# tokamak-network/Tokamak-zk-EVM

Measured on AMD Instinct MI355X. Metric: constraints/sec (prove step), higher is better.
Workload: dtype u32 limbs (255-bit Fr / 381-bit Fq modular integer arithmetic)

## Files before the change

include/tkmk.h:

```cpp
#ifndef TKMK_H
#define TKMK_H
#include <stdbool.h>
#include <stddef.h>
#include <stdint.h>

#ifdef __cplusplus
extern "C" {
#endif

typedef enum {
    TKMK_SUCCESS = 0,
    TKMK_ERR_INVALID_DEVICE = 1,
    TKMK_ERR_OUT_OF_MEMORY = 2,
    TKMK_ERR_INVALID_POINTER = 3,
    TKMK_ERR_ALLOCATION_FAILED = 4,
    TKMK_ERR_DEALLOCATION_FAILED = 5,
    TKMK_ERR_COPY_FAILED = 6,
    TKMK_ERR_SYNCHRONIZATION_FAILED = 7,
    TKMK_ERR_STREAM_CREATION_FAILED = 8,
    TKMK_ERR_STREAM_DESTRUCTION_FAILED = 9,
    TKMK_ERR_API_NOT_IMPLEMENTED = 10,
    TKMK_ERR_INVALID_ARGUMENT = 11,
    TKMK_ERR_NO_DEVICE = 12,
    TKMK_ERR_UNKNOWN = 999
} tkmk_error;

typedef struct { uint32_t limbs[8]; } tkmk_fr;
typedef struct { uint32_t limbs[12]; } tkmk_fq;
typedef struct { tkmk_fq x, y; } tkmk_g1_affine;
typedef struct { tkmk_fq x, y, z; } tkmk_g1_projective;
typedef void *tkmk_stream;

#define TKMK_BLS12_381_FR_ROOT_GENERATOR 5

tkmk_error tkmk_device_count(int *count);
tkmk_error tkmk_set_device(int device_id);
tkmk_error tkmk_diag_device_switch(int bound_device, int requested_device, int device_count);
tkmk_error tkmk_get_available_memory(size_t *total, size_t *free_bytes);
tkmk_error tkmk_malloc(void **ptr, size_t bytes);
tkmk_error tkmk_malloc_async(void **ptr, size_t bytes, tkmk_stream s);
tkmk_error tkmk_free(void *ptr);
tkmk_error tkmk_free_async(void *ptr, tkmk_stream s);
tkmk_error tkmk_memcpy_h2d(void *dst, const void *src, size_t bytes);
tkmk_error tkmk_memcpy_d2h(void *dst, const void *src, size_t bytes);
tkmk_error tkmk_memcpy_d2d(void *dst, const void *src, size_t bytes);
tkmk_error tkmk_memcpy_h2d_async(void *dst, const void *src, size_t bytes, tkmk_stream s);
tkmk_error tkmk_memcpy_d2h_async(void *dst, const void *src, size_t bytes, tkmk_stream s);
tkmk_error tkmk_memcpy_2d_d2d(void *dst, size_t dst_pitch, const void *src, size_t src_pitch, size_t width_bytes, size_t rows);
tkmk_error tkmk_memset(void *ptr, int value, size_t bytes);
tkmk_error tkmk_stream_create(tkmk_stream *s);
tkmk_error tkmk_stream_synchronize(tkmk_stream s);
tkmk_error tkmk_stream_destroy(tkmk_stream s);
tkmk_error tkmk_stream_set_background(tkmk_stream stream, int on);
tkmk_error tkmk_device_synchronize(void);
tkmk_error tkmk_release_scratch(void);
const char *tkmk_error_string(tkmk_error e);
tkmk_error bls12_381_generate_scalars(tkmk_fr *out_host, size_t n);
tkmk_error bls12_381_generate_random_affine_points(tkmk_g1_affine *out_host, size_t n);
int tkmk_is_hip_build(void);
tkmk_error tkmk_keccak256(const uint8_t *data, size_t len, uint8_t out[32]);
tkmk_error tkmk_r1cs_index(const uint8_t *section, size_t section_bytes, uint32_t n_constraints, uint32_t field_size,
                           uint64_t *starts, uint32_t *counts, size_t *consumed);

typedef struct {
    tkmk_stream stream_handle;
    int precompute_factor;
    int c;
    int bitsize;
    int batch_size;
    bool are_points_shared_in_batch;
    bool are_scalars_on_device;
    bool are_scalars_montgomery_form;
    bool are_points_on_device;
    bool are_points_montgomery_form;
    bool are_results_on_device;
    bool is_async;
    void *ext;
} tkmk_msm_config;

tkmk_msm_config tkmk_msm_default_config(void);

tkmk_error bls12_381_msm(const tkmk_fr *scalars, const tkmk_g1_affine *bases, int msm_size,
                         const tkmk_msm_config *cfg, tkmk_g1_projective *results);

tkmk_error bls12_381_msm_precompute_bases(const tkmk_g1_affine *bases, int msm_size, const tkmk_msm_config *cfg,
                                          tkmk_g1_affine *output_bases);

typedef struct {
    const tkmk_fr *scalars;
    const tkmk_g1_affine *bases;
    int msm_size;
} tkmk_msm_job;
tkmk_error tkmk_msm_multi(const tkmk_msm_job *jobs, int n_jobs, const tkmk_msm_config *cfg, tkmk_g1_projective *results);

#define TKMK_BASES_PLAIN 0
#define TKMK_BASES_MONTGOMERY 1
#define TKMK_BASES_CONVERTED 2
typedef struct {
    const tkmk_fr *scalars;
    const tkmk_g1_affine *bases;
    int msm_size;
    uint32_t scalar_cols, scalar_stride;
    uint32_t base_cols, base_stride;
    const uint32_t *base_index;
    uint64_t base_table_len;
    uint32_t table_c, table_factor;
} tkmk_msm_job_ex;
tkmk_error tkmk_msm_multi_ex(const tkmk_msm_job_ex *jobs, int n_jobs, const tkmk_msm_config *cfg, int bases_form,
                             tkmk_g1_projective *results);
tkmk_error bls12_381_msm_convert_bases(const tkmk_g1_affine *bases, uint64_t n, const tkmk_msm_config *cfg, tkmk_g1_affine *out);

typedef enum { TKMK_NTT_FORWARD = 0, TKMK_NTT_INVERSE = 1 } tkmk_ntt_dir;
typedef enum { TKMK_ORDER_NN = 0 } tkmk_ntt_ordering;

typedef struct {
    tkmk_stream stream_handle;
    tkmk_fr coset_gen;
    int batch_size;
    bool columns_batch;
    tkmk_ntt_ordering ordering;
    bool are_inputs_on_device;
    bool are_outputs_on_device;
    bool is_async;
    void *ext;
} tkmk_ntt_config;

typedef struct {
    tkmk_stream stream_handle;
    bool is_async;
    void *ext;
} tkmk_ntt_init_domain_config;

tkmk_ntt_config tkmk_ntt_default_config(void);
tkmk_error bls12_381_get_root_of_unity(uint64_t max_size, tkmk_fr *rou_out);
tkmk_error bls12_381_ntt_init_domain(const tkmk_fr *primitive_root, const tkmk_ntt_init_domain_config *cfg);
tkmk_error bls12_381_ntt_release_domain(void);
tkmk_error bls12_381_ntt_domain_size(uint64_t *size);
tkmk_error bls12_381_ntt(const tkmk_fr *input, int size, tkmk_ntt_dir dir, const tkmk_ntt_config *cfg,
                         tkmk_fr *output);

tkmk_error tkmk_bintt(const tkmk_fr *input, size_t x_size, size_t y_size, tkmk_ntt_dir dir,
                      const tkmk_fr *coset_x, const tkmk_fr *coset_y, bool on_device,
                      tkmk_stream stream, tkmk_fr *output);
tkmk_error tkmk_bintt_padded(const tkmk_fr *input, size_t in_x, size_t in_y, size_t x_size, size_t y_size, const tkmk_fr *coset_x,
                             const tkmk_fr *coset_y, tkmk_stream stream, tkmk_fr *output);

typedef struct {
    tkmk_stream stream_handle;
    bool is_a_on_device;
    bool is_b_on_device;
    bool is_result_on_device;
    bool is_async;
    int batch_size;
    bool columns_batch;
    void *ext;
} tkmk_vecops_config;

tkmk_vecops_config tkmk_vecops_default_config(void);
tkmk_error bls12_381_vector_add(const tkmk_fr *a, const tkmk_fr *b, uint64_t n, const tkmk_vecops_config *cfg, tkmk_fr *out);
tkmk_error bls12_381_vector_accumulate(tkmk_fr *a, const tkmk_fr *b, uint64_t n, const tkmk_vecops_config *cfg);
tkmk_error bls12_381_vector_sub(const tkmk_fr *a, const tkmk_fr *b, uint64_t n, const tkmk_vecops_config *cfg, tkmk_fr *out);
tkmk_error bls12_381_vector_mul(const tkmk_fr *a, const tkmk_fr *b, uint64_t n, const tkmk_vecops_config *cfg, tkmk_fr *out);
tkmk_error bls12_381_vector_div(const tkmk_fr *a, const tkmk_fr *b, uint64_t n, const tkmk_vecops_config *cfg, tkmk_fr *out);
tkmk_error bls12_381_vector_inv(const tkmk_fr *a, uint64_t n, const tkmk_vecops_config *cfg, tkmk_fr *out);
tkmk_error bls12_381_scalar_add_vec(const tkmk_fr *a, const tkmk_fr *b, uint64_t n, const tkmk_vecops_config *cfg, tkmk_fr *out);
tkmk_error bls12_381_scalar_sub_vec(const tkmk_fr *a, const tkmk_fr *b, uint64_t n, const tkmk_vecops_config *cfg, tkmk_fr *out);
tkmk_error bls12_381_scalar_mul_vec(const tkmk_fr *a, const tkmk_fr *b, uint64_t n, const tkmk_vecops_config *cfg, tkmk_fr *out);
tkmk_error bls12_381_vector_sum(const tkmk_fr *a, uint64_t n, const tkmk_vecops_config *cfg, tkmk_fr *out);
tkmk_error bls12_381_vector_product(const tkmk_fr *a, uint64_t n, const tkmk_vecops_config *cfg, tkmk_fr *out);
tkmk_error tkmk_vec_suffix_product(const tkmk_fr *a_dev, uint64_t n, tkmk_fr *out_dev, tkmk_stream stream);
tkmk_error bls12_381_matrix_transpose(const tkmk_fr *in, uint32_t rows, uint32_t cols, const tkmk_vecops_config *cfg, tkmk_fr *out);

tkmk_error tkmk_g1_ntt(const tkmk_g1_affine *in_dev, int bases_form, uint32_t in_stride, uint32_t x_size, uint32_t y_size, tkmk_ntt_dir dir,
                       tkmk_g1_affine *out_dev, tkmk_stream stream);
#define TKMK_G1_NTT_AXIS_X 1
#define TKMK_G1_NTT_AXIS_Y 2
tkmk_error tkmk_g1_ntt_axes(const tkmk_g1_affine *in_dev, int bases_form, uint32_t in_stride, uint32_t x_size, uint32_t y_size, tkmk_ntt_dir dir,
                            int axes, tkmk_g1_affine *out_dev, tkmk_stream stream);
tkmk_error tkmk_g1_scale(const tkmk_g1_affine *in_dev, uint64_t n, const tkmk_fr *scalar, tkmk_g1_affine *out_dev, tkmk_stream stream);
tkmk_error tkmk_g1_prefix_sums(const tkmk_g1_affine *in_dev, int bases_form, uint32_t rows, uint32_t cols, int transposed,
                               tkmk_g1_affine *out_dev, tkmk_stream stream);

typedef struct { tkmk_fq c0, c1; } tkmk_fq2;
typedef struct { tkmk_fq2 x, y; } tkmk_g2_affine;
typedef struct { tkmk_fq2 x, y, z; } tkmk_g2_projective;
tkmk_error bls12_381_g2_msm(const tkmk_fr *scalars, const tkmk_g2_affine *bases, int msm_size, const tkmk_msm_config *cfg,
                            tkmk_g2_projective *results);

typedef struct { uint32_t limbs[8]; } tkmk_bn254_fr;
typedef struct { uint32_t limbs[8]; } tkmk_bn254_fq;
typedef struct { tkmk_bn254_fq x, y; } tkmk_bn254_g1_affine;
typedef struct { tkmk_bn254_fq x, y, z; } tkmk_bn254_g1_projective;
tkmk_error bn254_msm(const tkmk_bn254_fr *scalars, const tkmk_bn254_g1_affine *bases, int msm_size,
                     const tkmk_msm_config *cfg, tkmk_bn254_g1_projective *results);
typedef struct {
    const tkmk_bn254_fr *scalars;
    const tkmk_bn254_g1_affine *bases;
    int msm_size;
} tkmk_bn254_msm_job;
tkmk_error bn254_msm_precompute_bases(const tkmk_bn254_g1_affine *bases, int msm_size, const tkmk_msm_config *cfg,
                                      tkmk_bn254_g1_affine *output_bases);
tkmk_error tkmk_bn254_msm_multi(const tkmk_bn254_msm_job *jobs, int n_jobs, const tkmk_msm_config *cfg,
                                tkmk_bn254_g1_projective *results);
tkmk_error bn254_get_root_of_unity(uint64_t max_size, tkmk_bn254_fr *rou_out);
tkmk_error bn254_ntt_init_domain(const tkmk_bn254_fr *primitive_root, const tkmk_ntt_init_domain_config *cfg);
tkmk_error bn254_ntt_release_domain(void);
tkmk_error bn254_ntt_domain_size(uint64_t *size);
tkmk_error bn254_ntt(const tkmk_bn254_fr *input, int size, tkmk_ntt_dir dir, const tkmk_ntt_config *cfg,
                     tkmk_bn254_fr *output);
tkmk_error tkmk_bn254_bintt(const tkmk_bn254_fr *input, size_t x_size, size_t y_size, tkmk_ntt_dir dir,
                            const tkmk_bn254_fr *coset_x, const tkmk_bn254_fr *coset_y, bool on_device, tkmk_stream stream,
                            tkmk_bn254_fr *output);
tkmk_error tkmk_bn254_fr_random_device(uint64_t seed, uint64_t first, uint64_t n, tkmk_bn254_fr *out_dev, tkmk_stream s);
tkmk_error tkmk_bn254_g1_batch_scalar_mul_device(const tkmk_bn254_fr *scalars_dev, const tkmk_bn254_g1_affine *base_host,
                                                 uint64_t n, tkmk_bn254_g1_affine *out_dev, tkmk_stream s);

tkmk_error tkmk_fr_random_device(uint64_t seed, uint64_t first, uint64_t n, tkmk_fr *out_dev, tkmk_stream s);
tkmk_error tkmk_gather_rows_device(const void *src_dev, uint32_t row_bytes, const uint32_t *idx_dev, uint64_t n, void *dst_dev,
                                   tkmk_stream s);
tkmk_error tkmk_g1_batch_scalar_mul_device(const tkmk_fr *scalars_dev, const tkmk_g1_affine *base_host,
                                           uint64_t n, tkmk_g1_affine *out_dev, tkmk_stream s);

tkmk_error tkmk_poly_find_degree(const tkmk_fr *coeffs_dev, uint32_t x_size, uint32_t y_size, int64_t *x_degree,
                                 int64_t *y_degree, tkmk_stream stream);
tkmk_error tkmk_poly_place(const tkmk_fr *src_dev, uint32_t sx, uint32_t sy, tkmk_fr *dst_dev, uint32_t dx, uint32_t dy,
                           uint32_t off_x, uint32_t off_y, tkmk_stream stream);
tkmk_error tkmk_poly_scale_coeffs(const tkmk_fr *src_dev, uint32_t x_size, uint32_t y_size, const tkmk_fr *factor_x,
                                  const tkmk_fr *factor_y, tkmk_fr *dst_dev, tkmk_stream stream);
tkmk_error tkmk_poly_mul_ones_x(const tkmk_fr *p_dev, uint32_t x_size, uint32_t y_size, uint32_t m, const tkmk_fr *scale,
                                uint32_t out_x_size, tkmk_fr *out_dev, tkmk_stream stream);
tkmk_error tkmk_poly_mul_x_minus_one_evals(const tkmk_fr *evals_dev, uint32_t x_size, uint32_t y_size, tkmk_fr *dst_dev,
                                           tkmk_stream stream);

typedef enum {
    TKMK_EXPR_LEAF = 0, TKMK_EXPR_CONST = 1, TKMK_EXPR_ADD = 2, TKMK_EXPR_SUB = 3, TKMK_EXPR_MUL = 4, TKMK_EXPR_SCALE = 5,
    TKMK_EXPR_MUL_X_MINUS_ONE = 6
} tkmk_expr_opcode;
typedef struct { uint8_t op; uint8_t arg; } tkmk_expr_instr;
tkmk_error tkmk_poly_expr_eval(const tkmk_expr_instr *prog, uint32_t n_instr, const tkmk_fr *const *leaves_dev, uint32_t n_leaves,
                               const tkmk_fr *consts, uint32_t n_consts, uint32_t x_size, uint32_t y_size, tkmk_fr *out_dev,
                               tkmk_stream stream);
typedef struct {
    const tkmk_fr *data;
    uint32_t x_len, y_len, rot_x, rot_y;
} tkmk_expr_leaf;
tkmk_error tkmk_poly_expr_eval_views(const tkmk_expr_instr *prog, uint32_t n_instr, const tkmk_expr_leaf *leaves, uint32_t n_leaves,
                                     const tkmk_fr *consts, uint32_t n_consts, uint32_t x_size, uint32_t y_size, tkmk_fr *out_dev,
                                     tkmk_stream stream);
tkmk_error tkmk_poly_expr_eval_views_slab(const tkmk_expr_instr *prog, uint32_t n_instr, const tkmk_expr_leaf *leaves, uint32_t n_leaves,
                                          const tkmk_fr *consts, uint32_t n_consts, uint32_t x_global, uint32_t x_first, uint32_t x_rows,
                                          uint32_t y_size, tkmk_fr *out_dev, tkmk_stream stream);
tkmk_error tkmk_poly_eval_x(const tkmk_fr *coeffs_dev, uint32_t x_size, uint32_t y_size, const tkmk_fr *x, tkmk_fr *out_dev,
                            tkmk_stream stream);
tkmk_error tkmk_poly_eval_y(const tkmk_fr *coeffs_dev, uint32_t x_size, uint32_t y_size, const tkmk_fr *y, tkmk_fr *out_dev,
                            tkmk_stream stream);
tkmk_error tkmk_poly_eval(const tkmk_fr *coeffs_dev, uint32_t x_size, uint32_t y_size, const tkmk_fr *x, const tkmk_fr *y,
                          tkmk_fr *out_host, tkmk_stream stream);
tkmk_error tkmk_poly_div_by_vanishing_opt(const tkmk_fr *p_dev, uint32_t x_size, uint32_t y_size, uint32_t c, uint32_t d,
                                          tkmk_fr *quo_x_dev, tkmk_fr *quo_y_dev, tkmk_stream stream);
tkmk_error tkmk_poly_lincomb(uint32_t n_terms, const tkmk_fr *coeffs_host, const tkmk_fr *const *polys_dev, const uint32_t *x_sizes,
                             const uint32_t *y_sizes, const uint32_t *off_x, const uint32_t *off_y, tkmk_fr *out_dev, uint32_t out_xs,
                             uint32_t out_ys, tkmk_stream stream);
tkmk_error tkmk_poly_div_by_ruffini(const tkmk_fr *p_dev, uint32_t x_size, uint32_t y_size, const tkmk_fr *x, const tkmk_fr *y,
// ... 56 lines not shown
```

tokamak-zk-evm_amd/csrc/ec_u.h:

```cpp
#pragma once
#include "ec.h"
#include "ffu.h"

template <class P>
struct ecu {
    using FU = ffu<P>;
    using FS = ff<P>;
    using GS = ec<FS>;
    using E = typename FU::E;
    struct A {
        E x, y;
    };
    struct X {
        E x, y, zz, zzz;
        bool inf;
    };

    static FF_HD X inf() {
        X r;
        r.x = FU::zero();
        r.y = FU::zero();
        r.zz = FU::zero();
        r.zzz = FU::zero();
        r.inf = true;
        return r;
    }
    static FF_HD bool load_affine(A &q, const affine_t<FS> &rec) {
        if (FS::is_zero(rec.x) && FS::is_zero(rec.y)) return false;
        q.x = FU::from_packed(rec.x);
        q.y = FU::from_packed(rec.y);
        return true;
    }
    static FF_HD A neg(const A &q) {
        A r;
        r.x = q.x;
        E m;
#pragma unroll
        for (int i = 0; i < FU::L; i++) m.l[i] = P::MODU[i];
        E t;
        uint32_t br = 0;
#pragma unroll
        for (int i = 0; i < FU::L; i++) {
            uint32_t d = m.l[i] - q.y.l[i] - br;
            br = d >> 31;
            t.l[i] = i < FU::L - 1 ? (d & FU::MASK) : d;
        }
        r.y = t;
        return r;
    }
    static FF_HD X from_affine(const A &q) {
        X r;
        r.x = q.x;
        r.y = q.y;
        r.zz = FU::one();
        r.zzz = FU::one();
        r.inf = false;
        return r;
    }

    static FF_HD xyzz_t<FS> to_sat(const X &p) {
        xyzz_t<FS> r;
        if (p.inf) return GS::inf();
        r.x = FU::to_sat_mont(p.x);
        r.y = FU::to_sat_mont(p.y);
        r.zz = FU::to_sat_mont(p.zz);
        r.zzz = FU::to_sat_mont(p.zzz);
        return r;
    }
    static FF_HD xyzz_t<FS> to_raw(const X &p) {
        xyzz_t<FS> r;
        if (p.inf) return GS::inf();
        r.x = FU::pack(FU::norm(p.x));
        r.y = FU::pack(FU::norm(p.y));
        r.zz = FU::pack(FU::norm(p.zz));
        r.zzz = FU::pack(FU::norm(p.zzz));
        return r;
    }
    static FF_HD xyzz_t<FS> raw_to_sat(const xyzz_t<FS> &raw) {
        if (FS::is_zero(raw.zz)) return GS::inf();
        xyzz_t<FS> r;
        r.x = FU::to_sat_mont(FU::unpack(raw.x));
        r.y = FU::to_sat_mont(FU::unpack(raw.y));
        r.zz = FU::to_sat_mont(FU::unpack(raw.zz));
        r.zzz = FU::to_sat_mont(FU::unpack(raw.zzz));
        return r;
    }
    static FF_HD X from_raw(const xyzz_t<FS> &raw) {
        X r;
        r.inf = FS::is_zero(raw.zz);
        if (r.inf) return inf();
        r.x = FU::unpack(raw.x);
        r.y = FU::unpack(raw.y);
        r.zz = FU::unpack(raw.zz);
        r.zzz = FU::unpack(raw.zzz);
        return r;
    }
    static FF_HD E from_sat_mont(const typename FS::E &s) {
        typename FS::E k;
#pragma unroll
        for (int i = 0; i < FS::N; i++) k.l[i] = P::KSATM[i];
        return FU::unpack(FS::mul(s, k));
    }
    static FF_HD X from_sat(const xyzz_t<FS> &p) {
        X r;
        r.inf = GS::is_inf(p);
        if (r.inf) return inf();
        r.x = from_sat_mont(p.x);
        r.y = from_sat_mont(p.y);
        r.zz = from_sat_mont(p.zz);
        r.zzz = from_sat_mont(p.zzz);
        return r;
    }
    static FF_HD X add_mixed_slow(const X &p, const A &q) {
        affine_t<FS> qs;
        qs.x = FU::to_sat_mont(q.x);
        qs.y = FU::to_sat_mont(q.y);
        return from_sat(GS::add_mixed(to_sat(p), qs));
    }

    static FF_HD X add_slow(const X &p, const X &q) { return from_sat(GS::add(to_sat(p), to_sat(q))); }
    static FF_HD X add(const X &p, const X &q) {
        if (p.inf) return q;
        if (q.inf) return p;
        E u1 = FU::mul(p.x, q.zz), u2 = FU::mul(q.x, p.zz);
        E s1 = FU::mul(p.y, q.zzz), s2 = FU::mul(q.y, p.zzz);
        E pd = FU::template sub<2>(u2, u1);
        if (FU::maybe_multiple_of_p(pd, 3)) return add_slow(p, q);
        E rd = FU::template sub<2>(s2, s1);
        E pp = FU::sqr(pd);
        E ppp = FU::mul(pd, pp);
        E qq = FU::mul(u1, pp);
        X r;
        r.inf = false;
        r.x = FU::template sub<4>(FU::sqr(rd), FU::add_dbl(ppp, qq));
        r.y = FU::mul_add(rd, FU::template sub<8>(qq, r.x), FU::template sub<2>(FU::zero(), s1), ppp);
        r.zz = FU::mul(FU::mul(p.zz, q.zz), pp);
        r.zzz = FU::mul(FU::mul(p.zzz, q.zzz), ppp);
        return r;
    }
    static FF_HD X dbl(const X &p) {
        if (p.inf) return p;
        E u = FU::dbl(p.y);
        E v = FU::sqr(u);
        E w = FU::mul(u, v);
        E sx = FU::mul(p.x, v);
        E x2 = FU::sqr(p.x);
        E m = FU::add(FU::dbl(x2), x2);
        X r;
        r.inf = false;
        r.x = FU::template sub<4>(FU::sqr(m), FU::dbl(sx));
        r.y = FU::mul_add(m, FU::template sub<8>(sx, r.x), FU::template sub<2>(FU::zero(), w), p.y);
        r.zz = FU::mul(v, p.zz);
        r.zzz = FU::mul(w, p.zzz);
        return r;
    }

    static FF_HD X add_mixed(const X &p, const A &q) {
        if (p.inf) return from_affine(q);
        E u2 = FU::mul(q.x, p.zz);
        E s2 = FU::mul(q.y, p.zzz);
        E pd = FU::template sub<8>(u2, p.x);
        if (FU::maybe_multiple_of_p(pd, 9)) return add_mixed_slow(p, q);
        E rd = FU::template sub<2>(s2, p.y);
        E pp = FU::sqr(pd);
        E ppp = FU::mul(pd, pp);
        E qq = FU::mul(p.x, pp);
        X r;
        r.inf = false;
        E t = FU::add_dbl(ppp, qq);
        r.x = FU::template sub<4>(FU::sqr(rd), t);
        E d = FU::template sub<8>(qq, r.x);
        r.y = FU::mul_add(rd, d, FU::template sub<2>(FU::zero(), p.y), ppp);
        r.zz = FU::mul(p.zz, pp);
        r.zzz = FU::mul(p.zzz, ppp);
        return r;
    }
};

using G1U = ecu<bls12_381_fq_params>;
```

tokamak-zk-evm_amd/csrc/ffu.h:

```cpp
#pragma once
#include <stdint.h>

#include "ff.h"

#if !defined(__HIP_DEVICE_COMPILE__)
#include <assert.h>
#define FFU_ASSERT(c) assert(c)
#else
#define FFU_ASSERT(c) ((void)0)
#endif

template <class P>
struct ffu {
    static constexpr int L = P::LU;
    static constexpr int N = P::N;
    static constexpr uint32_t W = P::WU, MASK = (1u << P::WU) - 1;
    struct alignas(8) E {
        uint32_t l[L];
    };
    using S = Fp<P>;

    static FF_HD E zero() {
        E r;
#pragma unroll
        for (int i = 0; i < L; i++) r.l[i] = 0;
        return r;
    }
    static FF_HD E one() {
        E r;
#pragma unroll
        for (int i = 0; i < L; i++) r.l[i] = P::ONEU[i];
        return r;
    }
    static FF_HD bool strict(const E &a) {
        for (int i = 0; i < L - 1; i++)
            if (a.l[i] > MASK) return false;
        return true;
    }
    static FF_HD bool below(const E &a, uint32_t k) { return (uint64_t)a.l[L - 1] * 1024 <= (uint64_t)k * P::TOP_PER_P_X1024 + 1024; }

    static FF_HD E norm(const E &a) {
        E r;
        uint32_t c = 0;
#pragma unroll
        for (int i = 0; i < L - 1; i++) {
            uint32_t t = a.l[i] + c;
            r.l[i] = t & MASK;
            c = t >> W;
        }
        r.l[L - 1] = a.l[L - 1] + c;
        return r;
    }
    static FF_HD E add(const E &a, const E &b) {
        FFU_ASSERT(strict(a) && strict(b));
        E t;
#pragma unroll
        for (int i = 0; i < L; i++) t.l[i] = a.l[i] + b.l[i];
        return norm(t);
    }
    static FF_HD E dbl(const E &a) { return add(a, a); }
    static FF_HD E add_dbl(const E &a, const E &b) {
        FFU_ASSERT(strict(a) && strict(b));
        E t;
#pragma unroll
        for (int i = 0; i < L; i++) t.l[i] = a.l[i] + (b.l[i] << 1);
        return norm(t);
    }
    template <int K>
    static FF_HD E sub(const E &a, const E &b) {
        FFU_ASSERT(strict(a) && strict(b) && below(b, K));
        E t;
#pragma unroll
        for (int i = 0; i < L; i++) {
            uint32_t c = K == 2 ? P::SUB2[i] : K == 4 ? P::SUB4[i] : K == 8 ? P::SUB8[i] : P::SUB16[i];
            FFU_ASSERT(c >= b.l[i]);
            t.l[i] = a.l[i] + (c - b.l[i]);
        }
        return norm(t);
    }

    static FF_HD E mul(const E &a, const E &b) {
        FFU_ASSERT(strict(a) && strict(b) && a.l[L - 1] <= MASK && b.l[L - 1] <= MASK);
        uint32_t m[L];
        uint64_t acc = 0;
        E r;
#pragma unroll
        for (int k = 0; k < L; k++) {
#pragma unroll
            for (int j = 0; j <= k; j++) acc += (uint64_t)a.l[j] * b.l[k - j];
#pragma unroll
            for (int j = 0; j < k; j++) acc += (uint64_t)m[j] * P::MODU[k - j];
            m[k] = ((uint32_t)acc * P::INVU) & MASK;
            acc += (uint64_t)m[k] * P::MODU[0];
            acc >>= W;
        }
#pragma unroll
        for (int k = L; k < 2 * L - 1; k++) {
#pragma unroll
            for (int j = k - L + 1; j < L; j++) {
                acc += (uint64_t)a.l[j] * b.l[k - j];
                acc += (uint64_t)m[j] * P::MODU[k - j];
            }
            r.l[k - L] = (uint32_t)acc & MASK;
            acc >>= W;
        }
        r.l[L - 1] = (uint32_t)acc;
        return r;
    }
    static FF_HD E mul_add(const E &a, const E &b, const E &c, const E &d) {
        static_assert(3 * L < (1 << (64 - 2 * (int)W)), "column accumulator would overflow");
        FFU_ASSERT(strict(a) && strict(b) && strict(c) && strict(d));
        FFU_ASSERT(a.l[L - 1] <= MASK && b.l[L - 1] <= MASK && c.l[L - 1] <= MASK && d.l[L - 1] <= MASK);
        uint32_t m[L];
        uint64_t acc = 0;
        E r;
#pragma unroll
        for (int k = 0; k < L; k++) {
#pragma unroll
            for (int j = 0; j <= k; j++) {
                acc += (uint64_t)a.l[j] * b.l[k - j];
                acc += (uint64_t)c.l[j] * d.l[k - j];
            }
#pragma unroll
            for (int j = 0; j < k; j++) acc += (uint64_t)m[j] * P::MODU[k - j];
            m[k] = ((uint32_t)acc * P::INVU) & MASK;
            acc += (uint64_t)m[k] * P::MODU[0];
            acc >>= W;
        }
#pragma unroll
        for (int k = L; k < 2 * L - 1; k++) {
#pragma unroll
            for (int j = k - L + 1; j < L; j++) {
                acc += (uint64_t)a.l[j] * b.l[k - j];
                acc += (uint64_t)c.l[j] * d.l[k - j];
                acc += (uint64_t)m[j] * P::MODU[k - j];
            }
            r.l[k - L] = (uint32_t)acc & MASK;
            acc >>= W;
        }
        r.l[L - 1] = (uint32_t)acc;
        return r;
    }
    static FF_HD E sqr(const E &a) {
        FFU_ASSERT(strict(a) && a.l[L - 1] <= MASK);
        uint32_t m[L], a2[L];
#pragma unroll
        for (int i = 0; i < L; i++) a2[i] = a.l[i] << 1;
        uint64_t acc = 0;
        E r;
#pragma unroll
        for (int k = 0; k < L; k++) {
#pragma unroll
            for (int j = 0; 2 * j < k; j++) acc += (uint64_t)a2[j] * a.l[k - j];
            if ((k & 1) == 0) acc += (uint64_t)a.l[k / 2] * a.l[k / 2];
#pragma unroll
            for (int j = 0; j < k; j++) acc += (uint64_t)m[j] * P::MODU[k - j];
            m[k] = ((uint32_t)acc * P::INVU) & MASK;
            acc += (uint64_t)m[k] * P::MODU[0];
            acc >>= W;
        }
#pragma unroll
        for (int k = L; k < 2 * L - 1; k++) {
#pragma unroll
            for (int j = k - L + 1; 2 * j < k; j++) acc += (uint64_t)a2[j] * a.l[k - j];
            if ((k & 1) == 0) acc += (uint64_t)a.l[k / 2] * a.l[k / 2];
#pragma unroll
            for (int j = k - L + 1; j < L; j++) acc += (uint64_t)m[j] * P::MODU[k - j];
            r.l[k - L] = (uint32_t)acc & MASK;
            acc >>= W;
        }
        r.l[L - 1] = (uint32_t)acc;
        return r;
    }

    static FF_HD bool maybe_multiple_of_p(const E &a, uint32_t jmax) { return ((a.l[0] * P::PINVU) & MASK) <= jmax; }

    static FF_HD E unpack(const S &s) {
        E r;
#pragma unroll
        for (int i = 0; i < L; i++) {
            int bit = (int)W * i, w = bit >> 5, sh = bit & 31;
            uint32_t lo = w < N ? s.l[w] : 0u, hi = w + 1 < N ? s.l[w + 1] : 0u;
            uint32_t v = sh ? (lo >> sh) | (hi << (32 - sh)) : lo;
            r.l[i] = i < L - 1 ? (v & MASK) : v;
        }
        return r;
    }
    static FF_HD S pack(const E &a) {
        S s;
#pragma unroll
        for (int w = 0; w < N; w++) {
            uint32_t v = 0;
#pragma unroll
            for (int i = 0; i < L; i++) {
                int lo = (int)W * i - 32 * w;
                if (lo >= 32 || lo + 32 <= 0) continue;
                v |= lo >= 0 ? a.l[i] << lo : a.l[i] >> (-lo);
            }
            s.l[w] = v;
        }
        return s;
    }
    static FF_HD E cond_sub_p(const E &a) {
        E t;
        uint32_t br = 0;
#pragma unroll
        for (int i = 0; i < L; i++) {
            uint32_t d = a.l[i] - P::MODU[i] - br;
            br = d >> 31;
            t.l[i] = i < L - 1 ? (d & MASK) : d;
        }
        uint32_t keep = 0u - br;
        E r;
#pragma unroll
        for (int i = 0; i < L; i++) r.l[i] = (a.l[i] & keep) | (t.l[i] & ~keep);
        return r;
    }
    static FF_HD S to_sat_mont(const E &a) {
        E c;
#pragma unroll
        for (int i = 0; i < L; i++) c.l[i] = P::RSATU[i];
        return pack(cond_sub_p(mul(a, c)));
    }
    static FF_HD E from_packed(const S &s) { return unpack(s); }
};

using Fqu = ffu<bls12_381_fq_params>;
using fqu_t = Fqu::E;
```

tokamak-zk-evm_amd/csrc/msm.hip:

```cpp
#include <stdio.h>
#include <stdlib.h>

#include <algorithm>
#include <map>
#include <memory>
#include <mutex>
#include <vector>

#include "common.h"
#include "ec_u.h"

#define TK_MSM_PRIMARY 1
#define TK_MSM_NS tk_msm_bls12_381
#define TK_MSM_FR_PARAMS bls12_381_fr_params
#define TK_MSM_FQ_PARAMS bls12_381_fq_params
#define TK_MSM_SCALAR_BITS 255
#define TK_MSM_ABI_FR tkmk_fr
#define TK_MSM_ABI_AFFINE tkmk_g1_affine
#define TK_MSM_ABI_PROJ tkmk_g1_projective
#define TK_MSM_ABI_JOB tkmk_msm_job
#define TK_MSM_SYM_MSM bls12_381_msm
#define TK_MSM_SYM_MULTI tkmk_msm_multi
#define TK_MSM_SYM_PRECOMPUTE bls12_381_msm_precompute_bases
#define TK_MSM_ABI_JOB_EX tkmk_msm_job_ex
#define TK_MSM_SYM_MULTI_EX tkmk_msm_multi_ex
#define TK_MSM_SYM_CONVERT bls12_381_msm_convert_bases
#include "msm_impl.inc"
```

tokamak-zk-evm_amd/csrc/msm_impl.inc:

```
namespace TK_MSM_NS {

using FrP = TK_MSM_FR_PARAMS;
using FqP = TK_MSM_FQ_PARAMS;
using Fr = ff<FrP>;
using Fq = ff<FqP>;
using fr_t = Fr::E;
using fq_t = Fq::E;
using G1 = ec<Fq>;
using g1_affine_t = affine_t<Fq>;
using g1_xyzz_t = xyzz_t<Fq>;
using G1U = ecu<FqP>;
using G1K = G1;
using FqK = Fq;
using g1k_xyzz = g1_xyzz_t;
using g1k_aff = g1_affine_t;
using abi_fr = TK_MSM_ABI_FR;
using abi_affine = TK_MSM_ABI_AFFINE;
using abi_proj = TK_MSM_ABI_PROJ;
using abi_job = TK_MSM_ABI_JOB;
#ifdef TK_MSM_SYM_MULTI_EX
using abi_job_ex = TK_MSM_ABI_JOB_EX;
#endif
constexpr size_t AFF_BYTES = sizeof(g1_affine_t), FR_BYTES = sizeof(fr_t);

static_assert(sizeof(g1_affine_t) == 2 * 4 * Fq::N && sizeof(g1_xyzz_t) == 4 * 4 * Fq::N, "layout");
static_assert(sizeof(abi_fr) == FR_BYTES && sizeof(abi_affine) == AFF_BYTES && sizeof(abi_proj) == 3 * 4 * Fq::N, "ABI layout");
static_assert(Fr::N == 8, "k_digits reads 8 scalar limbs");

struct msm_plan_t {
    uint32_t n;
    uint32_t c;
    uint32_t W;
    uint32_t B;
    uint32_t chunks;
    uint32_t chunk_len;
    uint32_t bits;
    uint32_t n_src;
    uint32_t W_src;
    uint32_t chunk;
    uint32_t win_parts;
    uint32_t hi_bits, lo_bits;
    uint32_t big;
};

struct msm_view_t {
    const uint32_t *index;
    uint32_t cols, stride;
    uint32_t limit;
    uint32_t *flag;
};
__device__ __forceinline__ uint32_t view_at(const msm_view_t &v, uint32_t k) {
    uint32_t r = k;
    if (v.index) r = v.index[k];
    else if (v.cols) {
        uint32_t row = k / v.cols;
        r = row * v.stride + (k - row * v.cols);
    }
    if (v.limit && r >= v.limit) {
        if (v.flag) atomicOr(v.flag, 1u);
        r = 0;
    }
    return r;
}
__device__ __forceinline__ uint32_t view_at_expanded(const msm_view_t &v, uint32_t k, uint32_t n_src, uint32_t level_rows) {
    if (!level_rows) return view_at(v, k);
    uint32_t j = k / n_src;
    return j * level_rows + view_at(v, k - j * n_src);
}
static inline msm_view_t view_identity() { return msm_view_t{nullptr, 0, 0, 0, nullptr}; }
static inline bool view_is_identity(const msm_view_t &v) { return !v.index && !v.cols; }

__global__ __launch_bounds__(256) void k_convert_bases(const g1_affine_t *__restrict__ in, g1_affine_t *__restrict__ out,
                                                      uint64_t n, int in_montgomery, msm_view_t bv) {
    uint64_t i = (uint64_t)blockIdx.x * blockDim.x + threadIdx.x;
    if (i >= n) return;
    g1_affine_t p = tk_load(in + view_at(bv, (uint32_t)i));
    if (!G1::is_inf(p)) {
        fq_t k;
#pragma unroll
        for (int j = 0; j < Fq::N; j++) k.l[j] = in_montgomery ? FqP::KSATM[j] : FqP::KSAT[j];
        p.x = Fq::mul(Fq::canon(p.x), k);
        p.y = Fq::mul(Fq::canon(p.y), k);
    }
    tk_store(out + i, p);
}

__global__ __launch_bounds__(256) void k_digits(const fr_t *__restrict__ scalars, uint32_t *__restrict__ dig, msm_plan_t pl,
                                               int scalars_mont, msm_view_t sv) {
    uint32_t i = blockIdx.x * blockDim.x + threadIdx.x;
    if (i >= pl.n_src) return;
    fr_t s = Fr::canon(tk_load(scalars + view_at(sv, i)));
    if (scalars_mont) s = Fr::from_mont(s);
    uint32_t carry = 0;
    const uint32_t mask = (1u << pl.c) - 1u;
    const uint32_t groups = pl.n / pl.n_src;
    uint32_t j = 0, t = 0;
    for (uint32_t w = 0; w < groups * pl.W; w++) {
        if (w >= pl.W_src) {
            dig[(uint64_t)t * pl.n + (uint64_t)j * pl.n_src + i] = 0;
            if (++t == pl.W) { t = 0; j++; }
            continue;
        }
        uint32_t lo = w * pl.c, li = lo >> 5, sh = lo & 31;
        uint32_t raw = 0;
        if (li < 8) {
            raw = s.l[li] >> sh;
            if (sh + pl.c > 32 && li + 1 < 8) raw |= s.l[li + 1] << (32 - sh);
        }
        raw &= mask;
        if (lo + pl.c > pl.bits) {
            uint32_t keep = pl.bits > lo ? pl.bits - lo : 0;
            raw &= keep >= 32 ? 0xffffffffu : ((1u << keep) - 1u);
        }
        uint32_t v = raw + carry;
        uint32_t rec;
        if (v > pl.B) {
            rec = ((1u << pl.c) - v) | 0x80000000u;
            carry = 1;
        } else {
            rec = v;
            carry = 0;
        }
        dig[(uint64_t)t * pl.n + (uint64_t)j * pl.n_src + i] = rec;
        if (++t == pl.W) { t = 0; j++; }
    }
}

__global__ __launch_bounds__(128) void k_precompute_bases(const g1_affine_t *__restrict__ in, g1_affine_t *__restrict__ out, uint64_t n,
                                                         int in_montgomery, uint32_t factor, uint32_t step) {
    uint64_t i = (uint64_t)blockIdx.x * blockDim.x + threadIdx.x;
    if (i >= n) return;
    g1_affine_t p = tk_load(in + i);
    const bool inf = G1::is_inf(p);
    if (!inf) {
        p.x = Fq::canon(p.x);
        p.y = Fq::canon(p.y);
        if (!in_montgomery) {
            p.x = Fq::to_mont(p.x);
            p.y = Fq::to_mont(p.y);
        }
    }
    fq_t k;
#pragma unroll
    for (int l = 0; l < Fq::N; l++) k.l[l] = FqP::KSATM[l];
    g1_xyzz_t acc = G1::from_affine(p);
    for (uint32_t j = 0; j < factor; j++) {
        g1_affine_t a = p;
        if (j) {
            for (uint32_t d = 0; d < step; d++) acc = G1::dbl(acc);
            a = G1::to_affine(acc);
        }
        if (!inf) {
            a.x = Fq::mul(a.x, k);
            a.y = Fq::mul(a.y, k);
        }
        tk_store(out + (uint64_t)j * n + i, a);
    }
}

__global__ __launch_bounds__(1024) void k_hist(const uint32_t *__restrict__ dig, uint32_t *__restrict__ counts, msm_plan_t pl,
                                              uint32_t shift) {
    extern __shared__ uint32_t hist[];
    const uint32_t w = blockIdx.y, ch = blockIdx.x;
    for (uint32_t b = threadIdx.x; b < pl.B; b += blockDim.x) hist[b] = 0;
    __syncthreads();
    uint32_t lo = ch * pl.chunk_len, hi = lo + pl.chunk_len;
    if (hi > pl.n) hi = pl.n;
    const uint32_t *d = dig + (uint64_t)w * pl.n;
    uint32_t i = lo + threadIdx.x;
    for (; i + 3 * 1024 < hi; i += 4 * 1024) {
        uint32_t r[4];
#pragma unroll
        for (int j = 0; j < 4; j++) r[j] = d[i + 1024 * j] & 0x7fffffffu;
#pragma unroll
        for (int j = 0; j < 4; j++)
            if (r[j]) atomicAdd(&hist[(r[j] - 1) >> shift], 1u);
    }
    for (; i < hi; i += 1024) {
        uint32_t r = d[i] & 0x7fffffffu;
        if (r) atomicAdd(&hist[(r - 1) >> shift], 1u);
    }
    __syncthreads();
    uint32_t *c = counts + (uint64_t)w * pl.B * pl.chunks;
    for (uint32_t b = threadIdx.x; b < pl.B; b += blockDim.x) c[(uint64_t)b * pl.chunks + ch] = hist[b];
}

__global__ __launch_bounds__(1024) void k_scan_local(const uint32_t *__restrict__ counts, uint32_t *__restrict__ local,
                                                    uint32_t *__restrict__ gtot, msm_plan_t pl) {
    __shared__ uint32_t part[1024];
    const uint32_t w = blockIdx.y, t = threadIdx.x, b = blockIdx.x * 1024 + t;
    uint32_t sum = 0;
    if (b < pl.B) {
        const uint32_t *c = counts + ((uint64_t)w * pl.B + b) * pl.chunks;
        uint32_t k = 0;
        for (; k + 8 <= pl.chunks; k += 8) {
            uint32_t v[8];
#pragma unroll
            for (int j = 0; j < 8; j++) v[j] = c[k + j];
#pragma unroll
            for (int j = 0; j < 8; j++) sum += v[j];
        }
        for (; k < pl.chunks; k++) sum += c[k];
    }
    part[t] = sum;
    __syncthreads();
    for (uint32_t off = 1; off < 1024; off <<= 1) {
        uint32_t v = t >= off ? part[t - off] : 0;
        __syncthreads();
        part[t] += v;
        __syncthreads();
    }
    if (b < pl.B) local[(uint64_t)w * pl.B + b] = part[t] - sum;
    if (t == 1023) gtot[w * gridDim.x + blockIdx.x] = part[t];
}
__global__ __launch_bounds__(1024) void k_scan_apply(uint32_t *__restrict__ counts, const uint32_t *__restrict__ local,
                                                    const uint32_t *__restrict__ gtot, uint32_t *__restrict__ bstart, msm_plan_t pl) {
    const uint32_t w = blockIdx.y, t = threadIdx.x, b = blockIdx.x * 1024 + t;
    uint32_t base = 0, total = 0;
    for (uint32_t g = 0; g < gridDim.x; g++) {
        uint32_t v = gtot[w * gridDim.x + g];
        if (g < blockIdx.x) base += v;
        total += v;
    }
    uint32_t *bs = bstart + (uint64_t)w * (pl.B + 1);
    if (b < pl.B) {
        uint32_t run = base + local[(uint64_t)w * pl.B + b];
        bs[b] = run;
        uint32_t *c = counts + ((uint64_t)w * pl.B + b) * pl.chunks;
        uint32_t k = 0;
        for (; k + 8 <= pl.chunks; k += 8) {
            uint32_t v[8];
#pragma unroll
            for (int j = 0; j < 8; j++) v[j] = c[k + j];
#pragma unroll
            for (int j = 0; j < 8; j++) {
                c[k + j] = run;
                run += v[j];
            }
        }
        for (; k < pl.chunks; k++) {
            uint32_t v = c[k];
            c[k] = run;
            run += v;
        }
    }
    if (blockIdx.x == 0 && t == 0) bs[pl.B] = total;
}

#define SCW_TPB 16
#define SCW_BINS (1024 / SCW_TPB)
__global__ __launch_bounds__(1024) void k_scan_local_wide(const uint32_t *__restrict__ counts, uint32_t *__restrict__ local,
                                                         uint32_t *__restrict__ gtot, msm_plan_t pl) {
    __shared__ uint32_t binsum[SCW_BINS];
    const uint32_t w = blockIdx.y, t = threadIdx.x, slot = t / SCW_TPB, sub = t % SCW_TPB, b = blockIdx.x * SCW_BINS + slot;
    const uint32_t per = (pl.chunks + SCW_TPB - 1) / SCW_TPB, lo = sub * per, hi = lo + per < pl.chunks ? lo + per : pl.chunks;
    uint32_t sum = 0;
    if (b < pl.B) {
        const uint32_t *c = counts + ((uint64_t)w * pl.B + b) * pl.chunks;
        for (uint32_t k = lo; k < hi; k++) sum += c[k];
    }
#pragma unroll
    for (uint32_t off = SCW_TPB / 2; off > 0; off >>= 1) sum += __shfl_down(sum, off, SCW_TPB);
    if (sub == 0) binsum[slot] = sum;
    __syncthreads();
    if (t < SCW_BINS) {
        uint32_t mine = binsum[t], incl = mine;
#pragma unroll
        for (uint32_t off = 1; off < SCW_BINS; off <<= 1) {
            uint32_t v = __shfl_up(incl, off, SCW_BINS);
            if (t >= off) incl += v;
        }
        const uint32_t bb = blockIdx.x * SCW_BINS + t;
        if (bb < pl.B) local[(uint64_t)w * pl.B + bb] = incl - mine;
        if (t == SCW_BINS - 1) gtot[w * gridDim.x + blockIdx.x] = incl;
    }
}
__global__ __launch_bounds__(1024) void k_scan_apply_wide(uint32_t *__restrict__ counts, const uint32_t *__restrict__ local,
                                                         const uint32_t *__restrict__ gtot, uint32_t *__restrict__ bstart, msm_plan_t pl) {
    const uint32_t w = blockIdx.y, t = threadIdx.x, slot = t / SCW_TPB, sub = t % SCW_TPB, b = blockIdx.x * SCW_BINS + slot;
    const uint32_t per = (pl.chunks + SCW_TPB - 1) / SCW_TPB, lo = sub * per, hi = lo + per < pl.chunks ? lo + per : pl.chunks;
    uint32_t base = 0, total = 0;
    for (uint32_t g = 0; g < gridDim.x; g++) {
        uint32_t v = gtot[w * gridDim.x + g];
        if (g < blockIdx.x) base += v;
        total += v;
    }
    uint32_t *bs = bstart + (uint64_t)w * (pl.B + 1);
    uint32_t *c = counts + ((uint64_t)w * pl.B + (b < pl.B ? b : 0)) * pl.chunks;
    uint32_t sum = 0;
    if (b < pl.B)
        for (uint32_t k = lo; k < hi; k++) sum += c[k];
    uint32_t incl = sum;
#pragma unroll
    for (uint32_t off = 1; off < SCW_TPB; off <<= 1) {
        uint32_t v = __shfl_up(incl, off, SCW_TPB);
        if (sub >= off) incl += v;
    }
    if (b < pl.B) {
        const uint32_t bin_start = base + local[(uint64_t)w * pl.B + b];
        if (sub == 0) bs[b] = bin_start;
        uint32_t run = bin_start + incl - sum;
        for (uint32_t k = lo; k < hi; k++) {
            uint32_t v = c[k];
            c[k] = run;
            run += v;
        }
    }
    if (blockIdx.x == 0 && t == 0) bs[pl.B] = total;
}

__global__ __launch_bounds__(1024) void k_scatter(const uint32_t *__restrict__ dig, const uint32_t *__restrict__ counts,
// ... 48 lines not shown
        const uint32_t *cs = seg_start + (uint64_t)w * (coarse_bins + 1);
        uint32_t s0 = cs[cb], s1 = cs[cb + 1];
        uint32_t per = sc_part_len(s1 - s0, parts);
        lo = s0 + part * per;
        if (lo > s1) lo = s1;
        hi = lo + per < s1 ? lo + per : s1;
        base = s0;
    } else {
        lo = part * chunk_len;
        hi = lo + chunk_len < n ? lo + chunk_len : n;
        if (lo > n) lo = n;
    }
    in0 += (uint64_t)w * n;
    if (PASS_B) in1 += (uint64_t)w * n;
    out0 += (uint64_t)w * n;
    if (!PASS_B) out1 += (uint64_t)w * n;
    if (tid < bins) cur[tid] = cursors[((uint64_t)sgm * bins + tid) * parts + part] + base;
    hist[tid] = 0;
    __syncthreads();
    for (uint32_t tlo = lo; tlo < hi; tlo += SC_TILE) {
        uint32_t v0[SC_PER], v1[SC_PER], rk[SC_PER];
        bool ok[SC_PER];
#pragma unroll
        for (int j = 0; j < SC_PER; j++) {
            uint32_t k = tlo + tid + 1024u * j;
            ok[j] = k < hi;
            v0[j] = v1[j] = rk[j] = 0;
            if (ok[j]) {
                if (PASS_B) {
                    v0[j] = in0[k];
                    v1[j] = in1[k];
                } else {
                    uint32_t rec = in0[k], r = rec & 0x7fffffffu;
                    ok[j] = r != 0;
                    v0[j] = (ok[j] ? view_at_expanded(bv, k, n_src, level_rows) : 0u) | (rec & 0x80000000u);
                    v1[j] = r - 1;
                }
            }
            if (ok[j]) rk[j] = atomicAdd(&hist[PASS_B ? (v1[j] & fmask) : (v1[j] >> fbits)], 1u);
        }
        __syncthreads();
        static_assert(SC_MAXBINS == 1024, "one bin per thread of the 1024-thread workgroup");
        const uint32_t mine = hist[tid];
        uint32_t incl = mine;
        const uint32_t lane = tid & 63u, wave = tid >> 6;
#pragma unroll
        for (uint32_t off = 1; off < 64; off <<= 1) {
            uint32_t t = __shfl_up(incl, off, 64);
            if (lane >= off) incl += t;
        }
        if (lane == 63) wsum[wave] = incl;
        __syncthreads();
        uint32_t before = 0, total = 0;
#pragma unroll
        for (uint32_t w2 = 0; w2 < 16; w2++) {
            uint32_t v = wsum[w2];
            total += v;
            if (w2 < wave) before += v;
        }
        start[tid] = before + incl - mine;
        __syncthreads();
#pragma unroll
        for (int j = 0; j < SC_PER; j++)
            if (ok[j]) {
                uint32_t b = PASS_B ? (v1[j] & fmask) : (v1[j] >> fbits);
                uint32_t pos = start[b] + rk[j];
                sv0[pos] = v0[j];
                sv1[pos] = v1[j];
            }
        __syncthreads();
#pragma unroll
        for (int j = 0; j < SC_PER; j++) {
            uint32_t k2 = tid + 1024u * j;
            if (k2 < total) {
                uint32_t a0 = sv0[k2], a1 = sv1[k2];
                uint32_t b = PASS_B ? (a1 & fmask) : (a1 >> fbits);
                uint32_t g = cur[b] + (k2 - start[b]);
                out0[g] = a0;
                if (!PASS_B) out1[g] = (uint16_t)(a1 & fmask);
            }
        }
        __syncthreads();
        cur[tid] += hist[tid];
        hist[tid] = 0;
        __syncthreads();
    }
}

__global__ __launch_bounds__(1024) void k_hist_fine(const uint16_t *__restrict__ key, const uint32_t *__restrict__ seg_start,
                                                   uint32_t *__restrict__ counts, uint32_t n, uint32_t coarse_bins, uint32_t fbits) {
    __shared__ uint32_t hist[SC_MAXFINE];
    const uint32_t fb_n = 1u << fbits;
    const uint32_t tid = threadIdx.x, part = blockIdx.x, parts = gridDim.x, sgm = blockIdx.y;
    const uint32_t w = sgm / coarse_bins, cb = sgm - w * coarse_bins;
    const uint32_t *cs = seg_start + (uint64_t)w * (coarse_bins + 1);
    uint32_t s0 = cs[cb], s1 = cs[cb + 1];
    uint32_t per = sc_part_len(s1 - s0, parts);
    uint32_t lo = s0 + part * per;
    if (lo > s1) lo = s1;
    uint32_t hi = lo + per < s1 ? lo + per : s1;
    if (tid < fb_n) hist[tid] = 0;
    __syncthreads();
    const uint16_t *k = key + (uint64_t)w * n;
    uint32_t i = lo + tid;
    for (; i + 3 * 1024 < hi; i += 4 * 1024) {
        uint32_t r[4];
#pragma unroll
        for (int j = 0; j < 4; j++) r[j] = k[i + 1024 * j];
#pragma unroll
        for (int j = 0; j < 4; j++) atomicAdd(&hist[r[j] & (fb_n - 1)], 1u);
    }
    for (; i < hi; i += 1024) atomicAdd(&hist[k[i] & (fb_n - 1)], 1u);
    __syncthreads();
    if (tid < fb_n) counts[((uint64_t)sgm * fb_n + tid) * parts + part] = hist[tid];
}

__global__ __launch_bounds__(256) void k_bstart_assemble(const uint32_t *__restrict__ coarse_start, const uint32_t *__restrict__ fine_start,
                                                        uint32_t *__restrict__ bstart, uint32_t W, uint32_t B, uint32_t coarse_bins,
                                                        uint32_t fbits) {
    uint64_t e = (uint64_t)blockIdx.x * blockDim.x + threadIdx.x;
    if (e >= (uint64_t)W * (B + 1)) return;
    uint32_t w = (uint32_t)(e / (B + 1)), b = (uint32_t)(e - (uint64_t)w * (B + 1));
    const uint32_t *cs = coarse_start + (uint64_t)w * (coarse_bins + 1);
    if (b == B) {
        bstart[e] = cs[coarse_bins];
        return;
    }
    uint32_t cb = b >> fbits, fb = b & ((1u << fbits) - 1);
    bstart[e] = cs[cb] + fine_start[((uint64_t)w * coarse_bins + cb) * ((1u << fbits) + 1) + fb];
}

__global__ void k_count_entries(const uint32_t *__restrict__ bstart, uint32_t W, uint32_t B, unsigned long long *__restrict__ cell) {
    unsigned long long t = 0;
    for (uint32_t w = 0; w < W; w++) t += bstart[(uint64_t)w * (B + 1) + B];
    atomicAdd(cell, t);
}

#define MSM_CHUNK 64
#define MSM_BIG 12
#define MSM_GIANT 2048
#define MSM_GIANT_PARTS 32
#define MSM_GIANT_CAP 2048

__device__ __forceinline__ uint32_t bucket_of(const uint32_t *__restrict__ bs, uint32_t B, uint32_t pos) {
    uint32_t lo = 0, hi = B;
    while (hi - lo > 1) {
        uint32_t mid = (lo + hi) >> 1;
        if (bs[mid] <= pos) lo = mid;
        else hi = mid;
    }
    return lo;
}

__global__ __launch_bounds__(256, 2) void k_accumulate_chunks(const g1_affine_t *__restrict__ bases, const uint32_t *__restrict__ sorted,
                                                          const uint32_t *__restrict__ bstart, g1_xyzz_t *__restrict__ buckets,
                                                          g1_xyzz_t *__restrict__ frag_head, g1_xyzz_t *__restrict__ frag_tail,
                                                          msm_plan_t pl, uint32_t chunks_per_window) {
    uint32_t gid = blockIdx.x * blockDim.x + threadIdx.x;
    if (gid >= pl.W * chunks_per_window) return;
    uint32_t w = gid / chunks_per_window, t = gid - w * chunks_per_window;
    const uint32_t *bs = bstart + (uint64_t)w * (pl.B + 1);
    const uint32_t total = bs[pl.B];
    uint32_t lo = t * pl.chunk;
    if (lo >= total) return;
    uint32_t hi = lo + pl.chunk < total ? lo + pl.chunk : total;
    const uint32_t *s = sorted + (uint64_t)w * pl.n;
    uint32_t b = bucket_of(bs, pl.B, lo);
    uint32_t bend = bs[b + 1];
    while (bend <= lo) bend = bs[++b + 1];
    const bool first_starts_here = bs[b] == lo;
    uint32_t nb = b + 2 <= pl.B ? bs[b + 2] : 0xffffffffu;
    uint32_t seg_lo = lo;
    G1U::X acc = G1U::inf();
    uint32_t rec_next = s[lo], rec_next2 = lo + 1 < hi ? s[lo + 1] : 0u;
    g1_affine_t raw = tk_load(bases + (rec_next & 0x7fffffffu));
    for (uint32_t k = lo; k < hi; k++) {
        const uint32_t rec = rec_next;
        G1U::A q;
        const bool have = G1U::load_affine(q, raw);
        rec_next = rec_next2;
        if (k + 1 < hi) {
            raw = tk_load(bases + (rec_next & 0x7fffffffu));
        }
        if (k + 2 < hi) rec_next2 = s[k + 2];
        if (have) {
            if (rec & 0x80000000u) q = G1U::neg(q);
            acc = G1U::add_mixed(acc, q);
        }
        if (k + 1 == bend || k + 1 == hi) {
            bool whole = (seg_lo != lo || first_starts_here) && k + 1 == bend;
            g1_xyzz_t *dst;
            if (whole) dst = buckets + (uint64_t)w * pl.B + b;
            else if (seg_lo == lo) dst = frag_head + (uint64_t)w * chunks_per_window + t;
            else dst = frag_tail + (uint64_t)w * chunks_per_window + t;
            tk_store(dst, G1U::to_raw(acc));
            acc = G1U::inf();
            seg_lo = k + 1;
            if (k + 1 < hi) {
                do {
                    b++;
                    bend = nb;
                    nb = b + 2 <= pl.B ? bs[b + 2] : 0xffffffffu;
                } while (bend <= k + 1);
            }
        }
    }
}

__global__ __launch_bounds__(256) void k_combine(const uint32_t *__restrict__ bstart, g1_xyzz_t *__restrict__ buckets,
                                                const g1_xyzz_t *__restrict__ frag_head, const g1_xyzz_t *__restrict__ frag_tail,
                                                msm_plan_t pl, uint32_t chunks_per_window, uint32_t *__restrict__ big,
                                                uint32_t big_cap, uint32_t *__restrict__ giant) {
    uint32_t gid = blockIdx.x * blockDim.x + threadIdx.x;
    if (gid >= pl.W * pl.B) return;
    uint32_t w = gid / pl.B, b = gid - w * pl.B;
    const uint32_t *bs = bstart + (uint64_t)w * (pl.B + 1);
    uint32_t sb = bs[b], eb = bs[b + 1];
    if (eb == sb) return;
    uint32_t t0 = sb / pl.chunk, t1 = (eb - 1) / pl.chunk;
    if (t0 == t1) return;
    if (t1 - t0 > MSM_GIANT) {
        uint32_t slot = atomicAdd(&giant[0], 1u);
        if (slot < MSM_GIANT_CAP) {
            giant[1 + slot] = gid;
            return;
        }
    }
    if (t1 - t0 > pl.big) {
        uint32_t slot = atomicAdd(&big[0], 1u);
        if (slot < big_cap) {
            big[1 + slot] = gid;
            return;
        }
    }
    const g1_xyzz_t *fh = frag_head + (uint64_t)w * chunks_per_window, *ft = frag_tail + (uint64_t)w * chunks_per_window;
    G1U::X acc = G1U::from_raw(tk_load(sb == t0 * pl.chunk ? fh + t0 : ft + t0));
    for (uint32_t t = t0 + 1; t <= t1; t++) acc = G1U::add(acc, G1U::from_raw(tk_load(fh + t)));
    tk_store(buckets + gid, G1U::to_raw(acc));
}

__global__ __launch_bounds__(256) void k_combine_big(const uint32_t *__restrict__ bstart, g1_xyzz_t *__restrict__ buckets,
                                                    const g1_xyzz_t *__restrict__ frag_head, const g1_xyzz_t *__restrict__ frag_tail,
                                                    msm_plan_t pl, uint32_t chunks_per_window, const uint32_t *__restrict__ big,
                                                    uint32_t big_cap) {
    __shared__ g1_xyzz_t sh[256];
    const uint32_t lane = threadIdx.x & 63u, wave = threadIdx.x >> 6;
    uint32_t count = big[0] < big_cap ? big[0] : big_cap;
    for (uint32_t base = blockIdx.x * 4u; base < count; base += gridDim.x * 4u) {
        const uint32_t i = base + wave;
        const bool live = i < count;
        uint32_t gid = 0;
        G1U::X acc = G1U::inf();
        if (live) {
            gid = big[1 + i];
            uint32_t w = gid / pl.B, b = gid - w * pl.B;
            const uint32_t *bs = bstart + (uint64_t)w * (pl.B + 1);
            uint32_t sb = bs[b], eb = bs[b + 1];
            uint32_t t0 = sb / pl.chunk, t1 = (eb - 1) / pl.chunk;
            const g1_xyzz_t *fh = frag_head + (uint64_t)w * chunks_per_window, *ft = frag_tail + (uint64_t)w * chunks_per_window;
            for (uint32_t t = t0 + lane; t <= t1; t += 64) {
                const g1_xyzz_t *src = (t == t0 && sb != t0 * pl.chunk) ? ft + t : fh + t;
                acc = G1U::add(acc, G1U::from_raw(tk_load(src)));
            }
        }
        sh[threadIdx.x] = G1U::to_raw(acc);
        __syncthreads();
        for (uint32_t st = 32; st > 0; st >>= 1) {
            if (lane < st) {
                acc = G1U::add(acc, G1U::from_raw(sh[threadIdx.x + st]));
                sh[threadIdx.x] = G1U::to_raw(acc);
            }
            __syncthreads();
        }
        if (live && lane == 0) tk_store(buckets + gid, G1U::to_raw(acc));
        __syncthreads();
    }
}

__global__ __launch_bounds__(256) void k_combine_giant_parts(const uint32_t *__restrict__ bstart, const g1_xyzz_t *__restrict__ frag_head,
                                                            const g1_xyzz_t *__restrict__ frag_tail, msm_plan_t pl,
                                                            uint32_t chunks_per_window, const uint32_t *__restrict__ giant,
                                                            g1_xyzz_t *__restrict__ part_out) {
    __shared__ g1_xyzz_t sh[256];
    uint32_t count = giant[0] < MSM_GIANT_CAP ? giant[0] : MSM_GIANT_CAP;
    for (uint32_t item = blockIdx.x; item < count * MSM_GIANT_PARTS; item += gridDim.x) {
        uint32_t i = item / MSM_GIANT_PARTS, part = item - i * MSM_GIANT_PARTS;
        uint32_t gid = giant[1 + i];
        uint32_t w = gid / pl.B, b = gid - w * pl.B;
        const uint32_t *bs = bstart + (uint64_t)w * (pl.B + 1);
        uint32_t sb = bs[b], eb = bs[b + 1];
        uint32_t t0 = sb / pl.chunk, t1 = (eb - 1) / pl.chunk;
        uint32_t per = (t1 - t0 + MSM_GIANT_PARTS) / MSM_GIANT_PARTS;
        uint32_t lo = t0 + part * per, hi = lo + per - 1 < t1 ? lo + per - 1 : t1;
        const g1_xyzz_t *fh = frag_head + (uint64_t)w * chunks_per_window, *ft = frag_tail + (uint64_t)w * chunks_per_window;
        G1U::X acc = G1U::inf();
        for (uint32_t t = lo + threadIdx.x; t <= hi && lo <= t1; t += 256) {
            const g1_xyzz_t *src = (t == t0 && sb != t0 * pl.chunk) ? ft + t : fh + t;
            acc = G1U::add(acc, G1U::from_raw(tk_load(src)));
        }
        sh[threadIdx.x] = G1U::to_raw(acc);
        __syncthreads();
        for (uint32_t st = 128; st > 0; st >>= 1) {
            if (threadIdx.x < st) {
                acc = G1U::add(acc, G1U::from_raw(sh[threadIdx.x + st]));
                sh[threadIdx.x] = G1U::to_raw(acc);
            }
            __syncthreads();
        }
        if (threadIdx.x == 0) tk_store(part_out + item, G1U::to_raw(acc));
        __syncthreads();
    }
}
__global__ __launch_bounds__(64) void k_combine_giant_final(g1_xyzz_t *__restrict__ buckets, const uint32_t *__restrict__ giant,
                                                           const g1_xyzz_t *__restrict__ part_in) {
    __shared__ g1_xyzz_t sh[MSM_GIANT_PARTS];
    uint32_t count = giant[0] < MSM_GIANT_CAP ? giant[0] : MSM_GIANT_CAP;
    for (uint32_t i = blockIdx.x; i < count; i += gridDim.x) {
        G1U::X acc = G1U::inf();
        if (threadIdx.x < MSM_GIANT_PARTS) {
            sh[threadIdx.x] = tk_load(part_in + (uint64_t)i * MSM_GIANT_PARTS + threadIdx.x);
            acc = G1U::from_raw(sh[threadIdx.x]);
        }
        __syncthreads();
        for (uint32_t st = MSM_GIANT_PARTS / 2; st > 0; st >>= 1) {
            if (threadIdx.x < st) {
                acc = G1U::add(acc, G1U::from_raw(sh[threadIdx.x + st]));
                sh[threadIdx.x] = G1U::to_raw(acc);
            }
            __syncthreads();
        }
        if (threadIdx.x == 0) tk_store(buckets + giant[1 + i], G1U::to_raw(acc));
        __syncthreads();
    }
}

#define MSM_SEG 8
__global__ __launch_bounds__(128) void k_reduce_segments(const g1_xyzz_t *__restrict__ buckets, g1_xyzz_t *__restrict__ seg_out,
                                                        msm_plan_t pl, uint32_t segs) {
    uint32_t gid = blockIdx.x * blockDim.x + threadIdx.x;
    if (gid >= pl.W * segs) return;
    uint32_t w = gid / segs, sg = gid - w * segs;
    uint32_t v0 = sg * MSM_SEG;
    uint32_t len = pl.B - v0 < MSM_SEG ? pl.B - v0 : MSM_SEG;
    const g1_xyzz_t *bk = buckets + (uint64_t)w * pl.B + v0;
    G1U::X run = G1U::inf(), tot = G1U::inf();
    for (int k = (int)len - 1; k >= 0; k--) {
        run = G1U::add(run, G1U::from_raw(tk_load(bk + k)));
        tot = G1U::add(tot, run);
    }
    if (v0) {
        G1U::X m = G1U::inf();
        for (int bit = 31 - __builtin_clz(v0); bit >= 0; bit--) {
            m = G1U::dbl(m);
            if ((v0 >> bit) & 1) m = G1U::add(m, run);
        }
        tot = G1U::add(tot, m);
    }
    tk_store(seg_out + gid, G1U::to_raw(tot));
}

// ... 167 lines not shown
    }
    for (int i = 0; i < Fq::N; i++) {
        o->x.limbs[i] = x.l[i];
        o->y.limbs[i] = y.l[i];
        o->z.limbs[i] = z.l[i];
    }
}

#ifdef TK_MSM_PRIMARY
TK_API tkmk_msm_config tkmk_msm_default_config(void) {
    tkmk_msm_config c;
    c.stream_handle = nullptr;
    c.precompute_factor = 1;
    c.c = 0;
    c.bitsize = 0;
    c.batch_size = 1;
    c.are_points_shared_in_batch = true;
    c.are_scalars_on_device = false;
    c.are_scalars_montgomery_form = false;
    c.are_points_on_device = false;
    c.are_points_montgomery_form = false;
    c.are_results_on_device = false;
    c.is_async = false;
    c.ext = nullptr;
    return c;
}
#endif


static bool xyzz_same_point(const g1_xyzz_t &a, const g1_xyzz_t &b) {
    g1_affine_t pa = G1::to_affine(a), pb = G1::to_affine(b);
    return Fq::eq(pa.x, pb.x) && Fq::eq(pa.y, pb.y);
}
static tkmk_error msm_debug_check(const msm_plan_t &pl, const fr_t *scalars, const g1_affine_t *bases, const uint32_t *d_dig,
                                  const uint32_t *d_sorted, const uint32_t *d_bstart, const g1_xyzz_t *d_buckets, hipStream_t s) {
    TK_HIP(hipStreamSynchronize(s));
    TK_HIP(hipGetLastError());
    std::vector<fr_t> sc(pl.n);
    std::vector<g1_affine_t> bs(pl.n);
    std::vector<uint32_t> dig((size_t)pl.W * pl.n), sorted((size_t)pl.W * pl.n), bstart((size_t)pl.W * (pl.B + 1));
    std::vector<g1_xyzz_t> buckets((size_t)pl.W * pl.B);
    TK_HIP(hipMemcpy(sc.data(), scalars, sc.size() * sizeof(fr_t), hipMemcpyDeviceToHost));
    TK_HIP(hipMemcpy(bs.data(), bases, bs.size() * sizeof(g1_affine_t), hipMemcpyDeviceToHost));
    {
        fq_t rp;
        for (int j = 0; j < Fq::N; j++) rp.l[j] = FqP::KSATM[j];
        fq_t rinv = Fq::inv(Fq::to_mont(rp));
        for (auto &b : bs)
            if (!G1::is_inf(b)) {
                b.x = Fq::mul(Fq::to_mont(b.x), rinv);
                b.y = Fq::mul(Fq::to_mont(b.y), rinv);
            }
    }
    TK_HIP(hipMemcpy(dig.data(), d_dig, dig.size() * 4, hipMemcpyDeviceToHost));
    TK_HIP(hipMemcpy(sorted.data(), d_sorted, sorted.size() * 4, hipMemcpyDeviceToHost));
    TK_HIP(hipMemcpy(bstart.data(), d_bstart, bstart.size() * 4, hipMemcpyDeviceToHost));
    TK_HIP(hipMemcpy(buckets.data(), d_buckets, buckets.size() * sizeof(g1_xyzz_t), hipMemcpyDeviceToHost));
    fprintf(stderr, "[msm debug] n=%u c=%u W=%u B=%u chunks=%u chunk_len=%u\n", pl.n, pl.c, pl.W, pl.B, pl.chunks, pl.chunk_len);
    int bad = 0;
    for (uint32_t i = 0; i < pl.n && bad < 5; i++) {
        unsigned __int128 acc = 0;
        for (int w = (int)pl.W - 1; w >= 0; w--) {
            uint32_t rec = dig[(size_t)w * pl.n + i];
            long long d = (long long)(rec & 0x7fffffffu);
            if (rec & 0x80000000u) d = -d;
            if ((rec & 0x7fffffffu) > pl.B) { fprintf(stderr, "[msm debug] digit too large i=%u w=%d rec=%08x\n", i, w, rec); bad++; }
            if ((uint32_t)w * pl.c < 100) acc = (acc << pl.c) + (unsigned __int128)(__int128)d;
        }
        uint64_t lo = (uint64_t)sc[i].l[0] | ((uint64_t)sc[i].l[1] << 32);
        (void)lo;
    }
    for (uint32_t w = 0; w < pl.W; w++) {
        const uint32_t *bsw = &bstart[(size_t)w * (pl.B + 1)];
        uint32_t nz = 0;
        for (uint32_t i = 0; i < pl.n; i++) nz += (dig[(size_t)w * pl.n + i] & 0x7fffffffu) != 0;
        if (bsw[pl.B] != nz && bad < 20) { fprintf(stderr, "[msm debug] w=%u total %u != nonzero digits %u\n", w, bsw[pl.B], nz); bad++; }
        for (uint32_t b = 0; b < pl.B; b++) {
            if (bsw[b] > bsw[b + 1]) { if (bad < 20) fprintf(stderr, "[msm debug] w=%u b=%u bstart not monotone\n", w, b); bad++; continue; }
            g1_xyzz_t acc = G1::inf();
            for (uint32_t k = bsw[b]; k < bsw[b + 1]; k++) {
                uint32_t rec = sorted[(size_t)w * pl.n + k], i = rec & 0x7fffffffu;
                if (i >= pl.n) { if (bad < 20) fprintf(stderr, "[msm debug] w=%u b=%u bad index %u\n", w, b, i); bad++; continue; }
                uint32_t drec = dig[(size_t)w * pl.n + i];
                if ((drec & 0x7fffffffu) != b + 1 || ((drec ^ rec) & 0x80000000u)) {
                    if (bad < 20) fprintf(stderr, "[msm debug] w=%u b=%u entry %u: digit rec %08x does not belong here\n", w, b, k, drec);
                    bad++;
                }
                g1_affine_t pnt = bs[i];
                if (rec & 0x80000000u) pnt.y = Fq::neg(pnt.y);
                acc = G1::add_mixed(acc, pnt);
            }
            buckets[(size_t)w * pl.B + b] = G1U::raw_to_sat(buckets[(size_t)w * pl.B + b]);
            bool okb = xyzz_same_point(acc, buckets[(size_t)w * pl.B + b]);
            if (atoi(getenv("TKMK_MSM_DEBUG")) >= 2 && w == 7 && bsw[b + 1] > bsw[b])
                fprintf(stderr, "[msm debug] w7 b=%u pos=%u cnt=%u %s\n", b, bsw[b], bsw[b + 1] - bsw[b], okb ? "ok" : "BAD");
            if (!okb) {
                if (bad < 20) {
                    const g1_xyzz_t &dv = buckets[(size_t)w * pl.B + b];
                    uint32_t rec0 = bsw[b + 1] > bsw[b] ? sorted[(size_t)w * pl.n + bsw[b]] : 0;
                    const char *cls = "other";
                    if (G1::is_inf(dv)) cls = "inf";
                    else if (xyzz_same_point(G1::neg(acc), dv)) cls = "negated";
                    fprintf(stderr, "[msm debug] w=%u b=%u bucket sum mismatch (%u entries) rec0=%08x device=%s zz0=%08x x0=%08x\n", w, b,
                            bsw[b + 1] - bsw[b], rec0, cls, dv.zz.l[0], dv.x.l[0]);
                }
                bad++;
            }
        }
    }
    fprintf(stderr, "[msm debug] %d inconsistencies\n", bad);
    return TKMK_SUCCESS;
}

#define MSM_MAX_WINDOWS 128
static uint32_t msm_choose_chunk(uint64_t entries, uint32_t W, uint32_t n) {
    static const uint32_t slots = [] {
        int dev = 0, cus = 256;
        if (hipGetDevice(&dev) == hipSuccess) (void)hipDeviceGetAttribute(&cus, hipDeviceAttributeMultiprocessorCount, dev);
        if (cus <= 0) cus = 256;
        return (uint32_t)cus * 4u * 2u * 64u;
    }();
    if (getenv("TKMK_MSM_FIXED_CHUNK")) return MSM_CHUNK;
    if (const char *e = getenv("TKMK_MSM_CHUNK_LEN")) {
        int v = atoi(e);
        if (v >= 8 && v <= 8192) return (uint32_t)v;
    }
    uint64_t target = entries / (8ull * slots);
    if (target < 48) target = 48;
    if (target > 224) target = 224;
    uint64_t r = (entries + target * slots / 2) / (target * slots);
    if (r < 1) r = 1;
    uint64_t lanes_per_window = r * slots / W;
    if (lanes_per_window < 1) lanes_per_window = 1;
    uint64_t chunk = (n + lanes_per_window - 1) / lanes_per_window;
    if (chunk < 32) chunk = 32;
    if (chunk > 256) chunk = 256;
    if (entries > (1ull << 30)) {
        uint64_t big = entries / (32ull * slots);
        if (big > 4096) big = 4096;
        if (big > chunk) chunk = big;
    }
    return (uint32_t)chunk;
}
#define MSM_MAX_C 20
static uint32_t msm_resolve_c(uint32_t c_req, uint32_t n_src) {
    uint32_t c = c_req ? c_req : choose_c(n_src);
    if (c < 2) c = 2;
    if (c > MSM_MAX_C) c = MSM_MAX_C;
    static const bool force_one_pass = getenv("TKMK_MSM_ONE_PASS") != nullptr;
    if (c > 16 && (force_one_pass || n_src < (1u << 18))) c = 16;
    return c;
}

static thread_local bool tl_background_batch = false;
static tkmk_error msm_enqueue(const fr_t *scalars, const g1_affine_t *bases_mont, uint32_t n_src, uint32_t factor, uint32_t c_req,
                              uint32_t bits, bool scalars_mont, hipStream_t s, g1_xyzz_t *wins_host, msm_plan_t *plan_out,
                              msm_view_t sv = view_identity(), msm_view_t bv = view_identity(), uint32_t level_rows = 0) {
    msm_plan_t pl;
    static const bool force_one_pass = getenv("TKMK_MSM_ONE_PASS") != nullptr;
    pl.bits = bits;
    pl.c = level_rows ? c_req : msm_resolve_c(c_req, n_src);
    if (pl.c < 2 || pl.c > MSM_MAX_C) return TKMK_ERR_INVALID_ARGUMENT;
    pl.n_src = n_src;
    pl.W_src = bits / pl.c + 1;
    if (factor < 1) factor = 1;
    if (factor > pl.W_src) factor = pl.W_src;
    if ((uint64_t)n_src * factor >= (1ull << 31)) return TKMK_ERR_INVALID_ARGUMENT;
    if (factor > 1 && !view_is_identity(bv) && !level_rows) return TKMK_ERR_INVALID_ARGUMENT;
    if (level_rows && (uint64_t)level_rows * factor >= (1ull << 31)) return TKMK_ERR_INVALID_ARGUMENT;
    const uint32_t n = n_src * factor;
    pl.n = n;
    pl.W = (pl.W_src + factor - 1) / factor;
    pl.B = 1u << (pl.c - 1);
    pl.chunk = msm_choose_chunk((uint64_t)pl.W * n, pl.W, n);
    {
        static const uint32_t big_env = getenv("TKMK_MSM_BIG") ? (uint32_t)atoi(getenv("TKMK_MSM_BIG")) : 0u;
        const uint64_t avg_spans = (uint64_t)n / ((uint64_t)pl.chunk * pl.B);
        pl.big = big_env ? big_env : (avg_spans >= 4 ? 4u * MSM_BIG : MSM_BIG);
    }
    pl.win_parts = pl.W >= 8 ? MSM_WIN_PARTS : 32;
    pl.hi_bits = pl.lo_bits = 0;
    if (pl.W == 1 && pl.c >= 15) {
        pl.lo_bits = (pl.c - 1) / 2;
        pl.hi_bits = pl.c - 1 - pl.lo_bits;
    }
    static const bool no_rowcol = getenv("TKMK_MSM_SEGMENT_TAIL") != nullptr;
    if (no_rowcol) pl.hi_bits = pl.lo_bits = 0;
    uint32_t want = (512 + pl.W - 1) / pl.W;
    if (getenv("TKMK_MSM_CHUNKS")) want = (uint32_t)atoi(getenv("TKMK_MSM_CHUNKS"));
    uint32_t maxc = (n + 8191) / 8192;
    pl.chunks = want < maxc ? want : maxc;
    if (pl.chunks < 1) pl.chunks = 1;
    pl.chunk_len = (n + pl.chunks - 1) / pl.chunks;

    tk_scratch d_dig, d_sorted, d_counts, d_bstart, d_buckets, d_segs, d_wins;
    TK_TRY(d_dig.alloc((size_t)pl.W * n * 4, s));
    TK_TRY(d_sorted.alloc((size_t)pl.W * n * 4, s));
    const bool two_pass = !force_one_pass && pl.c >= 13 && n >= (1u << 18);
    if (pl.c > 16 && !two_pass) return TKMK_ERR_INVALID_ARGUMENT;
    {
        const uint32_t fb = pl.c >= 19 ? 9u : pl.c >= 17 ? 8u : 7u;
        TK_TRY(d_counts.alloc((size_t)pl.W * (two_pass ? (pl.B >> fb) : pl.B) * pl.chunks * 4, s));
    }
    TK_TRY(d_bstart.alloc((size_t)pl.W * (pl.B + 1) * 4, s));
    TK_TRY(d_buckets.alloc((size_t)pl.W * pl.B * sizeof(g1_xyzz_t), s));
    uint32_t segs = (pl.B + MSM_SEG - 1) / MSM_SEG;
    TK_TRY(d_segs.alloc((size_t)pl.W * segs * sizeof(g1_xyzz_t), s));
    TK_TRY(d_wins.alloc((size_t)pl.W * pl.win_parts * sizeof(g1_xyzz_t), s));

    tk_stat_add(TK_STAT_MSM_POINTS, n_src);
    tk_stat_add(TK_STAT_MSM_CALLS, 1);
    tk_prof prof(s);
    hipLaunchKernelGGL(k_digits, tk_div_up(n_src, 256), 256, 0, s, scalars, d_dig.as<uint32_t>(), pl, scalars_mont ? 1 : 0, sv);
    prof.mark("msm.digits");
    size_t lds = (size_t)pl.B * 4;
    static std::once_flag attr_once;
    static hipError_t attr_err = hipSuccess;
    std::call_once(attr_once, [] {
        attr_err = hipFuncSetAttribute((const void *)k_hist, hipFuncAttributeMaxDynamicSharedMemorySize, 128 * 1024);
        if (attr_err == hipSuccess)
            attr_err = hipFuncSetAttribute((const void *)k_scatter, hipFuncAttributeMaxDynamicSharedMemorySize, 128 * 1024);
    });
    TK_HIP(attr_err);
    if (!two_pass) {
        hipLaunchKernelGGL(k_hist, dim3(pl.chunks, pl.W), 1024, lds, s, (const uint32_t *)d_dig.p, d_counts.as<uint32_t>(), pl, 0u);
        prof.mark("msm.hist");
        const uint32_t groups = (pl.B + 1023) / 1024;
        tk_scratch d_local, d_gtot;
        TK_TRY(d_local.alloc((size_t)pl.W * pl.B * 4, s));
        TK_TRY(d_gtot.alloc((size_t)pl.W * groups * 4, s));
        hipLaunchKernelGGL(k_scan_local, dim3(groups, pl.W), 1024, 0, s, (const uint32_t *)d_counts.p, d_local.as<uint32_t>(),
                           d_gtot.as<uint32_t>(), pl);
        hipLaunchKernelGGL(k_scan_apply, dim3(groups, pl.W), 1024, 0, s, d_counts.as<uint32_t>(), (const uint32_t *)d_local.p,
                           (const uint32_t *)d_gtot.p, d_bstart.as<uint32_t>(), pl);
        prof.mark("msm.scan");
        hipLaunchKernelGGL(k_scatter, dim3(pl.chunks, pl.W), 1024, lds, s, (const uint32_t *)d_dig.p, (const uint32_t *)d_counts.p,
                           d_sorted.as<uint32_t>(), pl, bv, level_rows);
        prof.mark("msm.scatter");
    } else {
        const uint32_t fbits = pl.c >= 19 ? 9u : pl.c >= 17 ? 8u : 7u, FB = 1u << fbits, CB = pl.B >> fbits;
        tk_scratch d_aidx, d_akey, d_cs, d_localA, d_gtotA, d_cntB, d_fs, d_localB, d_gtotB;
        TK_TRY(d_aidx.alloc((size_t)pl.W * n * 4, s));
        TK_TRY(d_akey.alloc((size_t)pl.W * n * 2, s));
        TK_TRY(d_cs.alloc((size_t)pl.W * (CB + 1) * 4, s));
        msm_plan_t pa = pl;
        pa.B = CB;
        hipLaunchKernelGGL(k_hist, dim3(pl.chunks, pl.W), 1024, (size_t)CB * 4, s, (const uint32_t *)d_dig.p, d_counts.as<uint32_t>(), pa,
                           fbits);
        prof.mark("msm.hist");
        TK_TRY(d_localA.alloc((size_t)pl.W * CB * 4, s));
        const bool wide_scan = pl.W <= 4 && pl.chunks >= 64;
        const uint32_t groupsA = wide_scan ? (CB + SCW_BINS - 1) / SCW_BINS : 1u;
        TK_TRY(d_gtotA.alloc((size_t)pl.W * groupsA * 4, s));
        if (wide_scan) {
            hipLaunchKernelGGL(k_scan_local_wide, dim3(groupsA, pl.W), 1024, 0, s, (const uint32_t *)d_counts.p, d_localA.as<uint32_t>(),
                               d_gtotA.as<uint32_t>(), pa);
            hipLaunchKernelGGL(k_scan_apply_wide, dim3(groupsA, pl.W), 1024, 0, s, d_counts.as<uint32_t>(), (const uint32_t *)d_localA.p,
                               (const uint32_t *)d_gtotA.p, d_cs.as<uint32_t>(), pa);
        } else {
            hipLaunchKernelGGL(k_scan_local, dim3(1, pl.W), 1024, 0, s, (const uint32_t *)d_counts.p, d_localA.as<uint32_t>(),
                               d_gtotA.as<uint32_t>(), pa);
            hipLaunchKernelGGL(k_scan_apply, dim3(1, pl.W), 1024, 0, s, d_counts.as<uint32_t>(), (const uint32_t *)d_localA.p,
                               (const uint32_t *)d_gtotA.p, d_cs.as<uint32_t>(), pa);
        }
        prof.mark("msm.scan");
        hipLaunchKernelGGL(k_scatter_staged<false>, dim3(pl.chunks, pl.W), 1024, 0, s, (const uint32_t *)d_dig.p, (const uint16_t *)nullptr,
                           (const uint32_t *)nullptr, (const uint32_t *)d_counts.p, d_aidx.as<uint32_t>(), d_akey.as<uint16_t>(), n, CB, CB,
                           pl.chunk_len, fbits, bv, pl.n_src, level_rows);
        const uint32_t segs_b = pl.W * CB;
        TK_TRY(d_cntB.alloc((size_t)segs_b * FB * SC_PARTS * 4, s));
        TK_TRY(d_fs.alloc((size_t)segs_b * (FB + 1) * 4, s));
        TK_TRY(d_localB.alloc((size_t)segs_b * FB * 4, s));
        TK_TRY(d_gtotB.alloc((size_t)segs_b * 4, s));
        hipLaunchKernelGGL(k_hist_fine, dim3(SC_PARTS, segs_b), 1024, 0, s, (const uint16_t *)d_akey.p, (const uint32_t *)d_cs.p,
                           d_cntB.as<uint32_t>(), n, CB, fbits);
        msm_plan_t pb = pl;
        pb.B = FB;
        pb.chunks = SC_PARTS;
        hipLaunchKernelGGL(k_scan_local, dim3(1, segs_b), 1024, 0, s, (const uint32_t *)d_cntB.p, d_localB.as<uint32_t>(),
                           d_gtotB.as<uint32_t>(), pb);
        hipLaunchKernelGGL(k_scan_apply, dim3(1, segs_b), 1024, 0, s, d_cntB.as<uint32_t>(), (const uint32_t *)d_localB.p,
                           (const uint32_t *)d_gtotB.p, d_fs.as<uint32_t>(), pb);
        hipLaunchKernelGGL(k_bstart_assemble, tk_div_up((size_t)pl.W * (pl.B + 1), 256), 256, 0, s, (const uint32_t *)d_cs.p,
                           (const uint32_t *)d_fs.p, d_bstart.as<uint32_t>(), pl.W, pl.B, CB, fbits);
        hipLaunchKernelGGL(k_scatter_staged<true>, dim3(SC_PARTS, segs_b), 1024, 0, s, (const uint32_t *)d_aidx.p, (const uint16_t *)d_akey.p,
                           (const uint32_t *)d_cs.p, (const uint32_t *)d_cntB.p, d_sorted.as<uint32_t>(), (uint16_t *)nullptr, n, FB, CB,
                           0u, fbits, view_identity(), 0u, 0u);
        prof.mark("msm.scatter");
    }
    if (unsigned long long *cell = tk_stat_device_entries())
        hipLaunchKernelGGL(k_count_entries, 1, 1, 0, s, (const uint32_t *)d_bstart.p, pl.W, pl.B, cell);
    const uint32_t cpw = (n + pl.chunk - 1) / pl.chunk;
    const uint32_t big_cap = pl.W * pl.B;
    tk_scratch d_fh, d_ft, d_big, d_giant, d_gpart;
    TK_TRY(d_fh.alloc((size_t)pl.W * cpw * sizeof(g1_xyzz_t), s));
    TK_TRY(d_ft.alloc((size_t)pl.W * cpw * sizeof(g1_xyzz_t), s));
    TK_TRY(d_big.alloc((size_t)(big_cap + 1) * 4, s));
    TK_TRY(d_giant.alloc((size_t)(MSM_GIANT_CAP + 1) * 4, s));
    TK_TRY(d_gpart.alloc((size_t)MSM_GIANT_CAP * MSM_GIANT_PARTS * sizeof(g1_xyzz_t), s));
    TK_HIP(hipMemsetAsync(d_buckets.p, 0, (size_t)pl.W * pl.B * sizeof(g1_xyzz_t), s));
    TK_HIP(hipMemsetAsync(d_big.p, 0, 4, s));
    TK_HIP(hipMemsetAsync(d_giant.p, 0, 4, s));
    static const uint32_t acc_lds = [] {
        const char *e = getenv("TKMK_MSM_ACC_LDS");
        uint32_t v = e ? (uint32_t)atoi(e) : 0u;
        if (v && hipFuncSetAttribute((const void *)k_accumulate_chunks, hipFuncAttributeMaxDynamicSharedMemorySize, (int)v) != hipSuccess) v = 0;
        return v;
    }();
    static const uint32_t bg_lds = [] {
        const char *e = getenv("TKMK_MSM_BACKGROUND_LDS");
        uint32_t v = e ? (uint32_t)atoi(e) : 98304u;
        if (v && hipFuncSetAttribute((const void *)k_accumulate_chunks, hipFuncAttributeMaxDynamicSharedMemorySize, (int)v) != hipSuccess) v = 0;
        return v;
    }();
    const uint32_t lds_claim = (tl_background_batch && bg_lds) ? bg_lds : acc_lds;
    prof.mark("msm.prepare");
    hipLaunchKernelGGL(k_accumulate_chunks, tk_div_up((size_t)pl.W * cpw, 256), 256, lds_claim, s, bases_mont, (const uint32_t *)d_sorted.p,
                       (const uint32_t *)d_bstart.p, d_buckets.as<g1_xyzz_t>(), d_fh.as<g1_xyzz_t>(), d_ft.as<g1_xyzz_t>(), pl, cpw);
    prof.mark("msm.accumulate");
    hipLaunchKernelGGL(k_combine, tk_div_up((size_t)pl.W * pl.B, 256), 256, 0, s, (const uint32_t *)d_bstart.p, d_buckets.as<g1_xyzz_t>(),
                       (const g1_xyzz_t *)d_fh.p, (const g1_xyzz_t *)d_ft.p, pl, cpw, d_big.as<uint32_t>(), big_cap, d_giant.as<uint32_t>());
    if ((uint64_t)n > (uint64_t)MSM_GIANT * pl.chunk) {
        hipLaunchKernelGGL(k_combine_giant_parts, 1024, 256, 0, s, (const uint32_t *)d_bstart.p, (const g1_xyzz_t *)d_fh.p,
                           (const g1_xyzz_t *)d_ft.p, pl, cpw, (const uint32_t *)d_giant.p, d_gpart.as<g1_xyzz_t>());
        hipLaunchKernelGGL(k_combine_giant_final, 256, 64, 0, s, d_buckets.as<g1_xyzz_t>(), (const uint32_t *)d_giant.p,
                           (const g1_xyzz_t *)d_gpart.p);
    }
    hipLaunchKernelGGL(k_combine_big, 1024, 256, 0, s, (const uint32_t *)d_bstart.p, d_buckets.as<g1_xyzz_t>(),
                       (const g1_xyzz_t *)d_fh.p, (const g1_xyzz_t *)d_ft.p, pl, cpw, (const uint32_t *)d_big.p, big_cap);
    prof.mark("msm.combine");
    size_t wins_count = (size_t)pl.W * pl.win_parts;
    if (pl.lo_bits) {
        const uint32_t HI = 1u << pl.hi_bits, LO = 1u << pl.lo_bits;
        g1_xyzz_t *rows = d_segs.as<g1_xyzz_t>(), *cols = rows + HI;
        hipLaunchKernelGGL(k_reduce_rows_cols, HI / 4 + LO / 2, 256, 0, s, (const g1_xyzz_t *)d_buckets.p, rows, cols, HI, LO);
        prof.mark("msm.reduce_segments");
        wins_count = 1 + pl.hi_bits + pl.lo_bits;
        hipLaunchKernelGGL(k_reduce_bits, (unsigned)wins_count, 256, 0, s, (const g1_xyzz_t *)rows, (const g1_xyzz_t *)cols, HI, LO, pl.hi_bits,
                           d_wins.as<g1_xyzz_t>());
        prof.mark("msm.reduce_windows");
    } else {
        hipLaunchKernelGGL(k_reduce_segments, tk_div_up((size_t)pl.W * segs, 128), 128, 0, s, (const g1_xyzz_t *)d_buckets.p,
                           d_segs.as<g1_xyzz_t>(), pl, segs);
        prof.mark("msm.reduce_segments");
        hipLaunchKernelGGL(k_reduce_windows, dim3(pl.W, pl.win_parts), 256, 0, s, (const g1_xyzz_t *)d_segs.p, d_wins.as<g1_xyzz_t>(), segs, pl.win_parts);
        prof.mark("msm.reduce_windows");
    }
    TK_HIP(hipGetLastError());
    if (getenv("TKMK_MSM_DEBUG"))
        fprintf(stderr, "[msm debug] ptrs dig=%p sorted=%p counts=%p bstart=%p buckets=%p (+%zu) segs=%p (+%zu) wins=%p\n", d_dig.p,
                d_sorted.p, d_counts.p, d_bstart.p, d_buckets.p, (size_t)pl.W * pl.B * sizeof(g1_xyzz_t), d_segs.p,
                (size_t)pl.W * segs * sizeof(g1_xyzz_t), d_wins.p);
    if (getenv("TKMK_MSM_DEBUG") && factor == 1 && view_is_identity(sv) && view_is_identity(bv) && !level_rows) TK_TRY(msm_debug_check(pl, scalars, bases_mont, d_dig.as<uint32_t>(), d_sorted.as<uint32_t>(),
                                                          d_bstart.as<uint32_t>(), d_buckets.as<g1_xyzz_t>(), s));
    TK_HIP(hipMemcpyAsync(wins_host, d_wins.p, wins_count * sizeof(g1_xyzz_t), hipMemcpyDeviceToHost, s));
    prof.finish();
    *plan_out = pl;
    return TKMK_SUCCESS;
}

static g1_xyzz_t msm_horner(const msm_plan_t &pl, const g1_xyzz_t *wins) {
    if (pl.lo_bits) {
        g1_xyzz_t hi = G1::inf(), lo = G1::inf();
        for (int k = (int)pl.hi_bits - 1; k >= 0; k--) hi = G1::add(G1::dbl(hi), G1U::raw_to_sat(wins[1 + k]));
        for (int k = (int)pl.lo_bits - 1; k >= 0; k--) lo = G1::add(G1::dbl(lo), G1U::raw_to_sat(wins[1 + pl.hi_bits + k]));
        for (uint32_t k = 0; k < pl.lo_bits; k++) hi = G1::dbl(hi);
        return G1::add(G1::add(G1U::raw_to_sat(wins[0]), hi), lo);
    }
    g1_xyzz_t acc = G1::inf();
    for (int w = (int)pl.W - 1; w >= 0; w--) {
        for (uint32_t k = 0; k < pl.c; k++) acc = G1::dbl(acc);
        for (uint32_t part = 0; part < pl.win_parts; part++) acc = G1::add(acc, G1U::raw_to_sat(wins[w * pl.win_parts + part]));
    }
    return acc;
}

static tkmk_error msm_one(const fr_t *scalars, const g1_affine_t *bases_mont, uint32_t n, uint32_t factor, uint32_t c_req, uint32_t bits,
                          bool scalars_mont, hipStream_t s, g1_xyzz_t *result_host) {
    tk_frame frame(s);
    std::vector<g1_xyzz_t> wins_v((size_t)MSM_MAX_WINDOWS * MSM_WIN_PARTS);
    g1_xyzz_t *wins = wins_v.data();
    msm_plan_t pl;
    TK_TRY(msm_enqueue(scalars, bases_mont, n, factor, c_req, bits, scalars_mont, s, wins, &pl));
    TK_HIP(hipStreamSynchronize(s));
    *result_host = msm_horner(pl, wins);
    return TKMK_SUCCESS;
}

struct msm_slot {
    hipStream_t s = nullptr;
    hipEvent_t done = nullptr;
    g1_xyzz_t *wins = nullptr;
    tk_frame *frame = nullptr;
    msm_plan_t pl;
    int job = -1;
};
struct msm_pipe_job {
    const fr_t *scalars;
    const g1_affine_t *bases;
    uint32_t n;
    bool convert, bases_mont;
    uint32_t factor = 1;
    msm_view_t sv = view_identity(), bv = view_identity();
    uint32_t c = 0;
    uint32_t level_rows = 0;
};
struct msm_pipe_set {
    std::mutex mu;
    std::vector<msm_slot> slots;
};
static std::mutex g_pipe_sets_mu;
static std::map<hipStream_t, std::unique_ptr<msm_pipe_set>> g_pipe_sets;
static msm_pipe_set &msm_pipe_set_of(hipStream_t caller) {
    std::lock_guard<std::mutex> lk(g_pipe_sets_mu);
    std::unique_ptr<msm_pipe_set> &p = g_pipe_sets[caller];
    if (!p) p.reset(new msm_pipe_set());
    return *p;
}

void drop_pipe_set(hipStream_t caller) {
    std::unique_ptr<msm_pipe_set> set;
    {
        std::lock_guard<std::mutex> lk(g_pipe_sets_mu);
        auto it = g_pipe_sets.find(caller);
        if (it == g_pipe_sets.end()) return;
        set = std::move(it->second);
        g_pipe_sets.erase(it);
    }
    std::lock_guard<std::mutex> lk(set->mu);
    for (msm_slot &sl : set->slots) {
        (void)hipStreamSynchronize(sl.s);
        (void)hipStreamDestroy(sl.s);
        (void)hipEventDestroy(sl.done);
        (void)hipHostFree(sl.wins);
    }
    set->slots.clear();
}

static tkmk_error msm_pipe_slots(std::vector<msm_slot> &g_slots, uint32_t want) {
    while (g_slots.size() < want) {
        msm_slot sl;
        TK_HIP(hipStreamCreateWithFlags(&sl.s, hipStreamNonBlocking));
        TK_HIP(hipEventCreateWithFlags(&sl.done, hipEventDisableTiming));
        TK_HIP(hipHostMalloc((void **)&sl.wins, (size_t)MSM_MAX_WINDOWS * MSM_WIN_PARTS * sizeof(g1_xyzz_t), hipHostMallocDefault));
        g_slots.push_back(sl);
    }
    return TKMK_SUCCESS;
}

static tkmk_error msm_pipe_finish(msm_slot &sl, g1_xyzz_t *results) {
    if (sl.job < 0) return TKMK_SUCCESS;
    hipError_t e = hipEventSynchronize(sl.done);
    delete sl.frame;
    sl.frame = nullptr;
    int j = sl.job;
    sl.job = -1;
    TK_HIP(e);
    results[j] = msm_horner(sl.pl, sl.wins);
    return TKMK_SUCCESS;
}

static tkmk_error msm_pipeline(const std::vector<msm_pipe_job> &jobs, uint32_t c_req, uint32_t bits, bool scalars_mont,
                               hipStream_t caller, g1_xyzz_t *results) {
    msm_pipe_set &set = msm_pipe_set_of(caller);
    std::lock_guard<std::mutex> lk(set.mu);
    tl_background_batch = tk_stream_is_background(caller);
    std::vector<msm_slot> &g_slots = set.slots;
    const uint32_t n_streams = tk_msm_pipeline_streams();
    const uint32_t K = jobs.size() < n_streams ? (uint32_t)jobs.size() : n_streams;
    TK_TRY(msm_pipe_slots(g_slots, K));
    hipEvent_t ready;
    TK_HIP(hipEventCreateWithFlags(&ready, hipEventDisableTiming));
    TK_HIP(hipEventRecord(ready, caller));
    tkmk_error err = TKMK_SUCCESS;
    for (size_t j = 0; j < jobs.size() && err == TKMK_SUCCESS; j++) {
        msm_slot &sl = g_slots[j % K];
        err = msm_pipe_finish(sl, results);
        if (err != TKMK_SUCCESS) break;
        const msm_pipe_job &jb = jobs[j];
        if (j < K) {
            hipError_t e = hipStreamWaitEvent(sl.s, ready, 0);
            if (e != hipSuccess) { err = TKMK_ERR_UNKNOWN; break; }
        }
        sl.frame = new tk_frame(sl.s);
        sl.job = (int)j;
        const g1_affine_t *bm = jb.bases;
        if (jb.convert) {
            tk_scratch d_bm;
            err = d_bm.alloc((size_t)jb.n * AFF_BYTES, sl.s);
            if (err != TKMK_SUCCESS) break;
            hipLaunchKernelGGL(k_convert_bases, tk_div_up(jb.n, 256), 256, 0, sl.s, jb.bases, d_bm.as<g1_affine_t>(), (uint64_t)jb.n,
                               jb.bases_mont ? 1 : 0, jb.bv);
            bm = d_bm.as<g1_affine_t>();
        }
        err = msm_enqueue(jb.scalars, bm, jb.n, jb.factor, jb.c ? jb.c : c_req, bits, scalars_mont, sl.s, sl.wins, &sl.pl, jb.sv,
                          jb.convert ? view_identity() : jb.bv, jb.convert ? 0u : jb.level_rows);
        if (err != TKMK_SUCCESS) break;
        if (hipEventRecord(sl.done, sl.s) != hipSuccess) err = TKMK_ERR_UNKNOWN;
    }
    {
        std::vector<msm_slot *> live;
        for (auto &sl : g_slots)
            if (sl.job >= 0) live.push_back(&sl);
        std::sort(live.begin(), live.end(), [](msm_slot *a, msm_slot *b) { return a->job < b->job; });
        for (msm_slot *sl : live) {
            if (err != TKMK_SUCCESS) (void)hipStreamSynchronize(sl->s);
            tkmk_error e2 = msm_pipe_finish(*sl, results);
            if (err == TKMK_SUCCESS) err = e2;
        }
    }
    (void)hipEventDestroy(ready);
    return err;
}

TK_API tkmk_error TK_MSM_SYM_MSM(const abi_fr *scalars, const abi_affine *bases, int msm_size, const tkmk_msm_config *cfg,
                                abi_proj *results) {
    if (!cfg || cfg->ext) return TKMK_ERR_INVALID_ARGUMENT;
    if (msm_size < 0 || cfg->batch_size < 1 || cfg->bitsize < 0 || cfg->bitsize > 255 || cfg->c < 0 || cfg->c > MSM_MAX_C ||
        cfg->precompute_factor < 0)
        return TKMK_ERR_INVALID_ARGUMENT;
    if (!results) return TKMK_ERR_INVALID_POINTER;
    TK_TRY(tk_require_device());
    const uint32_t n = (uint32_t)msm_size, batch = (uint32_t)cfg->batch_size;
    const uint32_t bits = cfg->bitsize ? (uint32_t)cfg->bitsize : (uint32_t)TK_MSM_SCALAR_BITS;
    uint32_t factor = cfg->precompute_factor > 1 ? (uint32_t)cfg->precompute_factor : 1u;
    if (factor > 1) {
        if (n < 2) return TKMK_ERR_INVALID_ARGUMENT;
        if (cfg->c && msm_resolve_c((uint32_t)cfg->c, n) != (uint32_t)cfg->c) return TKMK_ERR_INVALID_ARGUMENT;
        const uint32_t w_src = bits / msm_resolve_c((uint32_t)cfg->c, n) + 1;
        if (factor > w_src) factor = w_src;
    }
    hipStream_t s = tk_stream(cfg->stream_handle);
    tk_frame frame(s);
    std::vector<abi_proj> host_res(batch);
    if (n == 0) {
        for (uint32_t b = 0; b < batch; b++) store_canonical(&host_res[b], G1::inf());
    } else {
        if (!scalars || !bases) return TKMK_ERR_INVALID_POINTER;
        const size_t n_bases = (cfg->are_points_shared_in_batch ? (size_t)n : (size_t)n * batch) * factor;
        tk_staged S, P;
        TK_TRY(S.in(scalars, (size_t)n * batch * FR_BYTES, cfg->are_scalars_on_device, s));
        TK_TRY(P.in(bases, n_bases * AFF_BYTES, cfg->are_points_on_device, s));
        if (n == 1) {
            tk_scratch d_out;
            TK_TRY(d_out.alloc((size_t)batch * sizeof(g1_xyzz_t), s));
            hipLaunchKernelGGL(k_msm_size1, tk_div_up(batch, 128), 128, 0, s, (const fr_t *)S.dev, (const g1_affine_t *)P.dev,
                               cfg->are_points_shared_in_batch ? 1 : 0, batch, cfg->are_points_montgomery_form ? 1 : 0,
                               cfg->are_scalars_montgomery_form ? 1 : 0, d_out.as<g1_xyzz_t>());
            TK_HIP(hipGetLastError());
            std::vector<g1_xyzz_t> r(batch);
            TK_HIP(hipMemcpyAsync(r.data(), d_out.p, (size_t)batch * sizeof(g1_xyzz_t), hipMemcpyDeviceToHost, s));
            TK_HIP(hipStreamSynchronize(s));
            for (uint32_t b = 0; b < batch; b++) store_canonical(&host_res[b], r[b]);
        } else if (n <= 64 && factor == 1 && batch <= 4096) {
            tk_scratch d_out;
            TK_TRY(d_out.alloc((size_t)batch * SM_NW * sizeof(g1_xyzz_t), s));
            hipLaunchKernelGGL(k_msm_small, dim3(SM_NW / 4, batch), 256, 0, s, (const fr_t *)S.dev, (const g1_affine_t *)P.dev,
                               cfg->are_points_shared_in_batch ? 1 : 0, n, cfg->are_points_montgomery_form ? 1 : 0,
                               cfg->are_scalars_montgomery_form ? 1 : 0, bits, d_out.as<g1_xyzz_t>());
            TK_HIP(hipGetLastError());
            std::vector<g1_xyzz_t> r((size_t)batch * SM_NW);
            TK_HIP(hipMemcpyAsync(r.data(), d_out.p, r.size() * sizeof(g1_xyzz_t), hipMemcpyDeviceToHost, s));
            TK_HIP(hipStreamSynchronize(s));
            tk_stat_add(TK_STAT_MSM_POINTS, (uint64_t)n * batch);
            tk_stat_add(TK_STAT_MSM_CALLS, batch);
            for (uint32_t b = 0; b < batch; b++) {
                g1_xyzz_t acc = G1::inf();
                for (int w = SM_NW - 1; w >= 0; w--) {
                    for (int k = 0; k < 4; k++) acc = G1::dbl(acc);
                    acc = G1::add(acc, r[(size_t)b * SM_NW + w]);
                }
                store_canonical(&host_res[b], acc);
            }
        } else {
            tk_scratch d_bm;
            const g1_affine_t *bm = (const g1_affine_t *)P.dev;
            if (factor == 1) {
                TK_TRY(d_bm.alloc(n_bases * AFF_BYTES, s));
                tk_prof prof(s);
                hipLaunchKernelGGL(k_convert_bases, tk_div_up(n_bases, 256), 256, 0, s, (const g1_affine_t *)P.dev,
                                   d_bm.as<g1_affine_t>(), (uint64_t)n_bases, cfg->are_points_montgomery_form ? 1 : 0, view_identity());
                prof.mark("msm.convert_bases");
                prof.finish();
                TK_HIP(hipGetLastError());
                bm = d_bm.as<g1_affine_t>();
            }
            if (batch == 1) {
                g1_xyzz_t r;
                TK_TRY(msm_one((const fr_t *)S.dev, bm, n, factor, (uint32_t)cfg->c, bits, cfg->are_scalars_montgomery_form, s, &r));
                store_canonical(&host_res[0], r);
            } else {
                std::vector<msm_pipe_job> jobs(batch);
                for (uint32_t b = 0; b < batch; b++)
                    jobs[b] = {(const fr_t *)S.dev + (size_t)b * n,
                               bm + (cfg->are_points_shared_in_batch ? 0 : (size_t)b * n * factor), n, false, false, factor,
                               view_identity(), view_identity()};
                std::vector<g1_xyzz_t> r(batch);
                TK_TRY(msm_pipeline(jobs, (uint32_t)cfg->c, bits, cfg->are_scalars_montgomery_form, s, r.data()));
                for (uint32_t b = 0; b < batch; b++) store_canonical(&host_res[b], r[b]);
            }
        }
    }
    if (cfg->are_results_on_device) {
        TK_HIP(hipMemcpyAsync(results, host_res.data(), (size_t)batch * sizeof(abi_proj), hipMemcpyHostToDevice, s));
        TK_HIP(hipStreamSynchronize(s));
    } else {
        for (uint32_t b = 0; b < batch; b++) results[b] = host_res[b];
    }
    return TKMK_SUCCESS;
}

TK_API tkmk_error TK_MSM_SYM_MULTI(const abi_job *jobs, int n_jobs, const tkmk_msm_config *cfg, abi_proj *results) {
    if (!cfg || cfg->ext || cfg->batch_size != 1 || n_jobs < 0) return TKMK_ERR_INVALID_ARGUMENT;
    const uint32_t factor = cfg->precompute_factor > 1 ? (uint32_t)cfg->precompute_factor : 1u;
    if (cfg->bitsize < 0 || cfg->bitsize > 255 || cfg->c < 0 || cfg->c > MSM_MAX_C) return TKMK_ERR_INVALID_ARGUMENT;
    if (n_jobs == 0) return TKMK_SUCCESS;
    if (!jobs || !results) return TKMK_ERR_INVALID_POINTER;
    TK_TRY(tk_require_device());
    const uint32_t bits = cfg->bitsize ? (uint32_t)cfg->bitsize : (uint32_t)TK_MSM_SCALAR_BITS;
    hipStream_t s = tk_stream(cfg->stream_handle);
    tk_frame frame(s);
    std::vector<abi_proj> host_res(n_jobs);
    std::vector<msm_pipe_job> pj;
    std::vector<int> pj_index;
    std::vector<tk_staged> staged((size_t)n_jobs * 2);
    for (int j = 0; j < n_jobs; j++) {
        if (jobs[j].msm_size < 0) return TKMK_ERR_INVALID_ARGUMENT;
        if (jobs[j].msm_size > 0 && (!jobs[j].scalars || !jobs[j].bases)) return TKMK_ERR_INVALID_POINTER;
    }
    for (int j = 0; j < n_jobs; j++) {
        const uint32_t n = (uint32_t)jobs[j].msm_size;
        if (n < 2) {
            if (factor > 1 && n == 1) return TKMK_ERR_INVALID_ARGUMENT;
            tkmk_msm_config c1 = *cfg;
            c1.are_results_on_device = false;
            c1.precompute_factor = 1;
            TK_TRY(TK_MSM_SYM_MSM(jobs[j].scalars, jobs[j].bases, (int)n, &c1, &host_res[j]));
            continue;
        }
        tk_staged &S = staged[2 * j], &P = staged[2 * j + 1];
        TK_TRY(S.in(jobs[j].scalars, (size_t)n * FR_BYTES, cfg->are_scalars_on_device, s));
        uint32_t f = factor;
        if (f > 1) {
            const uint32_t w_src = bits / msm_resolve_c((uint32_t)cfg->c, n) + 1;
            if (f > w_src) f = w_src;
        }
        TK_TRY(P.in(jobs[j].bases, (size_t)n * f * AFF_BYTES, cfg->are_points_on_device, s));
        pj.push_back({(const fr_t *)S.dev, (const g1_affine_t *)P.dev, n, f == 1, cfg->are_points_montgomery_form, f, view_identity(),
                      view_identity()});
        pj_index.push_back(j);
    }
    if (!pj.empty()) {
        std::vector<g1_xyzz_t> r(pj.size());
        TK_TRY(msm_pipeline(pj, (uint32_t)cfg->c, bits, cfg->are_scalars_montgomery_form, s, r.data()));
        for (size_t k = 0; k < pj.size(); k++) store_canonical(&host_res[pj_index[k]], r[k]);
    }
    if (cfg->are_results_on_device) {
        TK_HIP(hipMemcpyAsync(results, host_res.data(), (size_t)n_jobs * sizeof(abi_proj), hipMemcpyHostToDevice, s));
        TK_HIP(hipStreamSynchronize(s));
    } else {
        for (int j = 0; j < n_jobs; j++) results[j] = host_res[j];
    }
    return TKMK_SUCCESS;
}

#ifdef TK_MSM_SYM_MULTI_EX
static tkmk_error msm_ex_tiny(const abi_job_ex &jb, const tkmk_msm_config *cfg, int bases_form, abi_proj *out) {
    if (jb.msm_size == 0) {
        store_canonical(out, G1::inf());
        return TKMK_SUCCESS;
    }
    uint32_t bi = 0;
    if (jb.base_index) TK_HIP(hipMemcpy(&bi, jb.base_index, 4, hipMemcpyDeviceToHost));
    if (jb.base_table_len && bi >= jb.base_table_len) return TKMK_ERR_INVALID_ARGUMENT;
    fr_t sc;
    g1_affine_t pt;
    TK_HIP(hipMemcpy(&sc, jb.scalars, sizeof sc, hipMemcpyDeviceToHost));
    TK_HIP(hipMemcpy(&pt, (const g1_affine_t *)jb.bases + bi, sizeof pt, hipMemcpyDeviceToHost));
    tkmk_msm_config c1 = *cfg;
    c1.are_scalars_on_device = c1.are_points_on_device = c1.are_results_on_device = false;
    c1.precompute_factor = 1;
    c1.are_points_montgomery_form = bases_form == TKMK_BASES_MONTGOMERY;
    if (bases_form == TKMK_BASES_CONVERTED && !G1::is_inf(pt)) {
        fq_t rp;
        for (int j = 0; j < Fq::N; j++) rp.l[j] = FqP::KSATM[j];
        fq_t rinv = Fq::inv(Fq::to_mont(rp));
        pt.x = Fq::mul(pt.x, rinv);
        pt.y = Fq::mul(pt.y, rinv);
    }
    return TK_MSM_SYM_MSM((const abi_fr *)&sc, (const abi_affine *)&pt, 1, &c1, out);
}

TK_API tkmk_error TK_MSM_SYM_MULTI_EX(const abi_job_ex *jobs, int n_jobs, const tkmk_msm_config *cfg, int bases_form, abi_proj *results) {
    if (!cfg || cfg->ext || cfg->batch_size != 1 || n_jobs < 0 || cfg->precompute_factor > 1) return TKMK_ERR_INVALID_ARGUMENT;
    if (bases_form != TKMK_BASES_PLAIN && bases_form != TKMK_BASES_MONTGOMERY && bases_form != TKMK_BASES_CONVERTED) return TKMK_ERR_INVALID_ARGUMENT;
    if (cfg->bitsize < 0 || cfg->bitsize > 255 || cfg->c < 0 || cfg->c > MSM_MAX_C) return TKMK_ERR_INVALID_ARGUMENT;
    if (!cfg->are_scalars_on_device || !cfg->are_points_on_device) return TKMK_ERR_INVALID_ARGUMENT;
    if (n_jobs == 0) return TKMK_SUCCESS;
    if (!jobs || !results) return TKMK_ERR_INVALID_POINTER;
    TK_TRY(tk_require_device());
    const uint32_t bits = cfg->bitsize ? (uint32_t)cfg->bitsize : (uint32_t)TK_MSM_SCALAR_BITS;
    hipStream_t s = tk_stream(cfg->stream_handle);
    tk_frame frame(s);
    for (int j = 0; j < n_jobs; j++) {
        const abi_job_ex &jb = jobs[j];
        if (jb.msm_size < 0) return TKMK_ERR_INVALID_ARGUMENT;
        if (jb.msm_size > 0 && (!jb.scalars || !jb.bases)) return TKMK_ERR_INVALID_POINTER;
        if ((jb.scalar_cols && jb.scalar_stride < jb.scalar_cols) || (jb.base_cols && jb.base_stride < jb.base_cols)) return TKMK_ERR_INVALID_ARGUMENT;
        if (jb.msm_size > 0 && jb.base_cols && !jb.base_index && jb.base_table_len) {
            uint64_t last = (uint64_t)((uint32_t)jb.msm_size - 1) / jb.base_cols * jb.base_stride + ((uint32_t)jb.msm_size - 1) % jb.base_cols;
            if (last >= jb.base_table_len) return TKMK_ERR_INVALID_ARGUMENT;
        }
        if (jb.base_table_len >= (1ull << 31)) return TKMK_ERR_INVALID_ARGUMENT;
        if (jb.msm_size > 0 && jb.base_index && !jb.base_table_len) return TKMK_ERR_INVALID_ARGUMENT;
        if ((jb.table_c != 0) != (jb.table_factor != 0)) return TKMK_ERR_INVALID_ARGUMENT;
        if (jb.table_factor > 1) {
            if (bases_form != TKMK_BASES_CONVERTED || !jb.base_table_len || jb.table_c < 2 || jb.table_c > MSM_MAX_C) return TKMK_ERR_INVALID_ARGUMENT;
            if (jb.base_table_len * jb.table_factor >= (1ull << 31)) return TKMK_ERR_INVALID_ARGUMENT;
            if (jb.table_c > 16 && (uint64_t)jb.msm_size * jb.table_factor < (1ull << 18)) return TKMK_ERR_INVALID_ARGUMENT;
        }
    }
    tk_scratch d_flag;
    TK_TRY(d_flag.alloc(4, s));
    TK_HIP(hipMemsetAsync(d_flag.p, 0, 4, s));
    std::vector<abi_proj> host_res(n_jobs);
    std::vector<msm_pipe_job> pj;
    std::vector<int> pj_index;
    for (int j = 0; j < n_jobs; j++) {
        const abi_job_ex &jb = jobs[j];
        if (jb.msm_size < 2) {
            TK_TRY(msm_ex_tiny(jb, cfg, bases_form, &host_res[j]));
            continue;
        }
        msm_view_t sv{nullptr, jb.scalar_cols, jb.scalar_stride, 0, nullptr};
        msm_view_t bv{jb.base_index, jb.base_index ? 0u : jb.base_cols, jb.base_index ? 0u : jb.base_stride,
                      jb.base_index ? (uint32_t)jb.base_table_len : 0u, d_flag.as<uint32_t>()};
        msm_pipe_job pjob{(const fr_t *)jb.scalars, (const g1_affine_t *)jb.bases, (uint32_t)jb.msm_size, bases_form != TKMK_BASES_CONVERTED,
                          bases_form == TKMK_BASES_MONTGOMERY, 1u, sv, bv};
        if (jb.table_factor > 1) {
            pjob.factor = jb.table_factor;
            pjob.c = jb.table_c;
            pjob.level_rows = (uint32_t)jb.base_table_len;
        }
        pj.push_back(pjob);
        pj_index.push_back(j);
    }
    if (!pj.empty()) {
        std::vector<g1_xyzz_t> r(pj.size());
        TK_TRY(msm_pipeline(pj, (uint32_t)cfg->c, bits, cfg->are_scalars_montgomery_form, s, r.data()));
        uint32_t flag = 0;
        TK_HIP(hipMemcpyAsync(&flag, d_flag.p, 4, hipMemcpyDeviceToHost, s));
        TK_HIP(hipStreamSynchronize(s));
        if (flag) return TKMK_ERR_INVALID_ARGUMENT;
        for (size_t k = 0; k < pj.size(); k++) store_canonical(&host_res[pj_index[k]], r[k]);
    }
    if (cfg->are_results_on_device) {
        TK_HIP(hipMemcpyAsync(results, host_res.data(), (size_t)n_jobs * sizeof(abi_proj), hipMemcpyHostToDevice, s));
        TK_HIP(hipStreamSynchronize(s));
    } else {
        for (int j = 0; j < n_jobs; j++) results[j] = host_res[j];
    }
    return TKMK_SUCCESS;
}

TK_API tkmk_error TK_MSM_SYM_CONVERT(const abi_affine *bases, uint64_t n, const tkmk_msm_config *cfg, abi_affine *out) {
    if (!cfg || cfg->ext) return TKMK_ERR_INVALID_ARGUMENT;
    if (n == 0) return TKMK_SUCCESS;
    if (!bases || !out) return TKMK_ERR_INVALID_POINTER;
    if (n >= (1ull << 32)) return TKMK_ERR_INVALID_ARGUMENT;
    TK_TRY(tk_require_device());
    hipStream_t s = tk_stream(cfg->stream_handle);
    tk_frame frame(s);
    tk_staged P, O;
    TK_TRY(P.in(bases, (size_t)n * AFF_BYTES, cfg->are_points_on_device, s));
    TK_TRY(O.out(out, (size_t)n * AFF_BYTES, cfg->are_results_on_device, s));
    hipLaunchKernelGGL(k_convert_bases, tk_div_up(n, 256), 256, 0, s, (const g1_affine_t *)P.dev, (g1_affine_t *)O.dev, n,
                       cfg->are_points_montgomery_form ? 1 : 0, view_identity());
    TK_HIP(hipGetLastError());
    TK_TRY(O.copy_back(out, (size_t)n * AFF_BYTES, cfg->are_results_on_device, s));
    TK_HIP(hipStreamSynchronize(s));
    return TKMK_SUCCESS;
}
#endif

TK_API tkmk_error TK_MSM_SYM_PRECOMPUTE(const abi_affine *bases, int n_points, const tkmk_msm_config *cfg, abi_affine *output_bases) {
    if (!cfg || cfg->ext || n_points < 2 || cfg->bitsize < 0 || cfg->bitsize > 255 || cfg->c < 0 || cfg->c > MSM_MAX_C ||
        cfg->precompute_factor < 1)
        return TKMK_ERR_INVALID_ARGUMENT;
    if (!bases || !output_bases) return TKMK_ERR_INVALID_POINTER;
    TK_TRY(tk_require_device());
    const uint32_t n = (uint32_t)n_points;
    const uint32_t bits = cfg->bitsize ? (uint32_t)cfg->bitsize : (uint32_t)TK_MSM_SCALAR_BITS;
    const uint32_t c = cfg->c ? (uint32_t)cfg->c : msm_resolve_c(0, n);
    const uint32_t w_src = bits / c + 1;
    uint32_t factor = (uint32_t)cfg->precompute_factor;
    if (factor > w_src) factor = w_src;
    if ((uint64_t)n * factor >= (1ull << 31)) return TKMK_ERR_INVALID_ARGUMENT;
    const uint32_t wg = (w_src + factor - 1) / factor;
    hipStream_t s = tk_stream(cfg->stream_handle);
    tk_frame frame(s);
    tk_staged P, O;
    TK_TRY(P.in(bases, (size_t)n * AFF_BYTES, cfg->are_points_on_device, s));
    TK_TRY(O.out(output_bases, (size_t)n * factor * AFF_BYTES, cfg->are_results_on_device, s));
    hipLaunchKernelGGL(k_precompute_bases, tk_div_up(n, 128), 128, 0, s, (const g1_affine_t *)P.dev, (g1_affine_t *)O.dev, (uint64_t)n,
                       cfg->are_points_montgomery_form ? 1 : 0, factor, c * wg);
    TK_HIP(hipGetLastError());
    TK_TRY(O.copy_back(output_bases, (size_t)n * factor * AFF_BYTES, cfg->are_results_on_device, s));
    TK_HIP(hipStreamSynchronize(s));
    return TKMK_SUCCESS;
}

}
```

tokamak-zk-evm_amd/host/tkmk_host.hpp:

```cpp
#pragma once
#include "tkmk_base.hpp"
#include "tkmk_fr.hpp"

namespace tkmk {

template <class T>
class DeviceVec {
    T *p_ = nullptr;
    size_t n_ = 0;

  public:
    DeviceVec() = default;
    explicit DeviceVec(size_t n) : n_(n) { check(tkmk_malloc((void **)&p_, n * sizeof(T)), "DeviceVec::device_malloc"); }
    DeviceVec(const DeviceVec &) = delete;
    DeviceVec &operator=(const DeviceVec &) = delete;
    DeviceVec(DeviceVec &&o) noexcept : p_(o.p_), n_(o.n_) { o.p_ = nullptr, o.n_ = 0; }
    DeviceVec &operator=(DeviceVec &&o) noexcept {
        if (this != &o) {
            if (p_) tkmk_free(p_);
            p_ = o.p_, n_ = o.n_, o.p_ = nullptr, o.n_ = 0;
        }
        return *this;
    }
    ~DeviceVec() {
// ... 717 lines not shown
  private:
    explicit PolyExpr(Kind k) : kind(k) {}
    static PolyExpr binary(Kind k, PolyExpr l, PolyExpr r) {
        PolyExpr e{k};
        e.kids.push_back(std::move(l));
        e.kids.push_back(std::move(r));
        return e;
    }
    static std::shared_ptr<DeviceVec<ScalarField>> leaf_evals(const DensePolynomialExt *leaf, size_t xs, size_t ys, LeafCache &cache) {
        auto key = std::make_tuple(leaf, xs, ys);
        auto it = cache.find(key);
        if (it == cache.end()) {
            it = cache.emplace(key, std::make_shared<DeviceVec<ScalarField>>(leaf->evals_on(xs, ys))).first;
        }
        return it->second;
    }
    struct Program {
        std::vector<tkmk_expr_instr> code;
        struct Leaf {
            const DensePolynomialExt *p;
            size_t ord_x, ord_y;
        };
        std::vector<Leaf> leaves;
        std::vector<ScalarField> consts;
        uint8_t leaf_index(const DensePolynomialExt *p, size_t ord_x, size_t ord_y) {
            for (size_t i = 0; i < leaves.size(); i++)
                if (leaves[i].p == p && leaves[i].ord_x == ord_x && leaves[i].ord_y == ord_y) return (uint8_t)i;
            leaves.push_back({p, ord_x, ord_y});
            return (uint8_t)(leaves.size() - 1);
        }
        uint8_t const_index(const ScalarField &c) {
            for (size_t i = 0; i < consts.size(); i++)
                if (fr_eq(consts[i], c)) return (uint8_t)i;
            consts.push_back(c);
            return (uint8_t)(consts.size() - 1);
        }
    };
    int compile(Program &pg, int depth) const {
        if (pg.leaves.size() > 200 || pg.consts.size() > 200 || pg.code.size() > 1000) return -1;
        switch (kind) {
            case Poly: pg.code.push_back({TKMK_EXPR_LEAF, pg.leaf_index(leaf, shift_ord_x, shift_ord_y)}); return 1;
            case Scalar: pg.code.push_back({TKMK_EXPR_CONST, pg.const_index(scalar_)}); return 1;
            case Add:
            case Sub:
            case Mul: {
                int l = kids[0].compile(pg, depth);
                if (l < 0) return -1;
                int r = kids[1].compile(pg, depth + 1);
                if (r < 0) return -1;
                pg.code.push_back({(uint8_t)(kind == Add ? TKMK_EXPR_ADD : kind == Sub ? TKMK_EXPR_SUB : TKMK_EXPR_MUL), 0});
                return std::max(l, 1 + r);
            }
            case Scale: {
                int d = kids[0].compile(pg, depth);
                if (d < 0) return -1;
                pg.code.push_back({TKMK_EXPR_SCALE, pg.const_index(scalar_)});
                return d;
            }
            case MulXMinusOne: {
                int d = kids[0].compile(pg, depth);
                if (d < 0) return -1;
                pg.code.push_back({TKMK_EXPR_MUL_X_MINUS_ONE, 0});
                return d;
            }
            default: {
                if (kids.empty()) {
                    pg.code.push_back({TKMK_EXPR_CONST, pg.const_index(ScalarField{})});
                    return 1;
                }
                int need = 0;
                for (size_t i = 0; i < kids.size(); i++) {
                    int d = kids[i].compile(pg, depth + (i ? 1 : 0));
                    if (d < 0) return -1;
                    need = std::max(need, d + (i ? 1 : 0));
                    if (i) pg.code.push_back({TKMK_EXPR_ADD, 0});
                }
                return need;
            }
        }
    }
    DeviceVec<ScalarField> on_domain(size_t xs, size_t ys, LeafCache &cache) const {
        size_t n = xs * ys;
        tkmk_vecops_config c = dev_cfg();
        switch (kind) {
            case Poly: {
                if (!shift_ord_x && !shift_ord_y) return leaf_evals(leaf, xs, ys, cache)->clone();
                auto inv_root = [](size_t ord) {
                    ScalarField w;
                    check(bls12_381_get_root_of_unity(ord, &w), "get_root_of_unity");
                    ScalarField wi;
                    tkmk_vecops_config hc = tkmk_vecops_default_config();
                    check(bls12_381_vector_inv(&w, 1, &hc, &wi), "vector_inv");
                    return wi;
                };
                ScalarField wx = shift_ord_x ? inv_root(shift_ord_x) : fr_from_u32(1), wy = shift_ord_y ? inv_root(shift_ord_y) : fr_from_u32(1);
                return leaf->scale_coeffs(shift_ord_x ? &wx : nullptr, shift_ord_y ? &wy : nullptr).evals_on(xs, ys);
            }
            case Scalar: {
                std::vector<ScalarField> v(n, scalar_);
                return DeviceVec<ScalarField>::from_host(v);
            }
            case Add:
            case Sub:
            case Mul: {
                DeviceVec<ScalarField> l = kids[0].on_domain(xs, ys, cache), r = kids[1].on_domain(xs, ys, cache);
                auto fn = kind == Add ? bls12_381_vector_add : kind == Sub ? bls12_381_vector_sub : bls12_381_vector_mul;
                check(fn(l.ptr(), r.ptr(), n, &c, l.ptr()), "fused pointwise");
                return l;
            }
            case Scale: {
                DeviceVec<ScalarField> e = kids[0].on_domain(xs, ys, cache);
                if (fr_eq(scalar_, fr_from_u32(1))) return e;
                c.is_a_on_device = false;
                check(bls12_381_scalar_mul_vec(&scalar_, e.ptr(), n, &c, e.ptr()), "fused scale");
                return e;
            }
            case MulXMinusOne: {
                DeviceVec<ScalarField> e = kids[0].on_domain(xs, ys, cache);
                check(tkmk_poly_mul_x_minus_one_evals(e.ptr(), (uint32_t)xs, (uint32_t)ys, e.ptr(), nullptr), "fused x-1");
                return e;
            }
            default: {
                std::vector<ScalarField> z(n);
                DeviceVec<ScalarField> acc = DeviceVec<ScalarField>::from_host(z);
                for (auto &k : kids) {
                    DeviceVec<ScalarField> t = k.on_domain(xs, ys, cache);
                    check(bls12_381_vector_add(acc.ptr(), t.ptr(), n, &c, acc.ptr()), "fused sum");
                }
                return acc;
            }
        }
    }
};

struct CommitBox {
    std::string name;
    size_t x, y;
    const char *basis;
};
inline std::vector<CommitBox> *&commit_box_sink() {
    static thread_local std::vector<CommitBox> *sink = nullptr;
    return sink;
}

struct CommitComm {
    void *comm = nullptr;
    tkmk_error (*multi_ex_sharded)(void *comm, const tkmk_msm_job_ex *jobs, int n_jobs, const tkmk_msm_config *cfg, int bases_form, tkmk_g1_projective *results) = nullptr;
};
inline CommitComm &commit_comm() {
    static thread_local CommitComm c;
    return c;
}

class Sigma1 {
    DeviceVec<G1Affine> xy_powers_;
    size_t rs_x_, rs_y_;
    uint32_t table_c_ = 0, table_factor_ = 0;
    Shard shard_;
    size_t local_cols_;

  public:
    Sigma1(DeviceVec<G1Affine> &&xy_powers, size_t rs_x_size, size_t rs_y_size, uint32_t table_c = 0, Shard shard = Shard{})
        : xy_powers_(std::move(xy_powers)), rs_x_(rs_x_size), rs_y_(rs_y_size), shard_(shard), local_cols_(shard.cols_of(rs_y_size)) {
        if (shard_.world < 1 || shard_.rank >= shard_.world) throw Error("Sigma1: invalid shard");
        if (xy_powers_.len() != rs_x_ * local_cols_) throw Error("xy_powers has the wrong length");
        tkmk_msm_config cfg = tkmk_msm_default_config();
        cfg.are_points_on_device = cfg.are_results_on_device = true;
        if (table_c >= 2 && xy_powers_.len() >= 2) {
            const uint32_t windows = 255 / table_c + 1;
            if ((uint64_t)xy_powers_.len() * windows >= (1ull << 31)) throw Error("xy_powers is too large for a precomputed table");
            DeviceVec<G1Affine> table(xy_powers_.len() * windows);
            cfg.c = (int)table_c;
            cfg.precompute_factor = (int)windows;
            check(bls12_381_msm_precompute_bases(xy_powers_.ptr(), (int)xy_powers_.len(), &cfg, table.ptr()), "msm::precompute_bases");
            xy_powers_ = std::move(table);
            table_c_ = table_c, table_factor_ = windows;
        } else {
            check(bls12_381_msm_convert_bases(xy_powers_.ptr(), xy_powers_.len(), &cfg, xy_powers_.ptr()), "msm::convert_bases");
        }
    }
    size_t rs_x() const { return rs_x_; }
    size_t rs_y() const { return rs_y_; }
    size_t table_len() const { return rs_x_ * local_cols_; }
    size_t local_cols() const { return local_cols_; }
    const G1Affine *level0() const { return xy_powers_.ptr(); }
    const Shard &shard() const { return shard_; }
    static DeviceVec<G1Affine> cols_of_grid(const DeviceVec<G1Affine> &grid, size_t rs_x, size_t rs_y, Shard shard) {
        if (grid.len() != rs_x * rs_y) throw Error("cols_of_grid: the grid has the wrong length");
        if (rs_y % shard.world) throw Error("cols_of_grid: the grid's width is not a multiple of the number of ranks");
        const size_t lc = rs_y / shard.world;
        DeviceVec<G1Affine> out(rs_x * lc);
        if (out.len())
            check(tkmk_memcpy_2d_d2d(out.ptr(), sizeof(G1Affine), grid.ptr() + shard.rank, (size_t)shard.world * sizeof(G1Affine), sizeof(G1Affine), rs_x * lc), "cols_of_grid");
        return out;
    }
    static DeviceVec<G1Affine> rows_of_grid(const DeviceVec<G1Affine> &grid, size_t rs_x, size_t rs_y, Shard shard) {
        if (grid.len() != rs_x * rs_y) throw Error("rows_of_grid: the grid has the wrong length");
        const size_t rows = shard.rows_of(rs_x);
        DeviceVec<G1Affine> out(rows * rs_y);
        if (rows)
            check(tkmk_memcpy_2d_d2d(out.ptr(), rs_y * sizeof(G1Affine), grid.ptr() + (size_t)shard.rank * rs_y, (size_t)shard.world * rs_y * sizeof(G1Affine),
                                     rs_y * sizeof(G1Affine), rows),
                  "rows_of_grid");
        return out;
    }
    uint32_t table_c() const { return table_c_; }
    tkmk_msm_job_ex job(DensePolynomialExt &poly, const char *name = nullptr) const {
        const auto deg = commit_box_sink() ? poly.find_degree() : poly.shape_degree();
        size_t tx = (size_t)(deg.first + 1), ty = (size_t)(deg.second + 1);
        if (deg.first < 0 || deg.second < 0) tx = ty = 0;
        if (tx > rs_x_ || ty > rs_y_) throw Error("Insufficient length of sigma.sigma_1.xy_powers");
        if (auto *sink = commit_box_sink()) sink->push_back({name ? name : "?", tx, ty, "coeff"});
        const size_t mine = shard_.cols_of(ty);
        const ScalarField *scalars = poly.poly.ptr();
        size_t scalar_stride = poly.ly();
        if (shard_.world > 1 && poly.rep) {
            DensePolynomialExt d = poly.to_distributed();
            scalar_stride = d.ly();
            poly.commit_slice_ = std::move(d.poly);
            scalars = poly.commit_slice_.ptr();
        }
        tkmk_msm_job_ex j{};
        j.scalars = scalars;
        j.bases = xy_powers_.ptr();
        j.msm_size = (int)(tx * mine);
        j.scalar_cols = (uint32_t)mine, j.scalar_stride = (uint32_t)scalar_stride;
        j.base_cols = (uint32_t)mine, j.base_stride = (uint32_t)local_cols_;
        j.base_index = nullptr;
        j.base_table_len = table_len();
        if (table_c_ && (uint64_t)tx * mine * table_factor_ >= (1ull << 20)) j.table_c = table_c_, j.table_factor = table_factor_;
        return j;
    }
    static G1Affine to_affine(const tkmk_g1_projective &res) {
        G1Affine out{};
        bool inf = true;
        for (uint32_t l : res.z.limbs) inf &= l == 0;
        if (!inf) out.x = res.x, out.y = res.y;
        return out;
    }
    static tkmk_msm_config device_cfg() {
        tkmk_msm_config cfg = tkmk_msm_default_config();
        cfg.are_scalars_on_device = cfg.are_points_on_device = true;
        return cfg;
    }
    static std::vector<G1Affine> run_jobs(const std::vector<tkmk_msm_job_ex> &jobs, tkmk_stream stream = nullptr) {
        tkmk_msm_config cfg = device_cfg();
        cfg.stream_handle = stream;
        std::vector<tkmk_g1_projective> res(jobs.size());
        if (host_trace_on()) {
            std::string d;
            for (auto &j : jobs) d += " " + std::to_string(j.msm_size) + (j.table_c ? "t" : "") + (j.base_index ? "i" : "");
            host_trace("commit batch of %zu:%s", jobs.size(), d.c_str());
        }
        const CommitComm &cc = commit_comm();
        if (cc.comm) check(cc.multi_ex_sharded(cc.comm, jobs.data(), (int)jobs.size(), &cfg, TKMK_BASES_CONVERTED, res.data()), "tkmk_msm_multi_ex_sharded");
        else check(tkmk_msm_multi_ex(jobs.data(), (int)jobs.size(), &cfg, TKMK_BASES_CONVERTED, res.data()), "tkmk_msm_multi_ex");
        std::vector<G1Affine> out;
        for (auto &r : res) out.push_back(to_affine(r));
        return out;
    }
    G1Affine encode_poly(DensePolynomialExt &poly, const char *name = nullptr) const { return run_jobs({job(poly, name)})[0]; }
    tkmk_msm_job_ex job_evals(const DeviceVec<ScalarField> &evals, const char *name = nullptr, size_t whole_x = 0, size_t whole_y = 0) const {
        if (shard_.world != 1) throw Error("job_evals: a Lagrange-basis table is built over the rank's own part of the grid");
        if (evals.len() < rs_x_ * rs_y_) throw Error("evaluation vector shorter than the Lagrange table");
        if (auto *sink = commit_box_sink()) sink->push_back({name ? name : "?", whole_x ? whole_x : rs_x_, whole_y ? whole_y : rs_y_, "evals"});
        tkmk_msm_job_ex j{};
        j.scalars = evals.ptr();
        j.bases = xy_powers_.ptr();
        j.msm_size = (int)(rs_x_ * rs_y_);
        j.base_table_len = table_len();
        if (table_c_ && (uint64_t)rs_x_ * rs_y_ * table_factor_ >= (1ull << 20)) j.table_c = table_c_, j.table_factor = table_factor_;
        return j;
    }
    static ScalarField inverse_of_grid_size(size_t xs, size_t ys) { return fr_inv(fr_mul(fr_from_u32((uint32_t)xs), fr_from_u32((uint32_t)ys))); }
    DeviceVec<G1Affine> lagrange_points(size_t xs, size_t ys) const {
        if (shard_.world != 1) throw Error("Lagrange table: needs the whole grid (build it before the rows are sharded)");
        if (xs > rs_x_ || ys > rs_y_ || !is_pow2(xs) || !is_pow2(ys)) throw Error("Lagrange table: the grid must be a power-of-two corner of xy_powers");
        DeviceVec<G1Affine> lam(xs * ys);
        host_trace("lagrange_points %zu x %zu", xs, ys);
        check(tkmk_g1_ntt(xy_powers_.ptr(), TKMK_BASES_CONVERTED, (uint32_t)rs_y_, (uint32_t)xs, (uint32_t)ys, TKMK_NTT_INVERSE, lam.ptr(), nullptr), "tkmk_g1_ntt");
        const ScalarField inv_n = inverse_of_grid_size(xs, ys);
        check(tkmk_g1_scale(lam.ptr(), xs * ys, &inv_n, lam.ptr(), nullptr), "tkmk_g1_scale");
        return lam;
    }
    Sigma1 lagrange_of(size_t xs, size_t ys) const { return Sigma1(lagrange_points(xs, ys), xs, ys, table_c_); }
    static DeviceVec<G1Affine> lagrange_prefix_points(const DeviceVec<G1Affine> &lagrange, size_t xs, size_t ys) {
        DeviceVec<G1Affine> pre(xs * ys);
        host_trace("lagrange_prefix_of %zu x %zu", xs, ys);
        check(tkmk_g1_prefix_sums(lagrange.ptr(), TKMK_BASES_PLAIN, (uint32_t)xs, (uint32_t)ys, 1, pre.ptr(), nullptr), "tkmk_g1_prefix_sums");
        return pre;
    }
    Sigma1 lagrange_prefix_of(const DeviceVec<G1Affine> &lagrange, size_t xs, size_t ys) const {
        return Sigma1(lagrange_prefix_points(lagrange, xs, ys), xs * ys, 1, table_c_);
    }
    std::vector<G1Affine> encode_polys(const std::vector<DensePolynomialExt *> &polys, const std::vector<const char *> &names = {}) const {
        std::vector<tkmk_msm_job_ex> jobs;
        for (size_t k = 0; k < polys.size(); k++) jobs.push_back(job(*polys[k], k < names.size() ? names[k] : nullptr));
        return run_jobs(jobs);
    }
};

}
```

tokamak-zk-evm_amd/tkmk/__init__.py:

```python
import ctypes
import os

import numpy as np

os.environ.setdefault("GPU_MAX_HW_QUEUES", "8")

_PKG = os.path.dirname(os.path.dirname(os.path.abspath(__file__)))
LIB_PATH = os.environ.get("TKMK_HIP_LIBRARY") or os.path.join(_PKG, "libtkmk_hip.so")
_lib = None


class TkmkError(RuntimeError):
    def __init__(self, code, where):
        self.code = code
        msg = lib().tkmk_error_string(code).decode() if _lib is not None else str(code)
        super().__init__("%s failed: %s (tkmk_error %d)" % (where, msg, code))


class Fr(ctypes.Structure):
    _fields_ = [("limbs", ctypes.c_uint32 * 8)]


class MSMConfig(ctypes.Structure):
    _fields_ = [
        ("stream_handle", ctypes.c_void_p),
        ("precompute_factor", ctypes.c_int),
        ("c", ctypes.c_int),
        ("bitsize", ctypes.c_int),
        ("batch_size", ctypes.c_int),
        ("are_points_shared_in_batch", ctypes.c_bool),
        ("are_scalars_on_device", ctypes.c_bool),
        ("are_scalars_montgomery_form", ctypes.c_bool),
        ("are_points_on_device", ctypes.c_bool),
        ("are_points_montgomery_form", ctypes.c_bool),
        ("are_results_on_device", ctypes.c_bool),
        ("is_async", ctypes.c_bool),
        ("ext", ctypes.c_void_p),
    ]


class NTTConfig(ctypes.Structure):
    _fields_ = [
        ("stream_handle", ctypes.c_void_p),
        ("coset_gen", Fr),
        ("batch_size", ctypes.c_int),
        ("columns_batch", ctypes.c_bool),
        ("ordering", ctypes.c_int),
        ("are_inputs_on_device", ctypes.c_bool),
        ("are_outputs_on_device", ctypes.c_bool),
        ("is_async", ctypes.c_bool),
        ("ext", ctypes.c_void_p),
    ]


class NTTInitDomainConfig(ctypes.Structure):
    _fields_ = [("stream_handle", ctypes.c_void_p), ("is_async", ctypes.c_bool), ("ext", ctypes.c_void_p)]


class VecOpsConfig(ctypes.Structure):
    _fields_ = [
        ("stream_handle", ctypes.c_void_p),
        ("is_a_on_device", ctypes.c_bool),
        ("is_b_on_device", ctypes.c_bool),
        ("is_result_on_device", ctypes.c_bool),
        ("is_async", ctypes.c_bool),
        ("batch_size", ctypes.c_int),
        ("columns_batch", ctypes.c_bool),
        ("ext", ctypes.c_void_p),
    ]


SYMBOLS = [
    "tkmk_device_count", "tkmk_set_device", "tkmk_get_available_memory", "tkmk_malloc", "tkmk_malloc_async", "tkmk_free",
    "tkmk_free_async", "tkmk_memcpy_h2d", "tkmk_memcpy_d2h", "tkmk_memcpy_d2d", "tkmk_memcpy_h2d_async",
    "tkmk_memcpy_d2h_async", "tkmk_memcpy_2d_d2d", "tkmk_memset", "tkmk_stream_create", "tkmk_stream_synchronize", "tkmk_stream_destroy", "tkmk_stream_set_background",
    "tkmk_device_synchronize", "tkmk_release_scratch", "tkmk_error_string", "tkmk_is_hip_build", "tkmk_keccak256", "tkmk_r1cs_index", "tkmk_msm_default_config", "bls12_381_msm", "bls12_381_g2_msm", "tkmk_g1_ntt", "tkmk_g1_ntt_axes", "tkmk_g1_prefix_sums", "tkmk_g1_scale", "bls12_381_msm_precompute_bases", "bn254_msm_precompute_bases", "tkmk_msm_multi", "bn254_msm", "tkmk_bn254_msm_multi", "bn254_get_root_of_unity", "bn254_ntt_init_domain", "bn254_ntt_release_domain",
    "bn254_ntt", "tkmk_bn254_bintt", "tkmk_bn254_fr_random_device",
    "tkmk_bn254_g1_batch_scalar_mul_device",
    "tkmk_ntt_default_config", "bls12_381_get_root_of_unity", "bls12_381_ntt_init_domain", "bls12_381_ntt_release_domain",
    "bls12_381_ntt", "tkmk_bintt", "tkmk_vecops_default_config", "bls12_381_vector_add", "bls12_381_vector_sub",
    "bls12_381_vector_mul", "bls12_381_vector_div", "bls12_381_vector_inv", "bls12_381_scalar_add_vec",
    "bls12_381_scalar_sub_vec", "bls12_381_scalar_mul_vec", "bls12_381_vector_sum", "bls12_381_vector_product",
    "bls12_381_matrix_transpose", "tkmk_vec_suffix_product", "tkmk_fr_random_device", "tkmk_gather_rows_device", "tkmk_g1_batch_scalar_mul_device", "tkmk_profile_enable",
    "tkmk_profile_reset", "tkmk_profile_get", "tkmk_diag_bench", "tkmk_diag_field_mul", "tkmk_poly_find_degree",
    "tkmk_poly_place", "tkmk_poly_scale_coeffs", "tkmk_poly_mul_x_minus_one_evals", "tkmk_poly_mul_ones_x", "tkmk_poly_expr_eval", "tkmk_poly_expr_eval_views", "tkmk_poly_expr_eval_views_slab", "tkmk_poly_eval_x", "tkmk_poly_eval_y", "tkmk_poly_eval",
    "tkmk_poly_div_by_vanishing_opt", "tkmk_poly_div_by_ruffini", "tkmk_r1cs_eval_rows",
    "tkmk_msm_multi_ex", "bls12_381_msm_convert_bases", "tkmk_r1cs_library_create", "tkmk_r1cs_library_destroy", "tkmk_r1cs_library_eval",
    "tkmk_witness_route", "tkmk_fr_scatter_table", "tkmk_msm_set_pipeline_streams", "tkmk_msm_get_pipeline_streams", "tkmk_host_malloc", "tkmk_host_free", "tkmk_stats_reset", "tkmk_stats_get",
    "bls12_381_ntt_domain_size", "bn254_ntt_domain_size", "tkmk_poly_lincomb", "tkmk_bintt_padded", "tkmk_diag_device_switch", "tkmk_diag_gather_probe",
    "bls12_381_generate_random_affine_points", "bls12_381_generate_scalars", "bls12_381_polynomial_add", "bls12_381_polynomial_clone", "bls12_381_polynomial_coeffs_device_ptr", "bls12_381_polynomial_copy_coeffs", "bls12_381_polynomial_create_from_coefficients", "bls12_381_polynomial_create_from_rou_evaluations", "bls12_381_polynomial_degree", "bls12_381_polynomial_delete", "bls12_381_polynomial_divide", "bls12_381_polynomial_evaluate", "bls12_381_polynomial_get_coeff", "bls12_381_polynomial_multiply", "bls12_381_polynomial_multiply_by_scalar", "bls12_381_polynomial_nof_coeffs", "bls12_381_polynomial_slice", "bls12_381_polynomial_subtract", "bls12_381_vector_accumulate",
]


def lib():
    global _lib
    if _lib is None:
        if not os.path.exists(LIB_PATH):
            raise ImportError("libtkmk_hip.so is not built (run __graft_entry__.build()); there is no CPU fallback")
        _lib = ctypes.CDLL(LIB_PATH)
        _lib.tkmk_error_string.restype = ctypes.c_char_p
        _lib.tkmk_msm_default_config.restype = MSMConfig
        _lib.tkmk_ntt_default_config.restype = NTTConfig
        _lib.tkmk_vecops_default_config.restype = VecOpsConfig
    return _lib


def _check(code, where):
    if code != 0:
        raise TkmkError(code, where)


def _p(a):
    if a is None:
        return None
    if isinstance(a, DeviceBuffer):
        return ctypes.c_void_p(a.ptr)
    assert a.dtype == np.uint8 and a.flags["C_CONTIGUOUS"]
    return a.ctypes.data_as(ctypes.c_void_p)


def _on_dev(a):
    return isinstance(a, DeviceBuffer)


def _fr_struct(buf32):
    f = Fr()
    ctypes.memmove(ctypes.byref(f), buf32.ctypes.data, 32)
    return f


def _out_like(a, nbytes, out):
    if out is not None:
        return out
    if _on_dev(a):
        return DeviceBuffer(nbytes)
    return np.empty(nbytes, np.uint8)


class DeviceBuffer:

    def __init__(self, nbytes):
        p = ctypes.c_void_p()
        _check(lib().tkmk_malloc(ctypes.byref(p), ctypes.c_size_t(nbytes)), "tkmk_malloc")
        self.ptr = p.value
        self.nbytes = nbytes

    @classmethod
    def from_host(cls, arr):
        d = cls(arr.size)
        _check(lib().tkmk_memcpy_h2d(ctypes.c_void_p(d.ptr), _p(arr), ctypes.c_size_t(arr.size)), "tkmk_memcpy_h2d")
        return d

    def to_host(self, nbytes=None, offset=0):
        n = self.nbytes - offset if nbytes is None else nbytes
        out = np.empty(n, np.uint8)
        _check(lib().tkmk_memcpy_d2h(_p(out), ctypes.c_void_p(self.ptr + offset), ctypes.c_size_t(n)), "tkmk_memcpy_d2h")
        return out

    def free(self):
        if self.ptr:
            lib().tkmk_free(ctypes.c_void_p(self.ptr))
            self.ptr = 0

    def __del__(self):
        try:
            self.free()
        except Exception:
            pass


def device_count():
    n = ctypes.c_int()
    _check(lib().tkmk_device_count(ctypes.byref(n)), "tkmk_device_count")
    return n.value


def set_device(i):
    _check(lib().tkmk_set_device(int(i)), "tkmk_set_device")


def synchronize():
    _check(lib().tkmk_device_synchronize(), "tkmk_device_synchronize")


def available_memory():
    t, f = ctypes.c_size_t(), ctypes.c_size_t()
    _check(lib().tkmk_get_available_memory(ctypes.byref(t), ctypes.byref(f)), "tkmk_get_available_memory")
    return t.value, f.value


_NTT_SYMS = {
    "bls12_381": ("bls12_381_get_root_of_unity", "bls12_381_ntt_init_domain", "bls12_381_ntt_release_domain", "bls12_381_ntt", "tkmk_bintt"),
    "bn254": ("bn254_get_root_of_unity", "bn254_ntt_init_domain", "bn254_ntt_release_domain", "bn254_ntt", "tkmk_bn254_bintt"),
}


def get_root_of_unity(max_size, curve="bls12_381"):
    sym = _NTT_SYMS[curve][0]
    out = np.empty(32, np.uint8)
    _check(getattr(lib(), sym)(ctypes.c_uint64(max_size), _p(out)), sym)
    return out


_domain_size = {}


def init_ntt_domain_for_size(size, curve="bls12_381"):
    if size <= 0 or size & (size - 1):
        raise ValueError("NTT domain size must be a non-zero power of two")
    have = ntt_domain_size(curve)
    if have >= size:
        return
    if have:
        release_ntt_domain(curve)
    root = get_root_of_unity(size, curve)
    cfg = NTTInitDomainConfig(None, False, None)
    sym = _NTT_SYMS[curve][1]
    _check(getattr(lib(), sym)(_p(root), ctypes.byref(cfg)), sym)
    _domain_size[curve] = size


def ntt_domain_size(curve="bls12_381"):
    v = ctypes.c_uint64()
    sym = "bls12_381_ntt_domain_size" if curve == "bls12_381" else "bn254_ntt_domain_size"
    _check(getattr(lib(), sym)(ctypes.byref(v)), sym)
    return v.value


def bintt_padded(a, in_x, in_y, x_size, y_size, coset_x=None, coset_y=None, out=None):
# ... 4 lines not shown
    return out


def release_ntt_domain(curve="bls12_381"):
    sym = _NTT_SYMS[curve][2]
    _check(getattr(lib(), sym)(), sym)
    _domain_size.pop(curve, None)


STATS = {"msm_points": 0, "ntt_elements": 0}


def stats_reset():
    STATS["msm_points"] = STATS["ntt_elements"] = 0


def ntt(a, n, batch=1, columns_batch=False, inverse=False, coset_gen=None, out=None, stream=None, curve="bls12_381"):
    STATS["ntt_elements"] += int(n) * int(batch)
    cfg = lib().tkmk_ntt_default_config()
    cfg.batch_size = batch
    cfg.columns_batch = columns_batch
    if coset_gen is not None:
        cfg.coset_gen = _fr_struct(coset_gen)
    cfg.stream_handle = stream
    out = _out_like(a, 32 * n * batch, out)
    cfg.are_inputs_on_device = _on_dev(a)
    cfg.are_outputs_on_device = _on_dev(out)
    sym = _NTT_SYMS[curve][3]
    _check(getattr(lib(), sym)(_p(a), int(n), 1 if inverse else 0, ctypes.byref(cfg), _p(out)), sym)
    return out


def bintt(a, x_size, y_size, inverse=False, coset_x=None, coset_y=None, out=None, stream=None, curve="bls12_381"):
    STATS["ntt_elements"] += int(x_size) * int(y_size)
    out = _out_like(a, 32 * x_size * y_size, out)
    if _on_dev(a) != _on_dev(out):
        raise ValueError("tkmk_bintt takes both buffers on the same side")
    sym = _NTT_SYMS[curve][4]
    _check(getattr(lib(), sym)(_p(a), ctypes.c_size_t(x_size), ctypes.c_size_t(y_size), 1 if inverse else 0, _p(coset_x),
                               _p(coset_y), _on_dev(a), ctypes.c_void_p(stream), _p(out)), sym)
    return out


def _vec(name, a, b, n, out, batch=1, columns_batch=False, out_elems=None):
    cfg = lib().tkmk_vecops_default_config()
    cfg.is_a_on_device = _on_dev(a)
    cfg.is_b_on_device = _on_dev(b) if b is not None else False
    cfg.batch_size = batch
    cfg.columns_batch = columns_batch
    nbytes = 32 * (out_elems if out_elems is not None else n * batch)
    if out is None:
        out = DeviceBuffer(nbytes) if (_on_dev(a) or _on_dev(b)) else np.empty(nbytes, np.uint8)
    cfg.is_result_on_device = _on_dev(out)
    fn = getattr(lib(), name)
    if b is None:
        _check(fn(_p(a), ctypes.c_uint64(n), ctypes.byref(cfg), _p(out)), name)
    else:
        _check(fn(_p(a), _p(b), ctypes.c_uint64(n), ctypes.byref(cfg), _p(out)), name)
    return out


def vec_add(a, b, out=None):
    return _vec("bls12_381_vector_add", a, b, _len(a), out)


def vec_sub(a, b, out=None):
    return _vec("bls12_381_vector_sub", a, b, _len(a), out)


def vec_mul(a, b, out=None):
    return _vec("bls12_381_vector_mul", a, b, _len(a), out)


def vec_div(a, b, out=None):
    return _vec("bls12_381_vector_div", a, b, _len(a), out)


def vec_inv(a, out=None):
    return _vec("bls12_381_vector_inv", a, None, _len(a), out)


def scalar_add(s, v, out=None):
    return _vec("bls12_381_scalar_add_vec", s, v, _len(v), out)


def scalar_sub(s, v, out=None):
    return _vec("bls12_381_scalar_sub_vec", s, v, _len(v), out)


def scalar_mul(s, v, out=None):
    return _vec("bls12_381_scalar_mul_vec", s, v, _len(v), out)


def vec_sum(a, n=None, batch=1, columns_batch=False):
    n = _len(a) // batch if n is None else n
    return _vec("bls12_381_vector_sum", a, None, n, None, batch, columns_batch, out_elems=batch)


def vec_product(a, n=None, batch=1, columns_batch=False):
    n = _len(a) // batch if n is None else n
    return _vec("bls12_381_vector_product", a, None, n, None, batch, columns_batch, out_elems=batch)


def transpose(a, rows, cols, out=None):
    cfg = lib().tkmk_vecops_default_config()
    cfg.is_a_on_device = _on_dev(a)
    out = _out_like(a, 32 * rows * cols, out)
    cfg.is_result_on_device = _on_dev(out)
    _check(lib().bls12_381_matrix_transpose(_p(a), ctypes.c_uint32(rows), ctypes.c_uint32(cols), ctypes.byref(cfg), _p(out)),
           "bls12_381_matrix_transpose")
    return out


def _len(a):
    return (a.nbytes if _on_dev(a) else a.size) // 32


_CURVES = {
    "bls12_381": ("bls12_381_msm", "tkmk_msm_multi", "tkmk_fr_random_device", "tkmk_g1_batch_scalar_mul_device", 96,
                  "bls12_381_msm_precompute_bases"),
    "bn254": ("bn254_msm", "tkmk_bn254_msm_multi", "tkmk_bn254_fr_random_device", "tkmk_bn254_g1_batch_scalar_mul_device", 64,
              "bn254_msm_precompute_bases"),
}


def msm_windows(n, c=0, bitsize=0, curve="bls12_381", explicit_c=False):
    bits = bitsize or (255 if curve == "bls12_381" else 254)
    if not c:
        best, cost = 2, None
        for cc in range(2, 17):
            v = (255 // cc + 1) * (n + 4.0 * (1 << (cc - 1)))
            if cost is None or v < cost:
                best, cost = cc, v
        c = best
    if explicit_c:
        return bits // min(max(c, 2), 20) + 1
    c = min(max(c, 2), 20)
    if c > 16 and n < (1 << 18):
        c = 16
    return bits // c + 1


def msm_precompute_bases(bases, n, factor, c=0, bitsize=0, curve="bls12_381", points_montgomery=False):
    sym, aff = _CURVES[curve][5], _CURVES[curve][4]
    cfg = lib().tkmk_msm_default_config()
    cfg.precompute_factor = factor
    cfg.c, cfg.bitsize = c, bitsize
    cfg.are_points_on_device = _on_dev(bases)
    cfg.are_points_montgomery_form = points_montgomery
    cfg.are_results_on_device = True
    f = min(factor, msm_windows(n, c, bitsize, curve, explicit_c=bool(c)))
    out = DeviceBuffer(aff * n * f)
    _check(getattr(lib(), sym)(_p(bases), int(n), ctypes.byref(cfg), _p(out)), sym)
    return out


def msm(scalars, bases, msm_size=None, batch=1, shared_points=True, c=0, bitsize=0, stream=None, curve="bls12_381",
        precompute_factor=1, scalars_montgomery=False, points_montgomery=False):
    sym, aff = _CURVES[curve][0], _CURVES[curve][4]
    cfg = lib().tkmk_msm_default_config()
    n = _len(scalars) // batch if msm_size is None else msm_size
    STATS["msm_points"] += int(n) * int(batch)
    cfg.batch_size = batch
    cfg.are_points_shared_in_batch = shared_points
    cfg.are_scalars_on_device = _on_dev(scalars)
    cfg.are_points_on_device = _on_dev(bases)
    cfg.c = c
    cfg.bitsize = bitsize
    cfg.stream_handle = stream
    cfg.precompute_factor = precompute_factor
    cfg.are_scalars_montgomery_form = scalars_montgomery
    cfg.are_points_montgomery_form = points_montgomery
    out = np.empty(aff // 2 * 3 * batch, np.uint8)
    _check(getattr(lib(), sym)(_p(scalars), _p(bases), int(n), ctypes.byref(cfg), _p(out)), sym)
    return out


G1_NTT_AXIS_X, G1_NTT_AXIS_Y = 1, 2


def g1_ntt(points, x_size, y_size, inverse=False, bases_form=0, in_stride=None, out=None, axes=None):
    out = DeviceBuffer(96 * x_size * y_size) if out is None else out
    stride = ctypes.c_uint32(in_stride if in_stride is not None else y_size)
    if axes is None:
        _check(lib().tkmk_g1_ntt(_p(points), int(bases_form), stride, ctypes.c_uint32(x_size), ctypes.c_uint32(y_size), int(1 if inverse else 0), _p(out), None), "tkmk_g1_ntt")
    else:
        _check(lib().tkmk_g1_ntt_axes(_p(points), int(bases_form), stride, ctypes.c_uint32(x_size), ctypes.c_uint32(y_size), int(1 if inverse else 0), int(axes), _p(out),
                                      None), "tkmk_g1_ntt_axes")
    return out


def g1_prefix_sums(points, rows, cols, transposed=False, bases_form=0, out=None):
    out = DeviceBuffer(96 * rows * cols) if out is None else out
    _check(lib().tkmk_g1_prefix_sums(_p(points), int(bases_form), ctypes.c_uint32(rows), ctypes.c_uint32(cols), int(bool(transposed)), _p(out), None),
           "tkmk_g1_prefix_sums")
    return out


def g1_scale(points, n, scalar, out=None):
    out = DeviceBuffer(96 * n) if out is None else out
    sc = np.ascontiguousarray(np.frombuffer(bytes(scalar), np.uint8))
    _check(lib().tkmk_g1_scale(_p(points), ctypes.c_uint64(n), _p(sc), _p(out), None), "tkmk_g1_scale")
    return out


def msm_g2(scalars, bases, msm_size=None, batch=1, shared_points=True, c=0, bitsize=0, stream=None, scalars_montgomery=False,
           points_montgomery=False):
    cfg = lib().tkmk_msm_default_config()
    n = _len(scalars) // batch if msm_size is None else msm_size
    cfg.batch_size = batch
    cfg.are_points_shared_in_batch = shared_points
    cfg.are_scalars_on_device = _on_dev(scalars)
    cfg.are_points_on_device = _on_dev(bases)
    cfg.c = c
    cfg.bitsize = bitsize
    cfg.stream_handle = stream
    cfg.are_scalars_montgomery_form = scalars_montgomery
    cfg.are_points_montgomery_form = points_montgomery
    out = np.empty(288 * batch, np.uint8)
    _check(lib().bls12_381_g2_msm(_p(scalars), _p(bases), int(n), ctypes.byref(cfg), _p(out)), "bls12_381_g2_msm")
    return out


class MsmJob(ctypes.Structure):
    _fields_ = [("scalars", ctypes.c_void_p), ("bases", ctypes.c_void_p), ("msm_size", ctypes.c_int)]


def msm_multi(jobs, c=0, bitsize=0, stream=None, curve="bls12_381", precompute_factor=1):
    sym, aff = _CURVES[curve][1], _CURVES[curve][4]
    cfg = lib().tkmk_msm_default_config()
    cfg.precompute_factor = precompute_factor
    if not jobs:
        return np.empty(0, np.uint8)
    on_dev_s = {_on_dev(j[0]) for j in jobs}
    on_dev_p = {_on_dev(j[1]) for j in jobs}
    if len(on_dev_s) != 1 or len(on_dev_p) != 1:
        raise ValueError("msm_multi: every job's scalars (and every job's bases) must live on the same side")
    cfg.are_scalars_on_device = on_dev_s.pop()
    cfg.are_points_on_device = on_dev_p.pop()
    cfg.c = c
    cfg.bitsize = bitsize
    cfg.stream_handle = stream
    arr = (MsmJob * len(jobs))()
    for k, j in enumerate(jobs):
        n = j[2] if len(j) > 2 else _len(j[0])
        STATS["msm_points"] += int(n)
        arr[k] = MsmJob(_p(j[0]).value, _p(j[1]).value, int(n))
    out = np.empty(aff // 2 * 3 * len(jobs), np.uint8)
    _check(getattr(lib(), sym)(arr, len(jobs), ctypes.byref(cfg), _p(out)), sym)
    return out


class MsmJobEx(ctypes.Structure):
    _fields_ = [("scalars", ctypes.c_void_p), ("bases", ctypes.c_void_p), ("msm_size", ctypes.c_int),
                ("scalar_cols", ctypes.c_uint32), ("scalar_stride", ctypes.c_uint32), ("base_cols", ctypes.c_uint32),
                ("base_stride", ctypes.c_uint32), ("base_index", ctypes.c_void_p), ("base_table_len", ctypes.c_uint64),
                ("table_c", ctypes.c_uint32), ("table_factor", ctypes.c_uint32)]


BASES_PLAIN, BASES_MONTGOMERY, BASES_CONVERTED = 0, 1, 2


def msm_convert_bases(bases, n=None, points_montgomery=False, out=None):
    n = _len(bases) * 32 // 96 if n is None else n
    cfg = lib().tkmk_msm_default_config()
    cfg.are_points_on_device = _on_dev(bases)
    cfg.are_points_montgomery_form = points_montgomery
    cfg.are_results_on_device = True
    out = DeviceBuffer(96 * n) if out is None else out
    _check(lib().bls12_381_msm_convert_bases(_p(bases), ctypes.c_uint64(n), ctypes.byref(cfg), _p(out)), "bls12_381_msm_convert_bases")
    return out


def msm_job_ex_array(jobs):
    arr = (MsmJobEx * max(len(jobs), 1))()
    for k, j in enumerate(jobs):
        sv, bv, ix = j.get("scalar_view") or (0, 0), j.get("base_view") or (0, 0), j.get("base_index")
        STATS["msm_points"] += int(j["n"])
        tc, tf = j.get("table", (0, 0))
        arr[k] = MsmJobEx(_p(j["scalars"]).value + int(j.get("scalar_offset", 0)), _p(j["bases"]).value + int(j.get("base_offset", 0)), int(j["n"]),
                          sv[0], sv[1], bv[0], bv[1], None if ix is None else _p(ix).value, int(j.get("table_len", 0)), int(tc), int(tf))
    return arr


def msm_multi_ex(jobs, bases_form=BASES_PLAIN, c=0, bitsize=0, stream=None):
    cfg = lib().tkmk_msm_default_config()
    cfg.are_scalars_on_device = cfg.are_points_on_device = True
    cfg.c, cfg.bitsize, cfg.stream_handle = c, bitsize, stream
    if not jobs:
        return np.empty(0, np.uint8)
    arr = msm_job_ex_array(jobs)
    out = np.empty(144 * len(jobs), np.uint8)
    _check(lib().tkmk_msm_multi_ex(arr, len(jobs), ctypes.byref(cfg), int(bases_form), _p(out)), "tkmk_msm_multi_ex")
    return out


def projective_to_affine_bytes(proj, curve="bls12_381"):
    aff = _CURVES[curve][4]
    pb = aff // 2 * 3
    out = []
    for i in range(0, proj.size, pb):
        z = proj[i + aff:i + pb]
        out.append(np.zeros(aff, np.uint8) if not z.any() else proj[i:i + aff].copy())
    return np.concatenate(out)


def fr_random_device(seed, n, first=0, out=None, curve="bls12_381"):
    sym = _CURVES[curve][2]
    out = DeviceBuffer(32 * n) if out is None else out
    _check(getattr(lib(), sym)(ctypes.c_uint64(seed), ctypes.c_uint64(first), ctypes.c_uint64(n), _p(out), None), sym)
    return out


def g1_batch_scalar_mul_device(scalars_dev, base_host, n, out=None, curve="bls12_381"):
    sym, aff = _CURVES[curve][3], _CURVES[curve][4]
    out = DeviceBuffer(aff * n) if out is None else out
    _check(getattr(lib(), sym)(_p(scalars_dev), _p(base_host), ctypes.c_uint64(n), _p(out), None), sym)
    return out


def diag_bench(kind, iters, blocks, reps=3):
    ms = ctypes.c_float()
    _check(lib().tkmk_diag_bench(int(kind), ctypes.c_uint32(iters), ctypes.c_uint32(blocks), int(reps), ctypes.byref(ms)),
           "tkmk_diag_bench")
    return ms.value


def profile_enable(on=True):
    _check(lib().tkmk_profile_enable(1 if on else 0), "tkmk_profile_enable")


def profile_reset():
    _check(lib().tkmk_profile_reset(), "tkmk_profile_reset")


def msm_set_pipeline_streams(n):
    _check(lib().tkmk_msm_set_pipeline_streams(int(n)), "tkmk_msm_set_pipeline_streams")


def msm_get_pipeline_streams():
    return int(lib().tkmk_msm_get_pipeline_streams())


def profile_get(name):
    ms, cnt = ctypes.c_double(), ctypes.c_int()
    _check(lib().tkmk_profile_get(name.encode(), ctypes.byref(ms), ctypes.byref(cnt)), "tkmk_profile_get")
    return ms.value, cnt.value


def poly_lincomb(terms, out_xs, out_ys):
    n = len(terms)
    coeffs = np.ascontiguousarray(np.concatenate([np.asarray(t[0], np.uint8).reshape(32) for t in terms])) if n else np.zeros(32, np.uint8)
    ptrs = (ctypes.c_void_p * max(n, 1))(*[_p(t[1]).value for t in terms])
    arr = lambda k, d: (ctypes.c_uint32 * max(n, 1))(*[(t[k] if len(t) > k else d) for t in terms])
    out = DeviceBuffer(32 * out_xs * out_ys)
    _check(lib().tkmk_poly_lincomb(n, _p(coeffs), ptrs, arr(2, 1), arr(3, 1), arr(4, 0), arr(5, 0), _p(out), int(out_xs), int(out_ys), None),
           "tkmk_poly_lincomb")
    return out


def native_stats_reset():
    _check(lib().tkmk_stats_reset(), "tkmk_stats_reset")


def native_stats():
    out = {}
    for name in ("msm.points", "msm.calls", "msm.bucket_additions", "ntt.elements", "ntt.calls", "poly.elements"):
        v = ctypes.c_uint64()
        _check(lib().tkmk_stats_get(name.encode(), ctypes.byref(v)), "tkmk_stats_get")
        out[name] = v.value
    return out


def diag_field_mul(field, a, b):
    width = 32 if field == 0 else 48
    da, db = DeviceBuffer.from_host(a), DeviceBuffer.from_host(b)
    do = DeviceBuffer(a.size)
    _check(lib().tkmk_diag_field_mul(int(field), _p(da), _p(db), _p(do), ctypes.c_uint64(a.size // width)), "tkmk_diag_field_mul")
    return do.to_host()


def gather_rows_device(src, row_bytes, idx, out=None):
    if not isinstance(idx, DeviceBuffer):
        idx = DeviceBuffer.from_host(np.ascontiguousarray(idx, dtype=np.uint32).view(np.uint8))
    n = idx.nbytes // 4
    out = DeviceBuffer(row_bytes * n) if out is None else out
    _check(lib().tkmk_gather_rows_device(_p(src), ctypes.c_uint32(row_bytes), _p(idx), ctypes.c_uint64(n), _p(out), None),
           "tkmk_gather_rows_device")
    return out


class ExprInstr(ctypes.Structure):
    _fields_ = [("op", ctypes.c_uint8), ("arg", ctypes.c_uint8)]


def poly_expr_eval(prog, leaves, consts, n_consts, x_size, y_size, out=None):
    arr = (ExprInstr * len(prog))(*[ExprInstr(int(o), int(a)) for o, a in prog])
    ptrs = (ctypes.c_void_p * max(1, len(leaves)))(*[b.ptr for b in leaves])
    out = DeviceBuffer(32 * x_size * y_size) if out is None else out
    _check(lib().tkmk_poly_expr_eval(arr, ctypes.c_uint32(len(prog)), ptrs, ctypes.c_uint32(len(leaves)), _p(consts),
                                     ctypes.c_uint32(n_consts), ctypes.c_uint32(x_size), ctypes.c_uint32(y_size), _p(out), None),
           "tkmk_poly_expr_eval")
    return out


def poly_mul_ones_x(p, x_size, y_size, m, scale, out_x_size, out=None):
    out = DeviceBuffer(32 * out_x_size * y_size) if out is None else out
    _check(lib().tkmk_poly_mul_ones_x(_p(p), ctypes.c_uint32(x_size), ctypes.c_uint32(y_size), ctypes.c_uint32(m), _p(scale),
                                      ctypes.c_uint32(out_x_size), _p(out), None), "tkmk_poly_mul_ones_x")
    return out


class ExprLeaf(ctypes.Structure):
# ... 34 lines not shown
```

Before: 20.78 million.

## Store precomputed MSM bases as 128-byte accumulate-ready rows with branchless negation

Adds a new precomputed-base table format in which each affine point takes one aligned 128-byte row, with the infinity flag encoded inside the row, and a matching accumulate kernel that reads these rows. Point negation is folded into the mixed addition through a sign mask rather than a separate branch and neg call. The goal is fewer split cache lines on the random base gathers and less divergence in bucket accumulation. In exchange the table grows from 96 to 128 bytes per point, and the host now keeps both the converted powers and the new table in device memory.

```diff
diff --git a/include/tkmk.h b/include/tkmk.h
--- a/include/tkmk.h
+++ b/include/tkmk.h
@@ -96,6 +96,7 @@
 #define TKMK_BASES_PLAIN 0
 #define TKMK_BASES_MONTGOMERY 1
 #define TKMK_BASES_CONVERTED 2
+#define TKMK_BASES_ACC_READY 3
 typedef struct {
     const tkmk_fr *scalars;
     const tkmk_g1_affine *bases;
@@ -109,6 +110,7 @@
 tkmk_error tkmk_msm_multi_ex(const tkmk_msm_job_ex *jobs, int n_jobs, const tkmk_msm_config *cfg, int bases_form,
                              tkmk_g1_projective *results);
 tkmk_error bls12_381_msm_convert_bases(const tkmk_g1_affine *bases, uint64_t n, const tkmk_msm_config *cfg, tkmk_g1_affine *out);
+tkmk_error bls12_381_msm_precompute_bases_acc(const tkmk_g1_affine *bases, uint64_t n, const tkmk_msm_config *cfg, void *out, uint64_t *out_bytes);
 
 typedef enum { TKMK_NTT_FORWARD = 0, TKMK_NTT_INVERSE = 1 } tkmk_ntt_dir;
 typedef enum { TKMK_ORDER_NN = 0 } tkmk_ntt_ordering;
diff --git a/tokamak-zk-evm_amd/csrc/ec_u.h b/tokamak-zk-evm_amd/csrc/ec_u.h
--- a/tokamak-zk-evm_amd/csrc/ec_u.h
+++ b/tokamak-zk-evm_amd/csrc/ec_u.h
@@ -1,4 +1,6 @@
 #pragma once
+#include <type_traits>
+
 #include "ec.h"
 #include "ffu.h"
 
@@ -48,6 +50,38 @@
         r.y = t;
         return r;
     }
+    static FF_HD A neg_masked(const A &q, uint32_t m) {
+        A n = neg(q), r;
+        r.x = q.x;
+#pragma unroll
+        for (int i = 0; i < FU::L; i++) r.y.l[i] = (q.y.l[i] & ~m) | (n.y.l[i] & m);
+        return r;
+    }
+
+    struct alignas(128) Row {
+        uint32_t w[32];
+    };
+    static_assert(2 * FS::N <= 32, "row does not fit its line");
+    static constexpr uint32_t ROW_INF = 0xffffffffu;
+    static FF_HD Row to_row(const affine_t<FS> &rec) {
+        Row r;
+#pragma unroll
+        for (int i = 0; i < 32; i++) r.w[i] = 0;
+#pragma unroll
+        for (int i = 0; i < FS::N; i++) r.w[i] = rec.x.l[i], r.w[FS::N + i] = rec.y.l[i];
+        if (FS::is_zero(rec.x) && FS::is_zero(rec.y)) r.w[FS::N - 1] = ROW_INF;
+        return r;
+    }
+    static FF_HD void to_record(affine_t<FS> &r, const affine_t<FS> &a) { r = a; }
+    static FF_HD void to_record(Row &r, const affine_t<FS> &a) { r = to_row(a); }
+    static FF_HD bool load_row(A &q, const Row &r) {
+        typename FS::E x, y;
+#pragma unroll
+        for (int i = 0; i < FS::N; i++) x.l[i] = r.w[i], y.l[i] = r.w[FS::N + i];
+        q.x = FU::from_packed(x);
+        q.y = FU::from_packed(y);
+        return r.w[FS::N - 1] != ROW_INF;
+    }
     static FF_HD X from_affine(const A &q) {
         X r;
         r.x = q.x;
@@ -175,6 +209,27 @@
         r.zzz = FU::mul(p.zzz, ppp);
         return r;
     }
+    static FF_HD X add_mixed_signed(const X &p, const A &q, bool negate) { return add_mixed_masked(p, q, 0u - (uint32_t)negate); }
+    static FF_HD X add_mixed_masked(const X &p, const A &q, uint32_t m) {
+        if (p.inf) return from_affine(neg_masked(q, m));
+        E u2 = FU::mul(q.x, p.zz);
+        E s2 = FU::mul(q.y, p.zzz);
+        E pd = FU::template sub<8>(u2, p.x);
+        if (FU::maybe_multiple_of_p(pd, 9)) return add_mixed_slow(p, neg_masked(q, m));
+        E rd = FU::sub2_signed(s2, p.y, m);
+        E pp = FU::sqr(pd);
+        E ppp = FU::mul(pd, pp);
+        E qq = FU::mul(p.x, pp);
+        X r;
+        r.inf = false;
+        E t = FU::add_dbl(ppp, qq);
+        r.x = FU::template sub<4>(FU::sqr(rd), t);
+        E d = FU::template sub<8>(qq, r.x);
+        r.y = FU::template mul_add<true>(rd, d, FU::neg2_unswept(p.y), ppp);
+        r.zz = FU::mul(p.zz, pp);
+        r.zzz = FU::mul(p.zzz, ppp);
+        return r;
+    }
 };
 
 using G1U = ecu<bls12_381_fq_params>;
diff --git a/tokamak-zk-evm_amd/csrc/ffu.h b/tokamak-zk-evm_amd/csrc/ffu.h
--- a/tokamak-zk-evm_amd/csrc/ffu.h
+++ b/tokamak-zk-evm_amd/csrc/ffu.h
@@ -78,6 +78,25 @@
         }
         return norm(t);
     }
+    static FF_HD E neg2_unswept(const E &b) {
+        FFU_ASSERT(strict(b) && below(b, 2));
+        E t;
+#pragma unroll
+        for (int i = 0; i < L; i++) t.l[i] = P::SUB2[i] - b.l[i];
+        return t;
+    }
+    static FF_HD E sub2_signed(const E &a, const E &b, uint32_t m) {
+        FFU_ASSERT(m == 0u || m == ~0u);
+        FFU_ASSERT(strict(a) && strict(b) && below(b, 2) && below(a, 2));
+        E t;
+#pragma unroll
+        for (int i = 0; i < L; i++) {
+            const uint32_t c = P::SUB2[i];
+            FFU_ASSERT(c >= b.l[i] && c >= a.l[i]);
+            t.l[i] = ((a.l[i] ^ m) + ((c + 1u) & m)) + (c - b.l[i]);
+        }
+        return norm(t);
+    }
 
     static FF_HD E mul(const E &a, const E &b) {
         FFU_ASSERT(strict(a) && strict(b) && a.l[L - 1] <= MASK && b.l[L - 1] <= MASK);
@@ -107,10 +126,16 @@
         r.l[L - 1] = (uint32_t)acc;
         return r;
     }
+    template <bool C_UNSWEPT = false>
     static FF_HD E mul_add(const E &a, const E &b, const E &c, const E &d) {
-        static_assert(3 * L < (1 << (64 - 2 * (int)W)), "column accumulator would overflow");
-        FFU_ASSERT(strict(a) && strict(b) && strict(c) && strict(d));
-        FFU_ASSERT(a.l[L - 1] <= MASK && b.l[L - 1] <= MASK && c.l[L - 1] <= MASK && d.l[L - 1] <= MASK);
+        static_assert((C_UNSWEPT ? 4 : 3) * L < (1 << (64 - 2 * (int)W)), "column accumulator would overflow");
+        FFU_ASSERT(strict(a) && strict(b) && strict(d));
+        FFU_ASSERT(a.l[L - 1] <= MASK && b.l[L - 1] <= MASK && d.l[L - 1] <= MASK);
+        if (C_UNSWEPT) {
+            for (int i = 0; i < L; i++) FFU_ASSERT(c.l[i] < (1u << (W + 1)));
+        } else {
+            FFU_ASSERT(strict(c) && c.l[L - 1] <= MASK);
+        }
         uint32_t m[L];
         uint64_t acc = 0;
         E r;
diff --git a/tokamak-zk-evm_amd/csrc/msm.hip b/tokamak-zk-evm_amd/csrc/msm.hip
--- a/tokamak-zk-evm_amd/csrc/msm.hip
+++ b/tokamak-zk-evm_amd/csrc/msm.hip
@@ -22,6 +22,7 @@
 #define TK_MSM_SYM_MSM bls12_381_msm
 #define TK_MSM_SYM_MULTI tkmk_msm_multi
 #define TK_MSM_SYM_PRECOMPUTE bls12_381_msm_precompute_bases
+#define TK_MSM_SYM_PRECOMPUTE_ACC bls12_381_msm_precompute_bases_acc
 #define TK_MSM_ABI_JOB_EX tkmk_msm_job_ex
 #define TK_MSM_SYM_MULTI_EX tkmk_msm_multi_ex
 #define TK_MSM_SYM_CONVERT bls12_381_msm_convert_bases
diff --git a/tokamak-zk-evm_amd/csrc/msm_impl.inc b/tokamak-zk-evm_amd/csrc/msm_impl.inc
--- a/tokamak-zk-evm_amd/csrc/msm_impl.inc
+++ b/tokamak-zk-evm_amd/csrc/msm_impl.inc
@@ -22,6 +22,13 @@
 using abi_job_ex = TK_MSM_ABI_JOB_EX;
 #endif
 constexpr size_t AFF_BYTES = sizeof(g1_affine_t), FR_BYTES = sizeof(fr_t);
+#ifdef TK_MSM_SYM_PRECOMPUTE_ACC
+using acc_row_t = G1U::Row;
+constexpr size_t ACC_ROW_BYTES = sizeof(acc_row_t);
+static_assert(ACC_ROW_BYTES == 128 && alignof(acc_row_t) == 128, "one row per 128-byte line");
+#else
+struct acc_row_t;
+#endif
 
 static_assert(sizeof(g1_affine_t) == 2 * 4 * Fq::N && sizeof(g1_xyzz_t) == 4 * 4 * Fq::N, "layout");
 static_assert(sizeof(abi_fr) == FR_BYTES && sizeof(abi_affine) == AFF_BYTES && sizeof(abi_proj) == 3 * 4 * Fq::N, "ABI layout");
@@ -126,8 +133,9 @@
     }
 }
 
-__global__ __launch_bounds__(128) void k_precompute_bases(const g1_affine_t *__restrict__ in, g1_affine_t *__restrict__ out, uint64_t n,
-                                                         int in_montgomery, uint32_t factor, uint32_t step) {
+template <class Out>
+__device__ __forceinline__ void precompute_bases_body(const g1_affine_t *__restrict__ in, Out *__restrict__ out, uint64_t n, int in_montgomery,
+                                                      uint32_t factor, uint32_t step) {
     uint64_t i = (uint64_t)blockIdx.x * blockDim.x + threadIdx.x;
     if (i >= n) return;
     g1_affine_t p = tk_load(in + i);
@@ -154,9 +162,21 @@
             a.x = Fq::mul(a.x, k);
             a.y = Fq::mul(a.y, k);
         }
-        tk_store(out + (uint64_t)j * n + i, a);
-    }
-}
+        Out rec;
+        G1U::to_record(rec, a);
+        tk_store(out + (uint64_t)j * n + i, rec);
+    }
+}
+__global__ __launch_bounds__(128) void k_precompute_bases(const g1_affine_t *__restrict__ in, g1_affine_t *__restrict__ out, uint64_t n,
+                                                         int in_montgomery, uint32_t factor, uint32_t step) {
+    precompute_bases_body(in, out, n, in_montgomery, factor, step);
+}
+#ifdef TK_MSM_SYM_PRECOMPUTE_ACC
+__global__ __launch_bounds__(128) void k_precompute_bases_acc(const g1_affine_t *__restrict__ in, acc_row_t *__restrict__ out, uint64_t n,
+                                                             int in_montgomery, uint32_t factor, uint32_t step) {
+    precompute_bases_body(in, out, n, in_montgomery, factor, step);
+}
+#endif
 
 __global__ __launch_bounds__(1024) void k_hist(const uint32_t *__restrict__ dig, uint32_t *__restrict__ counts, msm_plan_t pl,
                                               uint32_t shift) {
@@ -511,10 +531,11 @@
     return lo;
 }
 
-__global__ __launch_bounds__(256, 2) void k_accumulate_chunks(const g1_affine_t *__restrict__ bases, const uint32_t *__restrict__ sorted,
-                                                          const uint32_t *__restrict__ bstart, g1_xyzz_t *__restrict__ buckets,
-                                                          g1_xyzz_t *__restrict__ frag_head, g1_xyzz_t *__restrict__ frag_tail,
-                                                          msm_plan_t pl, uint32_t chunks_per_window) {
+template <class Row>
+__device__ __forceinline__ void accumulate_chunks_body(const Row *__restrict__ bases, const uint32_t *__restrict__ sorted,
+                                                       const uint32_t *__restrict__ bstart, g1_xyzz_t *__restrict__ buckets,
+                                                       g1_xyzz_t *__restrict__ frag_head, g1_xyzz_t *__restrict__ frag_tail,
+                                                       const msm_plan_t &pl, uint32_t chunks_per_window) {
     uint32_t gid = blockIdx.x * blockDim.x + threadIdx.x;
     if (gid >= pl.W * chunks_per_window) return;
     uint32_t w = gid / chunks_per_window, t = gid - w * chunks_per_window;
@@ -532,19 +553,25 @@
     uint32_t seg_lo = lo;
     G1U::X acc = G1U::inf();
     uint32_t rec_next = s[lo], rec_next2 = lo + 1 < hi ? s[lo + 1] : 0u;
-    g1_affine_t raw = tk_load(bases + (rec_next & 0x7fffffffu));
+    Row raw = tk_load(bases + (rec_next & 0x7fffffffu));
     for (uint32_t k = lo; k < hi; k++) {
         const uint32_t rec = rec_next;
         G1U::A q;
-        const bool have = G1U::load_affine(q, raw);
+        bool have;
+        if constexpr (std::is_same<Row, g1_affine_t>::value) have = G1U::load_affine(q, raw);
+        else have = G1U::load_row(q, raw);
         rec_next = rec_next2;
         if (k + 1 < hi) {
             raw = tk_load(bases + (rec_next & 0x7fffffffu));
         }
         if (k + 2 < hi) rec_next2 = s[k + 2];
         if (have) {
-            if (rec & 0x80000000u) q = G1U::neg(q);
-            acc = G1U::add_mixed(acc, q);
+            if constexpr (std::is_same<Row, g1_affine_t>::value) {
+                if (rec & 0x80000000u) q = G1U::neg(q);
+                acc = G1U::add_mixed(acc, q);
+            } else {
+                acc = G1U::add_mixed_masked(acc, q, (uint32_t)((int32_t)rec >> 31));
+            }
         }
         if (k + 1 == bend || k + 1 == hi) {
             bool whole = (seg_lo != lo || first_starts_here) && k + 1 == bend;
@@ -565,6 +592,21 @@
         }
     }
 }
+
+__global__ __launch_bounds__(256, 2) void k_accumulate_chunks(const g1_affine_t *__restrict__ bases, const uint32_t *__restrict__ sorted,
+                                                          const uint32_t *__restrict__ bstart, g1_xyzz_t *__restrict__ buckets,
+                                                          g1_xyzz_t *__restrict__ frag_head, g1_xyzz_t *__restrict__ frag_tail,
+                                                          msm_plan_t pl, uint32_t chunks_per_window) {
+    accumulate_chunks_body(bases, sorted, bstart, buckets, frag_head, frag_tail, pl, chunks_per_window);
+}
+#ifdef TK_MSM_SYM_PRECOMPUTE_ACC
+__global__ __launch_bounds__(256, 2) void k_accumulate_chunks_rows(const acc_row_t *__restrict__ bases, const uint32_t *__restrict__ sorted,
+                                                               const uint32_t *__restrict__ bstart, g1_xyzz_t *__restrict__ buckets,
+                                                               g1_xyzz_t *__restrict__ frag_head, g1_xyzz_t *__restrict__ frag_tail,
+                                                               msm_plan_t pl, uint32_t chunks_per_window) {
+    accumulate_chunks_body(bases, sorted, bstart, buckets, frag_head, frag_tail, pl, chunks_per_window);
+}
+#endif
 
 __global__ __launch_bounds__(256) void k_combine(const uint32_t *__restrict__ bstart, g1_xyzz_t *__restrict__ buckets,
                                                 const g1_xyzz_t *__restrict__ frag_head, const g1_xyzz_t *__restrict__ frag_tail,
@@ -1038,10 +1080,18 @@
     return c;
 }
 
+static hipError_t acc_kernels_set_lds(uint32_t bytes) {
+    hipError_t e = hipFuncSetAttribute((const void *)k_accumulate_chunks, hipFuncAttributeMaxDynamicSharedMemorySize, (int)bytes);
+#ifdef TK_MSM_SYM_PRECOMPUTE_ACC
+    if (e == hipSuccess) e = hipFuncSetAttribute((const void *)k_accumulate_chunks_rows, hipFuncAttributeMaxDynamicSharedMemorySize, (int)bytes);
+#endif
+    return e;
+}
 static thread_local bool tl_background_batch = false;
 static tkmk_error msm_enqueue(const fr_t *scalars, const g1_affine_t *bases_mont, uint32_t n_src, uint32_t factor, uint32_t c_req,
                               uint32_t bits, bool scalars_mont, hipStream_t s, g1_xyzz_t *wins_host, msm_plan_t *plan_out,
-                              msm_view_t sv = view_identity(), msm_view_t bv = view_identity(), uint32_t level_rows = 0) {
+                              msm_view_t sv = view_identity(), msm_view_t bv = view_identity(), uint32_t level_rows = 0,
+                              const acc_row_t *acc_rows = nullptr) {
     msm_plan_t pl;
     static const bool force_one_pass = getenv("TKMK_MSM_ONE_PASS") != nullptr;
     pl.bits = bits;
@@ -1190,17 +1240,23 @@
     static const uint32_t acc_lds = [] {
         const char *e = getenv("TKMK_MSM_ACC_LDS");
         uint32_t v = e ? (uint32_t)atoi(e) : 0u;
-        if (v && hipFuncSetAttribute((const void *)k_accumulate_chunks, hipFuncAttributeMaxDynamicSharedMemorySize, (int)v) != hipSuccess) v = 0;
+        if (v && acc_kernels_set_lds(v) != hipSuccess) v = 0;
         return v;
     }();
     static const uint32_t bg_lds = [] {
         const char *e = getenv("TKMK_MSM_BACKGROUND_LDS");
         uint32_t v = e ? (uint32_t)atoi(e) : 98304u;
-        if (v && hipFuncSetAttribute((const void *)k_accumulate_chunks, hipFuncAttributeMaxDynamicSharedMemorySize, (int)v) != hipSuccess) v = 0;
+        if (v && acc_kernels_set_lds(v) != hipSuccess) v = 0;
         return v;
     }();
     const uint32_t lds_claim = (tl_background_batch && bg_lds) ? bg_lds : acc_lds;
     prof.mark("msm.prepare");
+#ifdef TK_MSM_SYM_PRECOMPUTE_ACC
+    if (acc_rows)
+        hipLaunchKernelGGL(k_accumulate_chunks_rows, tk_div_up((size_t)pl.W * cpw, 256), 256, lds_claim, s, acc_rows, (const uint32_t *)d_sorted.p,
+                           (const uint32_t *)d_bstart.p, d_buckets.as<g1_xyzz_t>(), d_fh.as<g1_xyzz_t>(), d_ft.as<g1_xyzz_t>(), pl, cpw);
+    else
+#endif
     hipLaunchKernelGGL(k_accumulate_chunks, tk_div_up((size_t)pl.W * cpw, 256), 256, lds_claim, s, bases_mont, (const uint32_t *)d_sorted.p,
                        (const uint32_t *)d_bstart.p, d_buckets.as<g1_xyzz_t>(), d_fh.as<g1_xyzz_t>(), d_ft.as<g1_xyzz_t>(), pl, cpw);
     prof.mark("msm.accumulate");
@@ -1237,7 +1293,7 @@
         fprintf(stderr, "[msm debug] ptrs dig=%p sorted=%p counts=%p bstart=%p buckets=%p (+%zu) segs=%p (+%zu) wins=%p\n", d_dig.p,
                 d_sorted.p, d_counts.p, d_bstart.p, d_buckets.p, (size_t)pl.W * pl.B * sizeof(g1_xyzz_t), d_segs.p,
                 (size_t)pl.W * segs * sizeof(g1_xyzz_t), d_wins.p);
-    if (getenv("TKMK_MSM_DEBUG") && factor == 1 && view_is_identity(sv) && view_is_identity(bv) && !level_rows) TK_TRY(msm_debug_check(pl, scalars, bases_mont, d_dig.as<uint32_t>(), d_sorted.as<uint32_t>(),
+    if (getenv("TKMK_MSM_DEBUG") && factor == 1 && view_is_identity(sv) && view_is_identity(bv) && !level_rows && !acc_rows) TK_TRY(msm_debug_check(pl, scalars, bases_mont, d_dig.as<uint32_t>(), d_sorted.as<uint32_t>(),
                                                           d_bstart.as<uint32_t>(), d_buckets.as<g1_xyzz_t>(), s));
     TK_HIP(hipMemcpyAsync(wins_host, d_wins.p, wins_count * sizeof(g1_xyzz_t), hipMemcpyDeviceToHost, s));
     prof.finish();
@@ -1290,6 +1346,7 @@
     msm_view_t sv = view_identity(), bv = view_identity();
     uint32_t c = 0;
     uint32_t level_rows = 0;
+    bool acc_rows = false;
 };
 struct msm_pipe_set {
     std::mutex mu;
@@ -1380,7 +1437,8 @@
             bm = d_bm.as<g1_affine_t>();
         }
         err = msm_enqueue(jb.scalars, bm, jb.n, jb.factor, jb.c ? jb.c : c_req, bits, scalars_mont, sl.s, sl.wins, &sl.pl, jb.sv,
-                          jb.convert ? view_identity() : jb.bv, jb.convert ? 0u : jb.level_rows);
+                          jb.convert ? view_identity() : jb.bv, jb.convert ? 0u : jb.level_rows,
+                          jb.acc_rows && !jb.convert ? (const acc_row_t *)jb.bases : nullptr);
         if (err != TKMK_SUCCESS) break;
         if (hipEventRecord(sl.done, sl.s) != hipSuccess) err = TKMK_ERR_UNKNOWN;
     }
@@ -1579,7 +1637,10 @@
 
 TK_API tkmk_error TK_MSM_SYM_MULTI_EX(const abi_job_ex *jobs, int n_jobs, const tkmk_msm_config *cfg, int bases_form, abi_proj *results) {
     if (!cfg || cfg->ext || cfg->batch_size != 1 || n_jobs < 0 || cfg->precompute_factor > 1) return TKMK_ERR_INVALID_ARGUMENT;
-    if (bases_form != TKMK_BASES_PLAIN && bases_form != TKMK_BASES_MONTGOMERY && bases_form != TKMK_BASES_CONVERTED) return TKMK_ERR_INVALID_ARGUMENT;
+    if (bases_form != TKMK_BASES_PLAIN && bases_form != TKMK_BASES_MONTGOMERY && bases_form != TKMK_BASES_CONVERTED && bases_form != TKMK_BASES_ACC_READY)
+        return TKMK_ERR_INVALID_ARGUMENT;
+    const bool acc_ready = bases_form == TKMK_BASES_ACC_READY;
+    if (acc_ready) bases_form = TKMK_BASES_CONVERTED;
     if (cfg->bitsize < 0 || cfg->bitsize > 255 || cfg->c < 0 || cfg->c > MSM_MAX_C) return TKMK_ERR_INVALID_ARGUMENT;
     if (!cfg->are_scalars_on_device || !cfg->are_points_on_device) return TKMK_ERR_INVALID_ARGUMENT;
     if (n_jobs == 0) return TKMK_SUCCESS;
@@ -1600,10 +1661,14 @@
         if (jb.base_table_len >= (1ull << 31)) return TKMK_ERR_INVALID_ARGUMENT;
         if (jb.msm_size > 0 && jb.base_index && !jb.base_table_len) return TKMK_ERR_INVALID_ARGUMENT;
         if ((jb.table_c != 0) != (jb.table_factor != 0)) return TKMK_ERR_INVALID_ARGUMENT;
+        if (acc_ready && jb.table_c != 0 && jb.table_factor < 2) return TKMK_ERR_INVALID_ARGUMENT;
         if (jb.table_factor > 1) {
             if (bases_form != TKMK_BASES_CONVERTED || !jb.base_table_len || jb.table_c < 2 || jb.table_c > MSM_MAX_C) return TKMK_ERR_INVALID_ARGUMENT;
             if (jb.base_table_len * jb.table_factor >= (1ull << 31)) return TKMK_ERR_INVALID_ARGUMENT;
             if (jb.table_c > 16 && (uint64_t)jb.msm_size * jb.table_factor < (1ull << 18)) return TKMK_ERR_INVALID_ARGUMENT;
+            if (acc_ready) {
+                if (((uintptr_t)jb.bases & (ACC_ROW_BYTES - 1)) != 0 || jb.msm_size == 1) return TKMK_ERR_INVALID_ARGUMENT;
+            }
         }
     }
     tk_scratch d_flag;
@@ -1627,6 +1692,7 @@
             pjob.factor = jb.table_factor;
             pjob.c = jb.table_c;
             pjob.level_rows = (uint32_t)jb.base_table_len;
+            pjob.acc_rows = acc_ready;
         }
         pj.push_back(pjob);
         pj_index.push_back(j);
@@ -1696,4 +1762,34 @@
     return TKMK_SUCCESS;
 }
 
-}
+#ifdef TK_MSM_SYM_PRECOMPUTE_ACC
+TK_API tkmk_error TK_MSM_SYM_PRECOMPUTE_ACC(const abi_affine *bases, uint64_t n_points, const tkmk_msm_config *cfg, void *out, uint64_t *out_bytes) {
+    if (!cfg || cfg->ext || n_points < 2 || n_points >= (1ull << 31) || cfg->bitsize < 0 || cfg->bitsize > 255 || cfg->c < 0 || cfg->c > MSM_MAX_C ||
+        cfg->precompute_factor < 1)
+        return TKMK_ERR_INVALID_ARGUMENT;
+    const uint32_t n = (uint32_t)n_points;
+    const uint32_t bits = cfg->bitsize ? (uint32_t)cfg->bitsize : (uint32_t)TK_MSM_SCALAR_BITS;
+    const uint32_t c = cfg->c ? (uint32_t)cfg->c : msm_resolve_c(0, n);
+    const uint32_t w_src = bits / c + 1;
+    uint32_t factor = (uint32_t)cfg->precompute_factor;
+    if (factor > w_src) factor = w_src;
+    if ((uint64_t)n * factor >= (1ull << 31)) return TKMK_ERR_INVALID_ARGUMENT;
+    if (out_bytes) *out_bytes = (uint64_t)n * factor * ACC_ROW_BYTES;
+    if (!out) return out_bytes ? TKMK_SUCCESS : TKMK_ERR_INVALID_POINTER;
+    if (!bases) return TKMK_ERR_INVALID_POINTER;
+    if (((uintptr_t)out & (ACC_ROW_BYTES - 1)) != 0) return TKMK_ERR_INVALID_ARGUMENT;
+    TK_TRY(tk_require_device());
+    const uint32_t wg = (w_src + factor - 1) / factor;
+    hipStream_t s = tk_stream(cfg->stream_handle);
+    tk_frame frame(s);
+    tk_staged P;
+    TK_TRY(P.in(bases, (size_t)n * AFF_BYTES, cfg->are_points_on_device, s));
+    hipLaunchKernelGGL(k_precompute_bases_acc, tk_div_up(n, 128), 128, 0, s, (const g1_affine_t *)P.dev, (acc_row_t *)out, (uint64_t)n,
+                       cfg->are_points_montgomery_form ? 1 : 0, factor, c * wg);
+    TK_HIP(hipGetLastError());
+    TK_HIP(hipStreamSynchronize(s));
+    return TKMK_SUCCESS;
+}
+#endif
+
+}
diff --git a/tokamak-zk-evm_amd/host/tkmk_host.hpp b/tokamak-zk-evm_amd/host/tkmk_host.hpp
--- a/tokamak-zk-evm_amd/host/tkmk_host.hpp
+++ b/tokamak-zk-evm_amd/host/tkmk_host.hpp
@@ -893,8 +893,13 @@
     return c;
 }
 
+struct alignas(128) AccRow {
+    unsigned char bytes[128];
+};
+
 class Sigma1 {
     DeviceVec<G1Affine> xy_powers_;
+    DeviceVec<AccRow> table_;
     size_t rs_x_, rs_y_;
     uint32_t table_c_ = 0, table_factor_ = 0;
     Shard shard_;
@@ -910,15 +915,18 @@
         if (table_c >= 2 && xy_powers_.len() >= 2) {
             const uint32_t windows = 255 / table_c + 1;
             if ((uint64_t)xy_powers_.len() * windows >= (1ull << 31)) throw Error("xy_powers is too large for a precomputed table");
-            DeviceVec<G1Affine> table(xy_powers_.len() * windows);
-            cfg.c = (int)table_c;
-            cfg.precompute_factor = (int)windows;
-            check(bls12_381_msm_precompute_bases(xy_powers_.ptr(), (int)xy_powers_.len(), &cfg, table.ptr()), "msm::precompute_bases");
-            xy_powers_ = std::move(table);
+            tkmk_msm_config tcfg = cfg;
+            tcfg.c = (int)table_c;
+            tcfg.precompute_factor = (int)windows;
+            uint64_t bytes = 0;
+            check(bls12_381_msm_precompute_bases_acc(xy_powers_.ptr(), xy_powers_.len(), &tcfg, nullptr, &bytes), "msm::precompute_bases_acc (size)");
+            if (bytes != (uint64_t)xy_powers_.len() * windows * sizeof(AccRow)) throw Error("unexpected size of the accumulate-ready commit table");
+            DeviceVec<AccRow> table(xy_powers_.len() * windows);
+            check(bls12_381_msm_precompute_bases_acc(xy_powers_.ptr(), xy_powers_.len(), &tcfg, table.ptr(), nullptr), "msm::precompute_bases_acc");
+            table_ = std::move(table);
             table_c_ = table_c, table_factor_ = windows;
-        } else {
-            check(bls12_381_msm_convert_bases(xy_powers_.ptr(), xy_powers_.len(), &cfg, xy_powers_.ptr()), "msm::convert_bases");
-        }
+        }
+        check(bls12_381_msm_convert_bases(xy_powers_.ptr(), xy_powers_.len(), &cfg, xy_powers_.ptr()), "msm::convert_bases");
     }
     size_t rs_x() const { return rs_x_; }
     size_t rs_y() const { return rs_y_; }
@@ -946,6 +954,10 @@
         return out;
     }
     uint32_t table_c() const { return table_c_; }
+    void use_table(tkmk_msm_job_ex &j) const {
+        j.bases = reinterpret_cast<const G1Affine *>(table_.ptr());
+        j.table_c = table_c_, j.table_factor = table_factor_;
+    }
     tkmk_msm_job_ex job(DensePolynomialExt &poly, const char *name = nullptr) const {
         const auto deg = commit_box_sink() ? poly.find_degree() : poly.shape_degree();
         size_t tx = (size_t)(deg.first + 1), ty = (size_t)(deg.second + 1);
@@ -969,7 +981,7 @@
         j.base_cols = (uint32_t)mine, j.base_stride = (uint32_t)local_cols_;
         j.base_index = nullptr;
         j.base_table_len = table_len();
-        if (table_c_ && (uint64_t)tx * mine * table_factor_ >= (1ull << 20)) j.table_c = table_c_, j.table_factor = table_factor_;
+        if (table_c_ && (uint64_t)tx * mine * table_factor_ >= (1ull << 20)) use_table(j);
         return j;
     }
     static G1Affine to_affine(const tkmk_g1_projective &res) {
@@ -994,8 +1006,8 @@
             host_trace("commit batch of %zu:%s", jobs.size(), d.c_str());
         }
         const CommitComm &cc = commit_comm();
-        if (cc.comm) check(cc.multi_ex_sharded(cc.comm, jobs.data(), (int)jobs.size(), &cfg, TKMK_BASES_CONVERTED, res.data()), "tkmk_msm_multi_ex_sharded");
-        else check(tkmk_msm_multi_ex(jobs.data(), (int)jobs.size(), &cfg, TKMK_BASES_CONVERTED, res.data()), "tkmk_msm_multi_ex");
+        if (cc.comm) check(cc.multi_ex_sharded(cc.comm, jobs.data(), (int)jobs.size(), &cfg, TKMK_BASES_ACC_READY, res.data()), "tkmk_msm_multi_ex_sharded");
+        else check(tkmk_msm_multi_ex(jobs.data(), (int)jobs.size(), &cfg, TKMK_BASES_ACC_READY, res.data()), "tkmk_msm_multi_ex");
         std::vector<G1Affine> out;
         for (auto &r : res) out.push_back(to_affine(r));
         return out;
@@ -1010,7 +1022,7 @@
         j.bases = xy_powers_.ptr();
         j.msm_size = (int)(rs_x_ * rs_y_);
         j.base_table_len = table_len();
-        if (table_c_ && (uint64_t)rs_x_ * rs_y_ * table_factor_ >= (1ull << 20)) j.table_c = table_c_, j.table_factor = table_factor_;
+        if (table_c_ && (uint64_t)rs_x_ * rs_y_ * table_factor_ >= (1ull << 20)) use_table(j);
         return j;
     }
     static ScalarField inverse_of_grid_size(size_t xs, size_t ys) { return fr_inv(fr_mul(fr_from_u32((uint32_t)xs), fr_from_u32((uint32_t)ys))); }
diff --git a/tokamak-zk-evm_amd/tkmk/__init__.py b/tokamak-zk-evm_amd/tkmk/__init__.py
--- a/tokamak-zk-evm_amd/tkmk/__init__.py
+++ b/tokamak-zk-evm_amd/tkmk/__init__.py
@@ -74,7 +74,7 @@
     "tkmk_device_count", "tkmk_set_device", "tkmk_get_available_memory", "tkmk_malloc", "tkmk_malloc_async", "tkmk_free",
     "tkmk_free_async", "tkmk_memcpy_h2d", "tkmk_memcpy_d2h", "tkmk_memcpy_d2d", "tkmk_memcpy_h2d_async",
     "tkmk_memcpy_d2h_async", "tkmk_memcpy_2d_d2d", "tkmk_memset", "tkmk_stream_create", "tkmk_stream_synchronize", "tkmk_stream_destroy", "tkmk_stream_set_background",
-    "tkmk_device_synchronize", "tkmk_release_scratch", "tkmk_error_string", "tkmk_is_hip_build", "tkmk_keccak256", "tkmk_r1cs_index", "tkmk_msm_default_config", "bls12_381_msm", "bls12_381_g2_msm", "tkmk_g1_ntt", "tkmk_g1_ntt_axes", "tkmk_g1_prefix_sums", "tkmk_g1_scale", "bls12_381_msm_precompute_bases", "bn254_msm_precompute_bases", "tkmk_msm_multi", "bn254_msm", "tkmk_bn254_msm_multi", "bn254_get_root_of_unity", "bn254_ntt_init_domain", "bn254_ntt_release_domain",
+    "tkmk_device_synchronize", "tkmk_release_scratch", "tkmk_error_string", "tkmk_is_hip_build", "tkmk_keccak256", "tkmk_r1cs_index", "tkmk_msm_default_config", "bls12_381_msm", "bls12_381_g2_msm", "tkmk_g1_ntt", "tkmk_g1_ntt_axes", "tkmk_g1_prefix_sums", "tkmk_g1_scale", "bls12_381_msm_precompute_bases", "bls12_381_msm_precompute_bases_acc", "bn254_msm_precompute_bases", "tkmk_msm_multi", "bn254_msm", "tkmk_bn254_msm_multi", "bn254_get_root_of_unity", "bn254_ntt_init_domain", "bn254_ntt_release_domain",
     "bn254_ntt", "tkmk_bn254_bintt", "tkmk_bn254_fr_random_device",
     "tkmk_bn254_g1_batch_scalar_mul_device",
     "tkmk_ntt_default_config", "bls12_381_get_root_of_unity", "bls12_381_ntt_init_domain", "bls12_381_ntt_release_domain",
@@ -385,6 +385,21 @@
     f = min(factor, msm_windows(n, c, bitsize, curve, explicit_c=bool(c)))
     out = DeviceBuffer(aff * n * f)
     _check(getattr(lib(), sym)(_p(bases), int(n), ctypes.byref(cfg), _p(out)), sym)
+    return out
+
+
+def msm_precompute_bases_acc(bases, n, factor, c=0, bitsize=0, points_montgomery=False):
+    cfg = lib().tkmk_msm_default_config()
+    cfg.precompute_factor = factor
+    cfg.c, cfg.bitsize = c, bitsize
+    cfg.are_points_on_device = _on_dev(bases)
+    cfg.are_points_montgomery_form = points_montgomery
+    cfg.are_results_on_device = True
+    nbytes = ctypes.c_uint64(0)
+    fn = lib().bls12_381_msm_precompute_bases_acc
+    _check(fn(_p(bases), ctypes.c_uint64(n), ctypes.byref(cfg), None, ctypes.byref(nbytes)), "bls12_381_msm_precompute_bases_acc")
+    out = DeviceBuffer(nbytes.value)
+    _check(fn(_p(bases), ctypes.c_uint64(n), ctypes.byref(cfg), _p(out), None), "bls12_381_msm_precompute_bases_acc")
     return out
 
 
@@ -491,7 +506,7 @@
                 ("table_c", ctypes.c_uint32), ("table_factor", ctypes.c_uint32)]
 
 
-BASES_PLAIN, BASES_MONTGOMERY, BASES_CONVERTED = 0, 1, 2
+BASES_PLAIN, BASES_MONTGOMERY, BASES_CONVERTED, BASES_ACC_READY = 0, 1, 2, 3
 
 
 def msm_convert_bases(bases, n=None, points_montgomery=False, out=None):
```

Result: faster. 21.41 million, median of 6 (+3.0%).
